# siyuanwu99/pred-occ-planner

Measured on AMD Instinct MI355X. Metric: replans/sec (SOGM update + QP: full replan = SOGM update + A* + corridors + QP + deconfliction), 128-agent batch per GPU, 200x200x200x20 voxel grid; aggregate over all agents, higher is better.
Workload: dtype f32 occupancy / f64 planning; 1 GPU; 128 agents/GPU x 1 GPU, 200x200x200x20 SOGM, sim_fkpcp-style moving cylinders, batched ADMM QP (BASELINE configs[2] per GPU); agents_total=128, cloud_points=622040, cylinders=555, map_input_staleness_ticks=0, parallelism=agents sharded x1, 1 all-gather/tick, exchange=local, sogm_grids_per_agent=3, sogm_reset=sparse (logged 32-byte sectors), sogm_cell_order=2x2x2 tiles, map_update=at the start of the tick

## Files before the change

include/sogm_abi_debug.h:

```cpp
#ifndef SOGM_ABI_DEBUG_H
#define SOGM_ABI_DEBUG_H
#include "sogm_abi.h"
#ifdef __cplusplus
extern "C" {
#endif

int sogm_sparse_reset_state(sogm_ctx *ctx, int32_t *out_host);

int         sogm_set_tuning(sogm_ctx *ctx, const char *key, double value);
int         sogm_get_tuning(const sogm_ctx *ctx, const char *key, double *out_value_host);
const char *sogm_tuning_key(int index);

int sogm_map_traffic(sogm_ctx *ctx, int64_t *out_host, int reset);

int sogm_grid_history(sogm_ctx *ctx, int32_t *out_host);

enum {
  SOGM_PROF_CLEAR = 0,
  SOGM_PROF_STAMP = 1,
  SOGM_PROF_SPLAT = 2,
  SOGM_PROF_ASTAR = 3,
  SOGM_PROF_CORRIDOR = 4,
  SOGM_PROF_QP = 5,
  SOGM_PROF_CLEAR_HEAD = 6,
  SOGM_PROF_EXCHANGE = 7,
  SOGM_PROF_N = 8
};
int sogm_set_profiling(sogm_ctx *ctx, int enable);
int sogm_set_profiling_slots(sogm_ctx *ctx, int slot_mask);
int sogm_profile_read(sogm_ctx *ctx, double *out_ms_host);
int sogm_profile_read_all(sogm_ctx *ctx, int slot, double *out_ms_host, int cap, int *out_n);

int sogm_device_clock(sogm_ctx *ctx, int64_t *out_ticks_host, void *stream);
int sogm_tick_clock(sogm_ctx *ctx, int64_t *out2_host);

int sogm_download_reference_layout(sogm_ctx *ctx, int agent, float *out_vt_host);

int sogm_dsp_download_state(sogm_dsp *d, int agent, float *store_host, float *objnum_host,
                            int32_t *counters_host);
int sogm_dsp_download_born(sogm_dsp *d, int agent, float *born_host, int cap, int32_t *n_born, int32_t *counters4);
int sogm_dsp_download_observations(sogm_dsp *d, int agent, int32_t *nobs_host, float *pc_host,
                                   float *maxlen_host);

int sogm_gridmap_download(sogm_gridmap *g, int agent, double *occupancy_host, int8_t *inflate_host,
                          int32_t *bounds_host, int32_t *counters_host);
int sogm_gridmap_force_frame(sogm_gridmap *g, int raycast_num);

int sogm_corridor_rules_batched(sogm_planner *counters_of, const SogmPlannerParams *pp_host, const double *start_pva,
                                const double *route, const int32_t *route_len, int route_cap, const double *polys,
                                const int32_t *nfaces, const int32_t *seg_state, int n, int max_faces, double *out_box,
                                double *out_shrunk, int32_t *out_seg_nfaces, int32_t *out_seg_state, double *out_polys,
                                int32_t *out_nfaces, int32_t *out_npoly, double *out_goal, void *stream);

#ifdef __cplusplus
}
#endif
#endif
```

pred-occ-planner_amd/_abi.py:

```python
import ctypes as C
import os

_HERE = os.path.dirname(os.path.abspath(__file__))
LIB_PATH = os.environ.get("SOGM_LIB_PATH") or os.path.join(_HERE, "libsogm_hip.so")

SOGM_ABI_VERSION = 6
SOGM_MAX_PIECES = 16
SOGM_MAP_FAKE = 0
SOGM_MAP_RISKBASE = 1
SOGM_MAP_RISKVOXEL = 2
SOGM_STORE_F32, SOGM_STORE_F16 = 0, 1
SOGM_LAYOUT_TILED = 16
SOGM_DSP_MAX_T = 16

SOGM_OK = 0
SOGM_ERR_INVALID_ARG = -1
SOGM_ERR_NO_DEVICE = -2
SOGM_ERR_HIP = -3
SOGM_ERR_CAPACITY = -4
SOGM_ERR_STATE = -5
SOGM_ERR_COMM = -6
SOGM_COMM_ID_BYTES = 128
PROF_CLEAR, PROF_STAMP, PROF_SPLAT, PROF_ASTAR, PROF_CORRIDOR, PROF_QP, PROF_CLEAR_HEAD, PROF_EXCHANGE, PROF_N = range(9)

COUNTER_NAMES = ("replan_ok", "fail_search", "fail_corridor", "fail_qp", "fail_unsafe", "corridor_capacity",
                 "pieces_capacity", "deconflict_capacity")

ASTAR_NO_PATH, ASTAR_INIT_ERR, ASTAR_SEARCH_ERR, ASTAR_REACH_HORIZON, ASTAR_REACH_END, ASTAR_NEAR_END = range(6)


class SogmSpec(C.Structure):
    _fields_ = [("L", C.c_int32), ("W", C.c_int32), ("H", C.c_int32), ("T", C.c_int32),
                ("resolution", C.c_float), ("time_resolution", C.c_float),
                ("risk_threshold", C.c_float), ("clearance", C.c_float),
                ("ground_height", C.c_float), ("ceiling_height", C.c_float),
                ("risk_threshold_region", C.c_float), ("risk_thres_reg_decay", C.c_float),
                ("risk_thres_vox_decay", C.c_float), ("map_kind", C.c_int32),
                ("storage", C.c_int32)]


class SogmDspParams(C.Structure):
    _fields_ = [("max_particle_num_voxel", C.c_int32), ("half_fov_h", C.c_int32),
                ("half_fov_v", C.c_int32), ("angle_resolution", C.c_int32),
                ("newborn_num", C.c_int32), ("obs_max_per_pyramid", C.c_int32),
                ("prediction_times", C.c_float * SOGM_DSP_MAX_T),
                ("sigma_observation", C.c_float), ("p_detection", C.c_float), ("kappa", C.c_float),
                ("newborn_weight", C.c_float), ("obstacle_thickness", C.c_float)]


class SogmGridMapParams(C.Structure):
    _fields_ = [("resolution", C.c_double), ("map_size", C.c_double * 3), ("local_update_range", C.c_double * 3),
                ("obstacles_inflation", C.c_double), ("fx", C.c_double), ("fy", C.c_double), ("cx", C.c_double),
                ("cy", C.c_double), ("depth_filter_maxdist", C.c_double), ("depth_filter_mindist", C.c_double),
                ("k_depth_scaling_factor", C.c_double), ("p_hit", C.c_double), ("p_miss", C.c_double),
                ("p_min", C.c_double), ("p_max", C.c_double), ("p_occ", C.c_double), ("max_ray_length", C.c_double),
                ("virtual_ceil_height", C.c_double), ("ground_height", C.c_double),
                ("use_depth_filter", C.c_int32), ("depth_filter_margin", C.c_int32), ("skip_pixel", C.c_int32),
                ("local_map_margin", C.c_int32), ("rows", C.c_int32), ("cols", C.c_int32)]


class SogmCylinder(C.Structure):
    _fields_ = [("type", C.c_int32), ("_pad", C.c_int32)] + [
        (k, C.c_double) for k in ("x", "y", "z", "w", "h", "vx", "vy", "qw", "qx", "qy", "qz")]


class SogmTrajRecord(C.Structure):
    _fields_ = [("drone_id", C.c_int32), ("n_pieces", C.c_int32), ("time_start", C.c_double),
                ("duration", C.c_double * SOGM_MAX_PIECES),
                ("cpts", C.c_double * (SOGM_MAX_PIECES * 15))]


class SogmAstarParams(C.Structure):
    _fields_ = [("max_tau", C.c_double), ("max_vel", C.c_double), ("max_acc", C.c_double),
                ("w_time", C.c_double), ("horizon", C.c_double), ("lambda_heu", C.c_double),
                ("resolution", C.c_double), ("time_resolution", C.c_double),
                ("allocate_num", C.c_int32), ("check_num", C.c_int32), ("tolerance", C.c_int32),
                ("shot_ignores_time", C.c_int32)]


class SogmPlannerParams(C.Structure):
    _fields_ = [("corridor_tau", C.c_double), ("init_range", C.c_double),
                ("shrink_size", C.c_double), ("opt_max_vel", C.c_double),
                ("opt_max_acc", C.c_double), ("fake_planner", C.c_int32),
                ("firi_iterations", C.c_int32), ("pc_capacity", C.c_int32),
                ("max_faces", C.c_int32)]


class SogmQpSettings(C.Structure):
    _fields_ = [("rho", C.c_double), ("sigma", C.c_double), ("alpha", C.c_double),
                ("eps_abs", C.c_double), ("eps_rel", C.c_double), ("max_iter", C.c_int32),
                ("check_termination", C.c_int32), ("scaling_iters", C.c_int32),
                ("adaptive_rho_interval", C.c_int32), ("residual_fp32", C.c_int32), ("reserved_", C.c_int32)]


class SogmWorld(C.Structure):
    _fields_ = [("cloud_xyz", C.c_void_p), ("block_bounds", C.c_void_p), ("cylinders", C.c_void_p),
                ("n_points", C.c_int32), ("n_blocks", C.c_int32), ("block_points", C.c_int32), ("n_cyl", C.c_int32)]


class SogmPrestamp(C.Structure):
    _fields_ = [("cloud_xyz", C.c_void_p), ("cloud_range", C.c_void_p), ("cylinders", C.c_void_p),
                ("n_cyl", C.c_int32), ("reserved_", C.c_int32), ("next_stamp", C.c_double),
                ("replan_start_offset", C.c_double), ("hover_inout", C.c_void_p), ("out_now", C.c_void_p),
                ("out_t_start", C.c_void_p), ("out_pva", C.c_void_p), ("out_poses", C.c_void_p),
                ("world", C.POINTER(SogmWorld))]


class SogmFlight(C.Structure):
    _fields_ = [("n_ticks", C.c_int32), ("first_tick", C.c_int32), ("t0", C.c_double), ("period", C.c_double),
                ("replan_start_offset", C.c_double), ("worlds", C.POINTER(SogmWorld)), ("goals", C.c_void_p),
                ("drone_ids", C.c_void_p), ("hover_inout", C.c_void_p), ("own_inout", C.c_void_p),
                ("tables", C.c_void_p), ("n_total", C.c_int32), ("agent0", C.c_int32), ("log_records", C.c_void_p),
                ("log_ok", C.c_void_p), ("nccl_comm", C.c_void_p)]


class SogmAuditParams(C.Structure):
    _fields_ = [("body", C.c_double * 3), ("sample_dt", C.c_double), ("goal_tolerance", C.c_double),
                ("t_obstacles", C.c_double), ("event_capacity", C.c_int32), ("reserved_", C.c_int32)]


class SogmAuditAgent(C.Structure):
    _fields_ = [("min_gap", C.c_double), ("min_gap_time", C.c_double), ("min_sep", C.c_double),
                ("min_sep_time", C.c_double), ("goal_time", C.c_double), ("first_collision_time", C.c_double),
                ("path_length", C.c_double), ("last_pos", C.c_double * 3), ("min_gap_obstacle", C.c_int32),
                ("min_sep_agent", C.c_int32), ("obstacle_samples", C.c_int32), ("agent_samples", C.c_int32),
                ("n_samples", C.c_int32), ("has_last", C.c_int32)]


class SogmAuditEvent(C.Structure):
    _fields_ = [("t", C.c_double), ("agent", C.c_int32), ("other", C.c_int32), ("kind", C.c_int32),
                ("reserved_", C.c_int32)]


SOGM_AUDIT_AGENT, SOGM_AUDIT_OBSTACLE = 0, 1
AUDIT_AGENT_BYTES = C.sizeof(SogmAuditAgent)
AUDIT_EVENT_BYTES = C.sizeof(SogmAuditEvent)


class SogmFsmParams(C.Structure):
    _fields_ = [("replan_duration", C.c_double), ("replan_start_time", C.c_double), ("goal_tolerance", C.c_double),
                ("new_plan_interval", C.c_double), ("replan_max_failures", C.c_int32), ("reserved_", C.c_int32)]


class SogmFsmState(C.Structure):
    _fields_ = [("traj_start", C.c_double), ("status", C.c_int32), ("fail", C.c_int32), ("success", C.c_int32),
                ("reserved_", C.c_int32)]


class SogmFlightFsm(C.Structure):
    _fields_ = [("prm", SogmFsmParams), ("check_duration", C.c_double), ("state_inout", C.c_void_p),
                ("log_state", C.c_void_p), ("log_due", C.c_void_p), ("log_safe", C.c_void_p), ("log_reached", C.c_void_p),
                ("log_pub", C.c_void_p), ("log_hover_start", C.c_void_p), ("log_own", C.c_void_p)]


FSM_STATE_BYTES = C.sizeof(SogmFsmState)
FSM_PUB_NONE, FSM_PUB_NEW, FSM_PUB_HOVER = 0, 1, 2

FLIGHT_MAX_TICKS = 64
FLIGHT_HDR_ERR, FLIGHT_HDR_FINISHED, FLIGHT_HDR_LATE_WGS = 4, 5, 15
FLIGHT_STAT_NAMES = ("gate_wait", "map", "search", "corridor", "qp", "finish", "chain", "ticks")
TRAJ_RECORD_BYTES = C.sizeof(SogmTrajRecord)
CYLINDER_BYTES = C.sizeof(SogmCylinder)

_vp = C.c_void_p
_i = C.c_int

PROTOTYPES = {
    "sogm_abi_version": (_i, []),
    "sogm_last_error": (C.c_char_p, []),
    "sogm_device_count": (_i, []),
    "sogm_create": (_i, [C.POINTER(SogmSpec), _i, _i, C.POINTER(_vp)]),
    "sogm_destroy": (None, [_vp]),
    "sogm_grid_bytes": (C.c_int64, [_vp]),
    "sogm_grid_ptr": (_vp, [_vp]),
    "sogm_set_sparse_reset": (_i, [_vp, _i, _i]),
    "sogm_sparse_reset_state": (_i, [_vp, _vp]),
    "sogm_grid_history": (_i, [_vp, _vp]),
    "sogm_map_traffic": (_i, [_vp, _vp, _i]),
    "sogm_set_resample": (_i, [_vp, C.c_float, _i, _vp, _i]),
    "sogm_set_tuning": (_i, [_vp, C.c_char_p, C.c_double]),
    "sogm_get_tuning": (_i, [_vp, C.c_char_p, C.POINTER(C.c_double)]),
    "sogm_tuning_key": (C.c_char_p, [_i]),
    "sogm_set_body_particles": (_i, [_vp, C.POINTER(C.c_double), _i]),
    "sogm_set_overlap_clear": (_i, [_vp, _i]),
    "sogm_set_profiling": (_i, [_vp, _i]),
    "sogm_set_profiling_slots": (_i, [_vp, _i]),
    "sogm_profile_read": (_i, [_vp, C.POINTER(C.c_double)]),
    "sogm_profile_read_all": (_i, [_vp, _i, C.POINTER(C.c_double), _i, C.POINTER(_i)]),
    "sogm_update_gt": (_i, [_vp, _vp, _vp, _vp, _i, _vp, _vp, _vp]),
    "sogm_project_neighbours": (_i, [_vp, _vp, _i, _vp, _vp]),
    "sogm_update_gt_swarm": (_i, [_vp, _vp, _vp, _vp, _i, _vp, _vp, _vp, _i, _vp, _vp]),
    "sogm_device_clock": (_i, [_vp, C.POINTER(C.c_int64), _vp]),
    "sogm_tick_clock": (_i, [_vp, C.POINTER(C.c_int64)]),
    "sogm_cloud_block_bounds": (_i, [_vp, _i, _i, _vp, _vp]),
    "sogm_update_world": (_i, [_vp, C.POINTER(SogmWorld), _vp, _vp, _vp, _i, _vp, _vp]),
    "sogm_set_future_risk": (_i, [_vp, _vp, _vp, _vp, _vp]),
    "sogm_download_reference_layout": (_i, [_vp, _i, _vp]),
    "sogm_tick_inputs": (_i, [_vp, _i, C.c_double, C.c_double, _vp, _vp, _vp, _vp, _vp, _vp]),
    "sogm_merge_latest": (_i, [_vp, _vp, _vp, _vp, _i, _vp]),
    "sogm_fsm_init": (_i, [_vp, _i, C.c_double, _vp]),
    "sogm_fsm_inputs": (_i, [C.POINTER(SogmFsmParams), _vp, _vp, _vp, _i, C.c_double, _vp, _vp, _vp, _vp, _vp, _vp, _vp,
                             _vp, _vp]),
    "sogm_fsm_apply": (_i, [C.POINTER(SogmFsmParams), _vp, _vp, _vp, _vp, _vp, _vp, _vp, _vp, _vp, _vp, _vp, _i,
                            C.c_double, _vp]),
    "sogm_map_state": (_i, [_vp, _i, C.POINTER(C.c_double), C.POINTER(C.c_float), _vp]),
    "sogm_traj_eval": (_i, [_vp, _i, _vp, _vp, _vp, _vp]),
    "sogm_firi_batched": (_i, [_vp, _i, _vp, _vp, _vp, _vp, _vp, _i, C.c_double, _i, _i, _i, _vp, _vp, _vp, _vp]),
    "sogm_planner_select_agents": (_i, [_vp, _i, _i]),
    "sogm_planner_set_search_mode": (_i, [_vp, _i]),
    "sogm_query_clear": (_i, [_vp, _vp, _vp, _vp, _i, _i, _vp, _vp]),
    "sogm_obstacle_points": (_i, [_vp, _vp, _vp, _vp, _vp, _vp, _i, _vp, _vp, _i, _vp]),
    "sogm_planner_create": (_i, [_vp, C.POINTER(SogmAstarParams), C.POINTER(SogmPlannerParams),
                                 C.POINTER(SogmQpSettings), C.POINTER(_vp)]),
    "sogm_planner_destroy": (None, [_vp]),
    "sogm_astar_search": (_i, [_vp, _vp, _vp, _vp, _vp, _vp, _vp, _i, _vp, _vp, _i, _vp]),
    "sogm_corridor_generate": (_i, [_vp, _vp, _vp, _vp, _vp, _i, _vp, _vp, _vp, _vp, _vp]),
    "sogm_bezier_qp_solve": (_i, [_vp, _vp, _vp, _vp, _vp, _vp, _vp, _vp, _vp, _vp]),
    "sogm_bezier_qp_solve_timed": (_i, [_vp, _vp, _vp, _vp, C.c_double, C.c_double, _vp, _vp, _vp, _vp, _vp, _vp, _vp]),
    "sogm_linprog_batched": (_i, [_i, _vp, _vp, _vp, _vp, _i, _vp, _vp, _vp]),
    "sogm_corridor_rules_batched": (_i, [_vp, _vp, _vp, _vp, _vp, _i, _vp, _vp, _vp, _i, _i, _vp, _vp, _vp, _vp, _vp, _vp,
                                         _vp, _vp, _vp]),
    "sogm_replan": (_i, [_vp, _vp, _vp, _vp, _vp, _vp, _vp, _vp]),
    "sogm_gridmap_create": (_i, [C.POINTER(SogmGridMapParams), _i, _i, C.POINTER(_vp)]),
    "sogm_gridmap_destroy": (None, [_vp]),
    "sogm_gridmap_update": (_i, [_vp, _vp, _vp, _vp, _vp, _vp]),
    "sogm_gridmap_query_inflate": (_i, [_vp, _vp, _vp, _i, _vp, _vp]),
    "sogm_gridmap_download": (_i, [_vp, _i, _vp, _vp, _vp, _vp]),
    "sogm_gridmap_force_frame": (_i, [_vp, _i]),
    "sogm_traj_safe": (_i, [_vp, _vp, _vp, C.c_double, _vp, _vp]),
    "sogm_safe_after_opt": (_i, [_vp, _vp, _vp, _vp, _i, _vp, _vp, _vp, _vp]),
    "sogm_planner_flow_error": (_i, [_vp]),
    "sogm_planner_flow_failures": (_i, [_vp, _vp]),
    "sogm_planner_set_publish": (_i, [_vp, _vp, _vp]),
    "sogm_planner_set_prestamp": (_i, [_vp, _vp]),
    "sogm_prestamp_pending": (_i, [_vp]),
    "sogm_prestamp_join": (_i, [_vp, _vp]),
    "sogm_update_prestamped": (_i, [_vp, _vp, _i, _vp, _vp]),
    "sogm_planner_counters": (_i, [_vp, C.POINTER(C.c_int64), _i]),
    "sogm_flight_run": (_i, [_vp, C.POINTER(SogmFlight), _vp]),
    "sogm_flight_prepare": (_i, [_vp, _i]),
    "sogm_flight_stats": (_i, [_vp, _vp, _vp]),
    "sogm_planner_set_swarm": (_i, [_vp, _vp, _i, _vp, _vp]),
    "sogm_planner_set_due": (_i, [_vp, _vp]),
    "sogm_planner_set_flight_fsm": (_i, [_vp, C.POINTER(SogmFlightFsm)]),
    "sogm_audit_init_agents": (_i, [_vp, _i, _vp]),
    "sogm_swarm_audit": (_i, [C.POINTER(SogmAuditParams), _vp, _i, _i, _vp, C.c_double, _i, C.c_double, _i, _i, _vp, _vp,
                              _vp, _i, _vp, _vp, _vp, _vp]),
    "sogm_traj_allgather": (_i, [_vp, _vp, _vp, _i, _vp, _vp]),
    "sogm_exchange_wait": (_i, [_vp, _vp]),
    "sogm_comm_unique_id": (_i, [C.c_char_p]),
    "sogm_comm_create": (_i, [C.c_char_p, _i, _i, _i, C.POINTER(_vp)]),
    "sogm_comm_destroy": (None, [_vp]),
    "sogm_comm_handle": (_vp, [_vp]),
    "sogm_comm_info": (_i, [_vp, _vp]),
    "sogm_filter_point_cloud": (_i, [_vp, _vp, _vp, C.c_float, _i, _vp, _vp, _vp]),
    "sogm_filter_reserve": (_i, [_vp, _i]),
    "sogm_dsp_create": (_i, [_vp, C.POINTER(SogmDspParams), _vp, _vp, _i, _vp, _i, _i, C.POINTER(_vp)]),
    "sogm_dsp_destroy": (None, [_vp]),
    "sogm_update_dsp": (_i, [_vp, _vp, _vp, _vp, _vp, _vp, _vp, _vp, _vp]),
    "sogm_dsp_publish": (_i, [_vp, _vp, _vp]),
    "sogm_dsp_download_state": (_i, [_vp, _i, _vp, _vp, _vp]),
    "sogm_dsp_download_born": (_i, [_vp, _i, _vp, _i, _vp, _vp]),
    "sogm_dsp_download_observations": (_i, [_vp, _i, _vp, _vp, _vp]),
}


class SogmError(RuntimeError):
    pass


def load_library(path=LIB_PATH):
    if not os.path.exists(path):
        raise SogmError(
            f"HIP extension not built: {path} is missing. Run `python -c 'import __graft_entry__ as g; "
            "g.build()'` (hipcc --offload-arch=gfx950). There is no CPU fallback.")
    try:
        import torch
    except ImportError:
        pass
    lib = C.CDLL(path)
    for name, (res, args) in PROTOTYPES.items():
        fn = getattr(lib, name)
        fn.restype = res
        fn.argtypes = args
    got = lib.sogm_abi_version()
    if got != SOGM_ABI_VERSION:
        raise SogmError(f"{path} implements ABI version {got}, this binding was written against {SOGM_ABI_VERSION}: "
                        "rebuild the extension (python -c 'import __graft_entry__ as g; g.build()')")
    return lib


_lib = None


def lib():
    global _lib
    if _lib is None:
        _lib = load_library()
    return _lib


def check(rc, what):
    if rc != SOGM_OK:
        msg = lib().sogm_last_error()
        raise SogmError(f"{what} failed: status {rc} ({msg.decode() if msg else ''})")
```

pred-occ-planner_amd/csrc/sogm_corridor.hip:

```cpp
#include <hip/hip_runtime.h>

#include <cfloat>

#include "../../include/sogm_detmath.h"
#include "sogm_fsm.hpp"
#include "sogm_lp.hpp"
#include "sogm_planner.hpp"

namespace sogm {
namespace {

__device__ inline double dot3(const double *a, const double *b) {
  return (a[0] * b[0] + a[1] * b[1]) + a[2] * b[2];
}

__device__ inline bool smoothedL1(double mu, double x, double &f, double &df) {
  if (x < 0.0) return false;
  if (x > mu) {
    f  = x - 0.5 * mu;
    df = 1.0;
    return true;
  }
  const double xdmu = x / mu, sqrxdmu = xdmu * xdmu, mumxd2 = mu - 0.5 * x;
  f  = mumxd2 * sqrxdmu * xdmu;
// ... 825 lines not shown
  const double   *rt    = DIRECT ? nullptr : io.route + (size_t)agent * io.route_cap * 6;
  const double   *sp    = DIRECT ? nullptr : io.start_pva + agent * 9;
  const int       cap   = pp.pc_capacity;
  const int       prob  = DIRECT ? fd.first + slot : 0;
  const double   *pc    = DIRECT ? fd.pc + (size_t)fd.pc_range[prob * 2] * 3 : ws.pc + (size_t)slot * cap * 3;
  double         *fpc   = ws.fpc + (size_t)slot * cap * 3;
  double         *tang  = ws.tang + (size_t)slot * cap * 4;
  double         *distR = ws.distr + (size_t)slot * cap;

  long long *dbg = ws.seg_dbg + (size_t)slot * 16;
  const long long tk0 = wall_clock64();
  const int M = DIRECT ? fd.n_bd : 6;
  if (lane == 0) {
    for (int k = 0; k < 12; ++k) dbg[k] = 0;
    if constexpr (DIRECT) {
      for (int i = 0; i < 4 * M; ++i) s_bd[i] = fd.bd[(size_t)prob * M * 4 + i];
      for (int k = 0; k < 3; ++k) {
        s_w[k]     = fd.a[prob * 3 + k];
        s_w[3 + k] = fd.b[prob * 3 + k];
      }
    } else {
      segment_box(pp, sp, rt, seg, s_box, s_w);
      for (int i = 0; i < 24; ++i) s_bd[i] = 0;
      for (int k = 0; k < 3; ++k) {
        s_bd[k * 4 + k]       = 1.0;
        s_bd[(k + 3) * 4 + k] = -1.0;
        s_bd[k * 4 + 3]       = -s_box[3 + k];
        s_bd[(k + 3) * 4 + 3] = s_box[k];
      }
    }
  }
  __syncthreads();

  int N = DIRECT ? fd.pc_range[prob * 2 + 1] - fd.pc_range[prob * 2] : ws.seg_npts[slot];
  int overflow = 0;
  if (N > cap) {
    N        = cap;
    overflow = 1;
  }
  __syncthreads();

  if (lane == 0) {
    dbg[0] = N;
    dbg[5] = wall_clock64() - tk0;
  }
  const double epsilon = DIRECT ? fd.epsilon : 1.0e-6;
  int          nH      = 0;
  const int    n_iter  = DIRECT ? fd.iterations : pp.firi_iterations;
  bool         seed_ok = true;
  if (lane == 0) {
    int ok = 1;
    for (int i = 0; i < M; ++i) {
      const double *h = s_bd + i * 4;
      if (dot3(h, s_w) + h[3] > 0.0 || dot3(h, s_w + 3) + h[3] > 0.0) ok = 0;
    }
    s_int[0] = ok;
  }
  __syncthreads();
  seed_ok = s_int[0] != 0;

  if (seed_ok) {
    double R[3][3] = {{1, 0, 0}, {0, 1, 0}, {0, 0, 1}};
    double p[3]    = {0.5 * (s_w[0] + s_w[3]), 0.5 * (s_w[1] + s_w[4]), 0.5 * (s_w[2] + s_w[5])};
    double r[3]    = {1, 1, 1};
    if constexpr (DIRECT)
      for (int k = 0; k < 3; ++k) r[k] = fd.r[prob * 3 + k];
    for (int loop = 0; loop < n_iter; ++loop) {
      if (lane == 0) {
        double forward[3][3], backward[3][3];
        for (int k = 0; k < 3; ++k)
          for (int j = 0; j < 3; ++j) {
            forward[k][j]    = (1.0 / r[k]) * R[j][k];
            backward[k][j]   = R[k][j] * r[j];
            s_fwd[k * 3 + j] = forward[k][j];
          }
        for (int i = 0; i < M; ++i) {
          const double *h = s_bd + i * 4;
          for (int j = 0; j < 3; ++j)
            s_fB[i * 3 + j] =
                (h[0] * backward[0][j] + h[1] * backward[1][j]) + h[2] * backward[2][j];
          s_fD[i] = h[3] + dot3(h, p);
        }
        const double da[3] = {s_w[0] - p[0], s_w[1] - p[1], s_w[2] - p[2]};
        const double db[3] = {s_w[3] - p[0], s_w[4] - p[1], s_w[5] - p[2]};
        for (int k = 0; k < 3; ++k) {
          s_fa[k] = dot3(forward[k], da);
          s_fb[k] = dot3(forward[k], db);
          s_p[k]  = p[k];
        }
        for (int i = 0; i < M; ++i) {
          const double *fb = s_fB + i * 3;
          s_dD[i]          = dabs(s_fD[i]) / sogm_det::sqrt_rn(dot3(fb, fb));
        }
      }
      __syncthreads();
      double lmin = INFINITY;
      int    lidx = 0x7fffffff;
      {
        double fwd[9], fa[3], fb[3], pp3[3];
        for (int k = 0; k < 9; ++k) fwd[k] = s_fwd[k];
        for (int k = 0; k < 3; ++k) {
          fa[k]  = s_fa[k];
          fb[k]  = s_fb[k];
          pp3[k] = s_p[k];
        }
        for (int i = lane; i < N; i += 64) {
          const double d[3] = {pc[i * 3] - pp3[0], pc[i * 3 + 1] - pp3[1], pc[i * 3 + 2] - pp3[2]};
          double       q[3];
          for (int k = 0; k < 3; ++k) q[k] = dot3(fwd + k * 3, d);
          double t[4];
          double dr = sogm_det::sqrt_rn(dot3(q, q));
          t[3]      = -dr;
          for (int k = 0; k < 3; ++k) t[k] = q[k] / dr;
          if (dot3(t, fa) + t[3] > epsilon) {
            const double delta[3] = {q[0] - fa[0], q[1] - fa[1], q[2] - fa[2]};
            const double s        = dot3(delta, fa) / dot3(delta, delta);
            for (int k = 0; k < 3; ++k) t[k] = fa[k] - s * delta[k];
            dr   = sogm_det::sqrt_rn(dot3(t, t));
            t[3] = -dr;
            for (int k = 0; k < 3; ++k) t[k] /= dr;
          }
          if (dot3(t, fb) + t[3] > epsilon) {
            const double delta[3] = {q[0] - fb[0], q[1] - fb[1], q[2] - fb[2]};
            const double s        = dot3(delta, fb) / dot3(delta, delta);
            for (int k = 0; k < 3; ++k) t[k] = fb[k] - s * delta[k];
            dr   = sogm_det::sqrt_rn(dot3(t, t));
            t[3] = -dr;
            for (int k = 0; k < 3; ++k) t[k] /= dr;
          }
          if (dot3(t, fa) + t[3] > epsilon) {
            const double u[3] = {fa[0] - q[0], fa[1] - q[1], fa[2] - q[2]};
            const double v[3] = {fb[0] - q[0], fb[1] - q[1], fb[2] - q[2]};
            double       n[3] = {u[1] * v[2] - u[2] * v[1], u[2] * v[0] - u[0] * v[2],
                                 u[0] * v[1] - u[1] * v[0]};
            const double nn   = sogm_det::sqrt_rn(dot3(n, n));
            if (nn > 0)
              for (int k = 0; k < 3; ++k) n[k] /= nn;
            for (int k = 0; k < 3; ++k) t[k] = n[k];
            t[3]            = -dot3(t, fa);
            const double sg = t[3] > 0.0 ? -1.0 : 1.0;
            for (int k = 0; k < 4; ++k) t[k] *= sg;
          }
          for (int k = 0; k < 3; ++k) fpc[i * 3 + k] = q[k];
          for (int k = 0; k < 4; ++k) tang[i * 4 + k] = t[k];
          distR[i]  = dr;
          {
            const unsigned long long act = __ballot(1);
            if (lane == 0) s_fw[i >> 6] = act;
          }
          if (dr < lmin) {
            lmin = dr;
            lidx = i;
          }
        }
      }
      wave_argmin(lmin, lidx);
      double minSqrR = lmin;
      int    pcMinId = lidx == 0x7fffffff ? 0 : lidx;
      double minSqrD = INFINITY;
      int    bdMinId = 0;
      unsigned bdFlags = M >= 32 ? 0xffffffffu : (1u << M) - 1u;
      for (int j = 0; j < M; ++j)
        if (s_dD[j] < minSqrD) {
          minSqrD = s_dD[j];
          bdMinId = j;
        }
      nH             = 0;
      bool completed = false;
      for (int i = 0; !completed && i < (M + N); ++i) {
        __syncthreads();
        if (lane == 0) {
          double *fh = s_fH + (nH < FIRI_MAX_H ? nH : FIRI_MAX_H - 1) * 4;
          if (minSqrD < minSqrR) {
            for (int k = 0; k < 3; ++k) fh[k] = s_fB[bdMinId * 3 + k];
            fh[3] = s_fD[bdMinId];
          } else {
            for (int k = 0; k < 4; ++k) fh[k] = tang[pcMinId * 4 + k];
            s_fw[pcMinId >> 6] &= ~(1ull << (pcMinId & 63));
          }
          for (int k = 0; k < 4; ++k) s_fh[k] = fh[k];
        }
        if (minSqrD < minSqrR) bdFlags &= ~(1u << bdMinId);
        __syncthreads();
        completed = true;
        minSqrD   = INFINITY;
        for (int j = 0; j < M; ++j)
          if (bdFlags & (1u << j)) {
            completed = false;
            if (minSqrD > s_dD[j]) {
              bdMinId = j;
              minSqrD = s_dD[j];
            }
          }
        const double fh0 = s_fh[0], fh1 = s_fh[1], fh2 = s_fh[2], fh3 = s_fh[3];
        double       lm = INFINITY;
        int          li = 0x7fffffff;
        int          open = 0;
        for (int j = lane; j < N; j += 64) {
          const unsigned long long word = s_fw[j >> 6];
          bool                     covered = false;
          if ((word >> lane) & 1ull) {
            const double *q = fpc + j * 3;
            if (((fh0 * q[0] + fh1 * q[1]) + fh2 * q[2]) + fh3 > -epsilon) {
              covered = true;
            } else {
              open = 1;
              if (lm > distR[j]) {
                lm = distR[j];
                li = j;
              }
            }
          }
          const unsigned long long clr = __ballot(covered);
          if (clr != 0ull && lane == 0) s_fw[j >> 6] = word & ~clr;
        }
        wave_argmin(lm, li);
        if (__any(open)) completed = false;
        minSqrR = lm;
        pcMinId = li == 0x7fffffff ? 0 : li;
        ++nH;
      }
      __syncthreads();
      if (nH > FIRI_MAX_H) {
        nH       = FIRI_MAX_H;
        overflow = 1;
      }
      for (int i = lane; i < nH; i += 64) {
        const double *fh = s_fH + i * 4;
        double        h[4];
        for (int j = 0; j < 3; ++j)
          h[j] = (fh[0] * s_fwd[0 * 3 + j] + fh[1] * s_fwd[1 * 3 + j]) + fh[2] * s_fwd[2 * 3 + j];
        h[3] = fh[3] - dot3(h, s_p);
        for (int k = 0; k < 4; ++k) s_poly[i * 4 + k] = h[k];
      }
      __syncthreads();
      if (lane == 0) {
        dbg[1 + (loop > 0)] = nH;
        dbg[6 + 2 * (loop > 0)] = wall_clock64() - tk0;
      }
      if (loop == n_iter - 1) break;
      {
        const int       mm  = nH < LP_MAX_ROWS - 9 ? nH : LP_MAX_ROWS - 9;
        const long long tm0 = wall_clock64();
        maxVolInsEllipsoid(s_poly, mm, R, p, r, sc, base + L::lm, base + L::handoff, dbg);
        if (lane == 0) dbg[7] = wall_clock64() - tm0;
      }
      __syncthreads();
    }
    if constexpr (DIRECT)
      if (lane == 0)
        for (int k = 0; k < 3; ++k) fd.r[prob * 3 + k] = r[k];
  }

  if constexpr (DIRECT) {
    int nf = seed_ok ? nH : 0;
    if (nf > fd.max_faces) {
      nf       = fd.max_faces;
      overflow = 1;
    }
    double *out = fd.hpoly + (size_t)prob * fd.max_faces * 4;
    for (int i = lane; i < nf * 4; i += 64) out[i] = s_poly[i];
    if (lane == 0) {
      fd.nfaces[prob] = nf;
      fd.status[prob] = overflow ? -3 : (seed_ok ? 1 : 0);
    }
    return;
  }
  int nf = seed_ok ? nH : 0;
  if (nf > pp.max_faces) {
    nf       = pp.max_faces;
    overflow = 1;
  }
  shrink_corridor(pp, s_w, s_poly, nf);
  wave_lds_sync();
  const bool valid = corridorValidW(s_poly, nf, nullptr, 0, sc);
  {
    double *out = ws.polys + (size_t)slot * pp.max_faces * 4;
    for (int i = lane; i < nf * 4; i += 64) out[i] = s_poly[i];
  }
  if (lane == 0) {
    ws.seg_nfaces[slot] = nf;
    ws.seg_state[slot]  = overflow ? -3 : (valid ? 1 : 0);
    ws.seg_npts[slot]   = N;
    dbg[10]             = wall_clock64() - tk0;
  }
}

__global__ __launch_bounds__(64) void k_corridor_segment(
    MapView m, SogmPlannerParams pp, CorridorWorkspace ws, const double *__restrict__ start_pva,
    const double *__restrict__ t_start, const double *__restrict__ route,
    const int32_t *__restrict__ route_len, int route_cap, int agent0) {
  extern __shared__ __attribute__((aligned(16))) char smem[];
  const CorridorIO io{.start_pva = start_pva, .t_start = t_start, .route = route, .route_len = route_len,
                      .route_cap = route_cap};
  corridor_segment_body<6, false>(m, pp, ws, io, blockIdx.y + agent0, blockIdx.x, smem, FiriDirect{});
}

__global__ __launch_bounds__(64) void k_firi_direct(MapView m, SogmPlannerParams pp, CorridorWorkspace ws,
                                                    FiriDirect fd) {
  extern __shared__ __attribute__((aligned(16))) char smem[];
  corridor_segment_body<FIRI_DIRECT_BD_MAX, true>(m, pp, ws, CorridorIO{}, blockIdx.x, 0, smem, fd);
}

__device__ __forceinline__ void corridor_finalize_body(const SogmPlannerParams &pp, const CorridorWorkspace &ws,
                                                       const CorridorIO &io, int agent, const LpScratch &sc) {
  const bool    w0    = threadIdx.x == 0;
  const int     MF    = pp.max_faces;
  const double *polys = ws.polys + (size_t)agent * SOGM_MAX_PIECES * MF * 4;
  const int    *nfs   = ws.seg_nfaces + agent * SOGM_MAX_PIECES;
  const int    *state = ws.seg_state + agent * SOGM_MAX_PIECES;
  const double *rt    = io.route + (size_t)agent * io.route_cap * 6;
  const double *sp    = io.start_pva + agent * 9;
  const int     rl    = io.points(agent);
  int           npoly = 0;
  if (w0) {
    for (int i = 0; i < SOGM_MAX_PIECES; ++i) io.out_nfaces[agent * SOGM_MAX_PIECES + i] = 0;
    for (int i = 0; i < 6; ++i) io.out_goal[agent * 6 + i] = 0;
    io.out_npoly[agent] = 0;
  }
  if (!pp.fake_planner && rl < 2) return;
  if (rl < 1) return;
  for (int i = 0; i < rl - 1 && i < SOGM_MAX_PIECES; ++i) {
    if (state[i] != 1) {
      if (state[i] == -3 && w0 && ws.counters) atomicAdd(&ws.counters[SOGM_CNT_CORRIDOR_CAPACITY], 1ull);
      break;
    }
    ++npoly;
  }
  if (npoly == SOGM_MAX_PIECES && io.route_len[agent] - 1 > SOGM_MAX_PIECES && w0 && ws.counters)
    atomicAdd(&ws.counters[SOGM_CNT_PIECES_CAPACITY], 1ull);
  if (npoly == 0) return;
  for (int i = 0; i + 1 < npoly; ++i) {
    if (!corridorValidW(polys + (size_t)i * MF * 4, nfs[i], polys + (size_t)(i + 1) * MF * 4,
                        nfs[i + 1], sc)) {
      if (i < 2) return;
      npoly = pp.fake_planner ? i + 1 : i;
      break;
    }
  }
  if (pp.fake_planner ? npoly == 0 : npoly <= 1) return;
  double gpos[3], gvel[3];
  int    gi = npoly - 1;
  for (int k = 0; k < 3; ++k) {
    gpos[k] = rt[gi * 6 + k];
    gvel[k] = rt[gi * 6 + 3 + k];
  }
  bool do_scan = true;
  if (!pp.fake_planner)
    do_scan = !goalReachableW(polys + (size_t)(npoly - 1) * MF * 4, nfs[npoly - 1], sp, gpos, sc);
  if (do_scan) {
    for (int it = npoly - 1; it != 0; --it) {
      if (goalReachableW(polys + (size_t)it * MF * 4, nfs[it], sp, gpos, sc)) {
        npoly         = it + 1;
        const int idx = npoly - 1;
        for (int k = 0; k < 3; ++k) {
          gpos[k] = rt[idx * 6 + k];
          gvel[k] = rt[idx * 6 + 3 + k];
        }
        break;
      }
    }
  }
  for (int i = 0; i < npoly; ++i) {
    if (w0) io.out_nfaces[agent * SOGM_MAX_PIECES + i] = nfs[i];
    const double *src = polys + (size_t)i * MF * 4;
    double       *dst = io.out_polys + ((size_t)agent * SOGM_MAX_PIECES + i) * MF * 4;
    for (int k = threadIdx.x; k < nfs[i] * 4; k += 64) dst[k] = src[k];
  }
  if (w0) {
    for (int k = 0; k < 3; ++k) {
      io.out_goal[agent * 6 + k]     = gpos[k];
      io.out_goal[agent * 6 + 3 + k] = gvel[k];
    }
    io.out_npoly[agent] = npoly;
  }
}

__global__ __launch_bounds__(64) void k_corridor_finalize(
    SogmPlannerParams pp, CorridorWorkspace ws, const double *__restrict__ start_pva,
    const double *__restrict__ route, const int32_t *__restrict__ route_len, int route_cap,
    double *__restrict__ out_polys, int32_t *__restrict__ out_nfaces,
    int32_t *__restrict__ out_npoly, double *__restrict__ out_goal, int agent0) {
  const CorridorIO io{.start_pva = start_pva, .route = route, .route_len = route_len, .route_cap = route_cap,
                      .out_polys = out_polys, .out_nfaces = out_nfaces, .out_npoly = out_npoly, .out_goal = out_goal};
  extern __shared__ __attribute__((aligned(16))) char smem[];
  corridor_finalize_body(pp, ws, io, blockIdx.x + agent0, LpLds::carve(smem));
}

struct CorridorRules {
  const SogmPlannerParams *pp;
  const double            *polys_in;
  const int32_t           *nfaces_in;
  const int32_t           *state_in;
  double                  *out_box;
};
__global__ __launch_bounds__(64) void k_corridor_rules(CorridorRules cr, CorridorWorkspace ws, CorridorIO io) {
  extern __shared__ __attribute__((aligned(16))) char smem[];
  double *base = (double *)smem, *s_poly = base + RulesLds::poly, *s_box = base + RulesLds::box, *s_w = base + RulesLds::w;
  const LpScratch sc{base + LpLds::work, base + LpLds::rows, (int *)(smem + RulesLds::perm)};
  const int               prob = blockIdx.x, lane = threadIdx.x;
  const SogmPlannerParams pp   = cr.pp[prob];
  const int               MF   = pp.max_faces;
  const int               rl   = io.points(prob);
  for (int seg = 0; seg < SOGM_MAX_PIECES; ++seg) {
    const int slot = prob * SOGM_MAX_PIECES + seg;
    if (seg >= rl - 1) {
      if (lane == 0) {
        ws.seg_state[slot]  = -2;
        ws.seg_nfaces[slot] = 0;
        for (int k = 0; k < 6; ++k) cr.out_box[slot * 6 + k] = 0.0;
      }
      continue;
    }
    int nf = cr.nfaces_in[slot];
    nf     = nf < 0 ? 0 : (nf > MF ? MF : nf);
    if (lane == 0) segment_box(pp, io.start_pva + prob * 9, io.route + (size_t)prob * io.route_cap * 6, seg, s_box, s_w);
    for (int i = lane; i < nf * 4; i += 64) s_poly[i] = cr.polys_in[(size_t)slot * MF * 4 + i];
    wave_lds_sync();
    shrink_corridor(pp, s_w, s_poly, nf);
    wave_lds_sync();
    const bool valid = corridorValidW(s_poly, nf, nullptr, 0, sc);
    double    *out   = ws.polys + (size_t)slot * MF * 4;
    for (int i = lane; i < nf * 4; i += 64) out[i] = s_poly[i];
    if (lane == 0) {
      for (int k = 0; k < 6; ++k) cr.out_box[slot * 6 + k] = s_box[k];
      ws.seg_nfaces[slot] = nf;
      ws.seg_state[slot]  = cr.state_in && cr.state_in[slot] == -3 ? -3 : (valid ? 1 : 0);
    }
    wave_lds_sync();
  }
  __threadfence_block();
  __syncthreads();
  corridor_finalize_body(pp, ws, io, prob, sc);
}

__device__ __forceinline__ bool corridor_slot(const MapView &m, const SogmPlannerParams &pp, const CorridorWorkspace &ws,
                                              const CorridorIO &io, int agent, int seg, char *smem, int *seg_done,
                                              bool cumulative, long long *stamps) {
  if (seg < io.points(agent) - 1) {
    corridor_points_body<1>(m, pp, ws, io, agent, seg);
    __threadfence_block();
    __syncthreads();
  }
  if (stamps && threadIdx.x == 0) stamps[13] = wall_clock64();
  corridor_segment_body<6, false>(m, pp, ws, io, agent, seg, smem, FiriDirect{});
  __syncthreads();
  if (stamps && threadIdx.x == 0) stamps[14] = wall_clock64();
  __threadfence();
  const int done = flow_ticket(&seg_done[agent]);
  if ((cumulative ? done & (SOGM_MAX_PIECES - 1) : done) != SOGM_MAX_PIECES - 1) return false;
  __threadfence();
  corridor_finalize_body(pp, ws, io, agent, LpLds::carve(smem));
  __syncthreads();
  return true;
}

__global__ __launch_bounds__(64) void k_corridor_flow(MapView m, SogmPlannerParams pp, CorridorWorkspace ws,
                                                      FlowCtl fc, CorridorIO io, int n_agents) {
  extern __shared__ __attribute__((aligned(16))) char smem[];
  const int lane  = threadIdx.x;
  const int total = n_agents * SOGM_MAX_PIECES;
  for (;;) {
    const int k = flow_ticket(&fc.hdr[FLOW_C_TICKET]);
    if (k >= total) break;
    const int agent = flow_wait_slot(fc.a_ready + k / SOGM_MAX_PIECES, &fc.hdr[FLOW_ERR]);
    if (agent < 0) break;
    __threadfence();
    const int seg = k % SOGM_MAX_PIECES;
    if (seg == 0 && lane == 0) fc.ts[agent * 8 + 2] = wall_clock64();
    if (corridor_slot(m, pp, ws, io, agent, seg, smem, fc.seg_done, false, nullptr)) {
      if (lane == 0) fc.ts[agent * 8 + 3] = wall_clock64();
      __threadfence();
      if (lane == 0) publish_next(fc.q_ready, &fc.hdr[FLOW_Q_READY_N], agent);
    }
    __syncthreads();
  }
}

__device__ __forceinline__ bool deconflict_pair_unsafe(const double *ca, int M, const SogmTrajRecord &r, int ego_id,
                                                       double now, const LpScratch &sc, unsigned long long *counters) {
  if (M <= 0) return false;
  if (r.n_pieces <= 0 || r.drone_id == ego_id) return false;
  double time_end = r.time_start;
  for (int k = 0; k < r.n_pieces; ++k) time_end += r.duration[k];
  if (!(r.time_start < now && now < time_end)) return false;
  double t     = now - r.time_start;
  int    piece = r.n_pieces - 1;
  for (int k = 0; k < r.n_pieces; ++k) {
    t -= r.duration[k];
    if (t < 0) {
      piece = k;
      break;
    }
  }
  const int nA = 5 * M, nB = (r.n_pieces - piece) * 5;
  if (nA + nB > DECONFLICT_MAX_ROWS) {
    if ((threadIdx.x & 63) == 0 && counters) atomicAdd(&counters[SOGM_CNT_DECONFLICT_CAPACITY], 1ull);
    return true;
  }
  double       *A = sc.A(), *b = sc.b();
  const double *cb = r.cpts + piece * 15;
  {
    double lo[6], hi[6];
    for (int k = 0; k < 6; ++k) {
      lo[k] = INFINITY;
      hi[k] = -INFINITY;
    }
    for (int q = threadIdx.x; q < nA; q += 64)
      for (int k = 0; k < 3; ++k) {
        lo[k] = fmin(lo[k], ca[q * 3 + k]);
        hi[k] = fmax(hi[k], ca[q * 3 + k]);
      }
    for (int q = threadIdx.x; q < nB; q += 64)
      for (int k = 0; k < 3; ++k) {
        lo[3 + k] = fmin(lo[3 + k], cb[q * 3 + k]);
        hi[3 + k] = fmax(hi[3 + k], cb[q * 3 + k]);
      }
    bool apart = false;
    for (int k = 0; k < 6; ++k)
      for (int d = 32; d >= 1; d >>= 1) {
        lo[k] = fmin(lo[k], __shfl_xor(lo[k], d, 64));
        hi[k] = fmax(hi[k], __shfl_xor(hi[k], d, 64));
      }
    for (int k = 0; k < 3; ++k) apart = apart || hi[k] < lo[3 + k] || hi[3 + k] < lo[k];
    if (apart) return false;
    double dirs[11][3] = {{1, 1, 0}, {1, -1, 0}, {1, 0, 1}, {1, 0, -1}, {0, 1, 1}, {0, 1, -1},
                          {1, 1, 1}, {1, 1, -1}, {1, -1, 1}, {1, -1, -1}, {0, 0, 0}};
    for (int k = 0; k < 3; ++k) dirs[10][k] = 0.5 * (lo[3 + k] + hi[3 + k]) - 0.5 * (lo[k] + hi[k]);
#pragma unroll
    for (int q = 0; q < 11; ++q) {
      const double n0 = dirs[q][0], n1 = dirs[q][1], n2 = dirs[q][2];
      double loA = INFINITY, hiA = -INFINITY, loB = INFINITY, hiB = -INFINITY;
      for (int i = threadIdx.x; i < nA; i += 64) {
        const double v = (n0 * ca[i * 3] + n1 * ca[i * 3 + 1]) + n2 * ca[i * 3 + 2];
        loA = fmin(loA, v);
        hiA = fmax(hiA, v);
      }
      for (int i = threadIdx.x; i < nB; i += 64) {
        const double v = (n0 * cb[i * 3] + n1 * cb[i * 3 + 1]) + n2 * cb[i * 3 + 2];
        loB = fmin(loB, v);
        hiB = fmax(hiB, v);
      }
      for (int d = 32; d >= 1; d >>= 1) {
        loA = fmin(loA, __shfl_xor(loA, d, 64));
        hiA = fmax(hiA, __shfl_xor(hiA, d, 64));
        loB = fmin(loB, __shfl_xor(loB, d, 64));
        hiB = fmax(hiB, __shfl_xor(hiB, d, 64));
      }
      if (hiA < loB || hiB < loA) return false;
    }
  }
  for (int q = threadIdx.x; q < nA + nB; q += 64) {
    if (q < nA) {
      A[q * 4 + 0] = -ca[q * 3 + 0];
      A[q * 4 + 1] = -ca[q * 3 + 1];
      A[q * 4 + 2] = -ca[q * 3 + 2];
      A[q * 4 + 3] = -1.0;
    } else {
      const int e  = q - nA;
      A[q * 4 + 0] = cb[e * 3 + 0];
      A[q * 4 + 1] = cb[e * 3 + 1];
      A[q * 4 + 2] = cb[e * 3 + 2];
      A[q * 4 + 3] = 1.0;
    }
    b[q] = -1.0;
  }
  if (threadIdx.x < 8) {
    const int q = nA + nB + threadIdx.x, k = threadIdx.x >> 1;
    for (int j = 0; j < 4; ++j) A[q * 4 + j] = j == k ? ((threadIdx.x & 1) ? -1.0 : 1.0) : 0.0;
    b[q] = 1.0e4;
  }
  wave_lds_sync();
  const double c[4] = {0, 0, 0, 0};
  double       x[4];
  const double v = linprog_wave<4>(c, nA + nB + 8, A, b, x, sc.work, sc.perm);
  wave_lds_sync();
  return v == INFINITY || v == -INFINITY;
}

__device__ inline bool deconflict_prefilter(const double *sA, int nA, const double *boxA, const double (*prA)[2],
                                            const SogmTrajRecord &r, int ego_id, double now) {
  const int np = r.n_pieces;
  if (np <= 0 || r.drone_id == ego_id) return false;
  const double ts = r.time_start;
  double       time_end = ts;
  for (int k = 0; k < np; ++k) time_end += r.duration[k];
  if (!(ts < now && now < time_end)) return false;
  double t     = now - ts;
  int    piece = np - 1;
  for (int k = 0; k < np; ++k) {
    t -= r.duration[k];
    if (t < 0) {
      piece = k;
      break;
    }
  }
  const int nB = (np - piece) * 5;
  if (nA + nB > DECONFLICT_MAX_ROWS) return true;
  const double *cb = r.cpts + piece * 15;
  const double  dirs[10][3] = {{1, 1, 0}, {1, -1, 0}, {1, 0, 1}, {1, 0, -1}, {0, 1, 1},
                               {0, 1, -1}, {1, 1, 1}, {1, 1, -1}, {1, -1, 1}, {1, -1, -1}};
  double lo[3] = {INFINITY, INFINITY, INFINITY}, hi[3] = {-INFINITY, -INFINITY, -INFINITY};
  double plo[10], phi[10];
#pragma unroll
  for (int q = 0; q < 10; ++q) {
    plo[q] = INFINITY;
    phi[q] = -INFINITY;
  }
#pragma unroll 4
  for (int i = 0; i < nB; ++i) {
    const double x = cb[i * 3], y = cb[i * 3 + 1], z = cb[i * 3 + 2];
    lo[0] = fmin(lo[0], x);
    hi[0] = fmax(hi[0], x);
    lo[1] = fmin(lo[1], y);
    hi[1] = fmax(hi[1], y);
    lo[2] = fmin(lo[2], z);
    hi[2] = fmax(hi[2], z);
#pragma unroll
    for (int q = 0; q < 10; ++q) {
      const double v = (dirs[q][0] * x + dirs[q][1] * y) + dirs[q][2] * z;
      plo[q]         = fmin(plo[q], v);
      phi[q]         = fmax(phi[q], v);
    }
  }
  for (int k = 0; k < 3; ++k)
    if (boxA[3 + k] < lo[k] || hi[k] < boxA[k]) return false;
#pragma unroll
  for (int q = 0; q < 10; ++q)
    if (prA[q][1] < plo[q] || phi[q] < prA[q][0]) return false;
  double n[3];
  for (int k = 0; k < 3; ++k) n[k] = 0.5 * (lo[k] + hi[k]) - 0.5 * (boxA[k] + boxA[3 + k]);
  double loA = INFINITY, hiA = -INFINITY, loB = INFINITY, hiB = -INFINITY;
  for (int i = 0; i < nA; ++i) {
    const double v = (n[0] * sA[i * 3] + n[1] * sA[i * 3 + 1]) + n[2] * sA[i * 3 + 2];
    loA            = fmin(loA, v);
    hiA            = fmax(hiA, v);
  }
  for (int i = 0; i < nB; ++i) {
    const double v = (n[0] * cb[i * 3] + n[1] * cb[i * 3 + 1]) + n[2] * cb[i * 3 + 2];
    loB            = fmin(loB, v);
    hiB            = fmax(hiB, v);
  }
  if (hiA < loB || hiB < loA) return false;
  return true;
}

__global__ __launch_bounds__(64) void k_safe_after_opt(const double *__restrict__ cpts,
                                                       const int32_t *__restrict__ npoly,
                                                       const SogmTrajRecord *__restrict__ rec, int n_rec,
                                                       const int32_t *__restrict__ ego_ids,
                                                       const double *__restrict__ t_now,
                                                       int32_t *__restrict__ out_safe, int agent0,
                                                       unsigned long long *counters) {
  extern __shared__ __attribute__((aligned(16))) double s_dyn[];
  const int a = blockIdx.y + agent0, i = blockIdx.x;
  if (deconflict_pair_unsafe(cpts + (size_t)a * SOGM_MAX_PIECES * 15, npoly[a], rec[i], ego_ids[a], t_now[a],
                             LpLds::carve(s_dyn), counters) &&
      threadIdx.x == 0)
    out_safe[a] = 0;
}

__device__ __forceinline__ int finish_agent(const FinishArgs &f, int a, const LpScratch &sc, int lane) {
  const int M    = f.npoly[a];
  int       safe = 1;
  const bool solved = f.ret[a] != 0 && M > 0 && (f.status[a] == 1 || f.status[a] == 2);
  if (f.swarm && solved) {
    const double *ca  = f.cpts + (size_t)a * SOGM_MAX_PIECES * 15;
    const int     ego = f.swarm_ego[a];
    const double  now = f.swarm_now[a];
    const int     nA  = 5 * M;
    double *sA = sc.work;
    double  boxA[6], prA[10][2];
    auto stage_A = [&]() {
      for (int q = lane; q < nA * 3; q += 64) sA[q] = ca[q];
      wave_lds_sync();
    };
    stage_A();
    {
      const double dirs[10][3] = {{1, 1, 0}, {1, -1, 0}, {1, 0, 1}, {1, 0, -1}, {0, 1, 1},
                                  {0, 1, -1}, {1, 1, 1}, {1, 1, -1}, {1, -1, 1}, {1, -1, -1}};
      double lo[13], hi[13];
#pragma unroll
      for (int k = 0; k < 13; ++k) {
        lo[k] = INFINITY;
        hi[k] = -INFINITY;
      }
      for (int q = lane; q < nA; q += 64) {
        const double x = sA[q * 3], y = sA[q * 3 + 1], z = sA[q * 3 + 2];
        lo[0] = fmin(lo[0], x);
        hi[0] = fmax(hi[0], x);
        lo[1] = fmin(lo[1], y);
        hi[1] = fmax(hi[1], y);
        lo[2] = fmin(lo[2], z);
        hi[2] = fmax(hi[2], z);
#pragma unroll
        for (int k = 0; k < 10; ++k) {
          const double v = (dirs[k][0] * x + dirs[k][1] * y) + dirs[k][2] * z;
          lo[3 + k]      = fmin(lo[3 + k], v);
          hi[3 + k]      = fmax(hi[3 + k], v);
        }
      }
#pragma unroll
      for (int k = 0; k < 13; ++k)
        for (int d = 32; d >= 1; d >>= 1) {
          lo[k] = fmin(lo[k], __shfl_xor(lo[k], d, 64));
          hi[k] = fmax(hi[k], __shfl_xor(hi[k], d, 64));
        }
      for (int k = 0; k < 3; ++k) {
        boxA[k]     = lo[k];
        boxA[3 + k] = hi[k];
      }
#pragma unroll
      for (int k = 0; k < 10; ++k) {
        prA[k][0] = lo[3 + k];
        prA[k][1] = hi[3 + k];
      }
    }
    for (int i0 = 0; i0 < f.n_swarm && safe; i0 += 64) {
      const int  i    = i0 + lane;
      const bool need = i < f.n_swarm && deconflict_prefilter(sA, nA, boxA, prA, f.swarm[i], ego, now);
      unsigned long long m = __ballot(need);
      bool               lp_ran = false;
      while (m != 0 && safe) {
        const int j = __builtin_ctzll(m);
        m &= m - 1;
        if (deconflict_pair_unsafe(ca, M, f.swarm[i0 + j], ego, now, sc, f.counters)) safe = 0;
        lp_ran = true;
      }
      if (lp_ran && safe && i0 + 64 < f.n_swarm) stage_A();
    }
  }
#ifdef SOGM_FLOW_DEBUG
  if (lane == 0) f.out_safe[a] = 101;
#else
  if (lane == 0 && f.out_safe) f.out_safe[a] = safe;
#endif
  const bool      good = solved && safe != 0;
  SogmTrajRecord *dst[3] = {f.out + a, (good && f.pub_own) ? f.pub_own + a : nullptr,
                            (good && f.pub_own && f.pub_table) ? f.pub_table + a : nullptr};
#pragma unroll
  for (int k = 0; k < 3; ++k) {
    SogmTrajRecord *r = dst[k];
    if (!r) continue;
    for (int i = lane; i < SOGM_MAX_PIECES; i += 64) r->duration[i] = (good && i < M) ? f.corridor_tau : 0.0;
    for (int i = lane; i < SOGM_MAX_PIECES * 15; i += 64)
      r->cpts[i] = (good && i < M * 15) ? f.cpts[(size_t)a * SOGM_MAX_PIECES * 15 + i] : 0.0;
    if (lane == 0) {
      r->drone_id   = f.drone_ids[a];
      r->time_start = f.t_start[a];
      r->n_pieces   = good ? M : 0;
    }
  }
  if (!good && f.pub_own && f.pub_table)
    copy_record(f.pub_table + a, f.pub_own + a, lane);
  if (lane == 0) f.out_ok[a] = good ? 1 : 0;
  return (safe ? 1 : 0) | (good ? 2 : 0);
}
// ... 3 lines not shown
  if (f.due && f.due[a] == 0) return;
  const int M = f.npoly[a];
  int       k = SOGM_CNT_REPLAN_OK;
  if (f.ret[a] == 0) k = SOGM_CNT_FAIL_SEARCH;
  else if (M <= 0) k = SOGM_CNT_FAIL_CORRIDOR;
  else if (!(f.status[a] == 1 || f.status[a] == 2)) k = SOGM_CNT_FAIL_QP;
  else if (!safe) k = SOGM_CNT_FAIL_UNSAFE;
  atomicAdd(&f.counters[k], 1ull);
}
__global__ __launch_bounds__(64) void k_finish_flow(FlowCtl fc, FinishArgs f, int n_agents) {
  extern __shared__ __attribute__((aligned(16))) double s_dyn[];
  const int lane = threadIdx.x;
  for (;;) {
    const int k = flow_ticket(&fc.hdr[FLOW_F_TICKET]);
    if (k >= n_agents) break;
    const int a = flow_wait_slot(fc.f_ready + k, &fc.hdr[FLOW_ERR]);
    if (a < 0) break;
    __threadfence();
    const int  code = finish_agent(f, a, LpLds::carve(s_dyn), lane);
    const bool safe = (code & 1) != 0;
    if (fc.p_ready) {
      __threadfence();
      if (lane == 0) publish_next(fc.p_ready, &fc.hdr[FLOW_P_READY_N], a);
    }
    if (lane == 0) {
      fc.ts[a * 8 + 6] = wall_clock64();
      finish_count(f, a, safe);
    }
  }
}

__device__ inline int flight_fsm_traj_safe(const MapView &m, const FlightFsmDev &u, const FinishArgs &f, int a, int lane) {
  const int mine = traj_safe_agent(m, a, f.pub_own[a], f.swarm_now[a], u.check_duration, lane, 64);
  return __ballot(mine == 0) == 0ull ? 1 : 0;
}
__device__ inline void flight_fsm_apply(const FlightFsmDev &u, const FinishArgs &f, int a, size_t row, bool ok, int safe,
                                        int lane) {
  const double stamp = f.swarm_now[a];
  int          kind  = 0;
  double       start = 0.0;
  if (lane == 0) {
    SogmFsmState  s       = u.state[a];
    const int32_t due     = u.due[a], reached = u.reached[a];
    const FsmPub  pub     = fsm_step(s, due, ok, safe != 0, reached != 0, stamp, u.prm);
    u.state[a]            = s;
    kind                  = pub.kind;
    start                 = pub.hover_start;
    if (u.log_state) u.log_state[row] = s;
    if (u.log_due) u.log_due[row] = due;
    if (u.log_safe) u.log_safe[row] = safe;
    if (u.log_reached) u.log_reached[row] = reached;
    if (u.log_pub) u.log_pub[row] = pub.kind;
    if (u.log_hover_start) u.log_hover_start[row] = pub.hover_start;
  }
  kind  = __shfl(kind, 0, 64);
  start = __shfl(start, 0, 64);
  if (kind == SOGM_FSM_PUB_HOVER) {
    const double p[3] = {u.pos_now[a * 3], u.pos_now[a * 3 + 1], u.pos_now[a * 3 + 2]};
    fsm_hover_record(f.pub_own[a], f.drone_ids[a], p, start, lane, 64);
    if (f.pub_table) fsm_hover_record(f.pub_table[a], f.drone_ids[a], p, start, lane, 64);
  }
  if (u.log_own) {
    __threadfence();
    copy_record(u.log_own + row, f.pub_own + a, lane);
  }
}

__global__ __launch_bounds__(64) void k_flight_light(MapView m, SogmPlannerParams pp, CorridorWorkspace ws, FlightCtl fl,
                                                     FlightLightDev d) {
  extern __shared__ __attribute__((aligned(16))) char smem[];
  const int      lane  = threadIdx.x;
  const unsigned total = (unsigned)fl.n_agents * (unsigned)fl.n_ticks * (SOGM_MAX_PIECES + 1);
  int           *err   = &fl.hdr[FL_ERR];
  fl_wg_started(fl, 2);
  long long      c1_prev = 0;
  int            kind_prev = 0;
  for (;;) {
    const unsigned t = (unsigned)flow_ticket(&fl.hdr[FL_LW_HEAD]);
    if (t >= total) break;
    const long long c0   = wall_clock64();
    const int       desc = wq_take(fl.lw, t, err);
    if (desc < 0) break;
    __threadfence();
    const long long c1 = wall_clock64();
    if (lane == 0) {
      if (c1_prev) {
        atomicAdd(&fl.prof[kind_prev == WK_FINISH ? 8 : 7], (unsigned long long)(c0 - c1_prev));
        atomicAdd(&fl.prof[kind_prev == WK_FINISH ? 15 : 14], 1ull);
      }
      atomicAdd(&fl.prof[6], (unsigned long long)(c1 - c0));
    }
    const int kind = wk_kind(desc), a = wk_agent(desc);
    c1_prev   = c1;
    kind_prev = kind;
    if (kind == WK_FINISH) {
      const int k  = fl.tick_of[a];
      const int kl = k - fl.first_tick;
      FinishArgs f = d.fin;
      f.swarm      = d.tables ? d.tables + (size_t)((k - fl.lag) & 3) * d.n_total : nullptr;
      f.pub_table  = d.tables ? d.tables + (size_t)(k & 3) * d.n_total + d.agent0 : nullptr;
      f.out        = d.log_records + (size_t)kl * fl.n_agents;
      f.out_ok     = d.log_ok + (size_t)kl * fl.n_agents;
      int traj_safe = 1;
      if (d.fsm.state) traj_safe = flight_fsm_traj_safe(m, d.fsm, f, a, lane);
      const int code = finish_agent(f, a, LpLds::carve(smem), lane);
      if (d.fsm.state) flight_fsm_apply(d.fsm, f, a, (size_t)kl * fl.n_agents + a, (code & 2) != 0, traj_safe, lane);
      __syncthreads();
      __threadfence();
      if (lane == 0) {
        const long long now = wall_clock64();
        long long      *ts  = fl.ts + (size_t)a * FL_TS, *acc = fl.acc + (size_t)a * 8;
        ts[6]               = now;
        acc[0] += ts[14] - ts[10];
        acc[1] += (ts[11] - ts[7]) - (ts[14] - ts[10]);
        acc[2] += ts[1] - ts[11];
        acc[3] += ts[3] - ts[1];
        acc[4] += ts[5] - ts[3];
        acc[5] += now - ts[5];
        acc[6] += now - ts[7];
        acc[7] += 1;
        if (fl.ts_log) {
          long long *lg = fl.ts_log + ((size_t)kl * fl.n_agents + a) * FL_TS;
          for (int q = 0; q < FL_TS; ++q) lg[q] = ts[q];
        }
        finish_count(f, a, (code & 1) != 0);
        const int A_      = fl.n_agents;
        const int done_kl = __hip_atomic_fetch_add(&fl.tick_done[kl], 1, __ATOMIC_ACQ_REL, __HIP_MEMORY_SCOPE_AGENT) + 1;
        if (atomicAdd(&fl.hdr[FL_FINISHED], 1) + 1 == A_ * fl.n_ticks)
          __hip_atomic_store(&fl.hdr[FL_END], fl.epoch, __ATOMIC_RELEASE, __HIP_MEMORY_SCOPE_AGENT);
        if (kl + 1 < fl.n_ticks) {
          fl.tick_of[a] = k + 1;
          ts[7]         = now;
          const bool urgent = fl.n_urgent > 0 && done_kl > A_ - fl.n_urgent;
          fl.urgent[a]      = urgent ? 1 : 0;
          fl_publish(urgent ? fl.u_ring : fl.m_ring, fl.ring_mask, &fl.hdr[urgent ? FL_U_READY : FL_M_READY], a);
        }
        if (done_kl == A_ && kl + fl.lag < fl.n_ticks && !fl.xready) fl_gate_release(fl, kl + fl.lag);
      }
      continue;
    }
    const int seg = wk_sub(desc);
    if (seg == 0 && lane == 0) fl.ts[a * FL_TS + 2] = wall_clock64();
    long long *sdbg = ws.seg_dbg + ((size_t)a * SOGM_MAX_PIECES + seg) * 16;
    if (lane == 0) {
      sdbg[12] = c1;
      sdbg[13] = 0;
      sdbg[14] = 0;
      sdbg[15] = (long long)(unsigned)__builtin_amdgcn_s_getreg(63492) | ((long long)(unsigned)__builtin_amdgcn_s_getreg(63508) << 32);
    }
    if (corridor_slot(m, pp, ws, d.cor, a, seg, smem, fl.seg_done, true, sdbg)) {
      if (lane == 0) {
        fl.ts[a * FL_TS + 3] = wall_clock64();
        fl_publish(fl.q_ring, fl.ring_mask, &fl.hdr[FL_Q_READY], a);
      }
    }
    __syncthreads();
  }
}

__global__ void k_flow_gate(FlowCtl fc, int expected) {
  if (threadIdx.x != 0) return;
  wait_at_least<WaitResidencyGate, false>(&fc.hdr[FLOW_ERR], &fc.hdr[FLOW_A_RESIDENT], expected);
}

template <int D>
__global__ __launch_bounds__(64) void k_linprog(const double *__restrict__ c, const double *__restrict__ A,
                                                const double *__restrict__ b,
                                                const int32_t *__restrict__ row_range,
                                                double *__restrict__ out_x, double *__restrict__ out_min) {
  extern __shared__ __attribute__((aligned(16))) double s_dyn[];
  const LpScratch sc = LpLds::carve(s_dyn);
  const int       p = blockIdx.x, lane = threadIdx.x;
  const int r0 = row_range[2 * p], rows = row_range[2 * p + 1] - r0;
  if (rows >= LP_MAX_ROWS || rows < 0) {
    if (lane == 0) {
      out_min[p] = __builtin_nan("");
      for (int j = 0; j < D; ++j) out_x[p * D + j] = __builtin_nan("");
    }
    return;
  }
  for (int i = lane; i < rows; i += 64) {
    for (int j = 0; j < D; ++j) sc.A()[i * D + j] = A[(size_t)(r0 + i) * D + j];
    sc.b()[i] = b[r0 + i];
  }
  wave_lds_sync();
  double cv[D], x[D];
  for (int j = 0; j < D; ++j) cv[j] = c[p * D + j];
  const double v = linprog_wave<D>(cv, rows, sc.A(), sc.b(), x, sc.work, sc.perm);
  if (lane == 0) {
    out_min[p] = v;
    for (int j = 0; j < D; ++j) out_x[p * D + j] = x[j];
  }
}

__global__ void k_fill_i32(int32_t *p, int n, int32_t v, int agent0) {
  const int i = blockIdx.x * blockDim.x + threadIdx.x;
  if (i < n) p[agent0 + i] = v;
}

hipError_t launch_deconflict(int n_agents, const double *cpts, const int32_t *npoly, const SogmTrajRecord *rec,
                             int n_rec, const int32_t *ego_ids, const double *t_now, int32_t *out_safe,
                             hipStream_t st, int agent0, unsigned long long *counters) {
  hipLaunchKernelGGL(k_fill_i32, dim3((n_agents + 63) / 64), dim3(64), 0, st, out_safe, n_agents, 1, agent0);
  if (n_rec > 0)
    hipLaunchKernelGGL(k_safe_after_opt, dim3(n_rec, n_agents), dim3(64), LpLds::bytes(), st, cpts, npoly, rec, n_rec,
                       ego_ids, t_now, out_safe, agent0, counters);
  return hipGetLastError();
}

hipError_t launch_flow_gate(const FlowCtl &fc, int expected, hipStream_t st) {
  hipLaunchKernelGGL(k_flow_gate, dim3(1), dim3(64), 0, st, fc, expected);
  return hipGetLastError();
}

hipError_t launch_corridor_flow(const MapView &m, const SogmPlannerParams &pp, const CorridorWorkspace &ws,
                                const FlowCtl &fc, int n_agents, int n_workgroups, const CorridorIO &io, hipStream_t st) {
  hipLaunchKernelGGL(k_corridor_flow, dim3(n_workgroups), dim3(64), SegmentLds<6>::bytes(pp.pc_capacity), st, m, pp,
                     ws, fc, io, n_agents);
  return hipGetLastError();
}

hipError_t launch_finish_flow(const FlowCtl &fc, int n_agents, int n_workgroups, const FinishArgs &f, hipStream_t st) {
  hipLaunchKernelGGL(k_finish_flow, dim3(n_workgroups), dim3(64), LpLds::bytes(), st, fc, f, n_agents);
  return hipGetLastError();
}

hipError_t launch_flight_light(const MapView &m, const SogmPlannerParams &pp, const CorridorWorkspace &ws, const FlightCtl &fl,
                               const FlightLightDev &d, int n_workgroups, hipStream_t st) {
  hipLaunchKernelGGL(k_flight_light, dim3(n_workgroups), dim3(64), SegmentLds<6>::bytes(pp.pc_capacity), st, m, pp, ws, fl, d);
  return hipGetLastError();
}

hipError_t launch_corridor(const MapView &m, const SogmPlannerParams &pp, const CorridorWorkspace &ws, int n_agents,
                           const CorridorIO &io, hipStream_t st, int agent0, hipEvent_t ev_map_read) {
  hipLaunchKernelGGL(k_corridor_points, dim3(SOGM_MAX_PIECES, n_agents), dim3(256), 0, st, m, pp, ws, io.start_pva,
                     io.t_start, io.route, io.route_len, io.route_cap, agent0);
  hipError_t e = hipGetLastError();
  if (e == hipSuccess && ev_map_read) e = hipEventRecord(ev_map_read, st);
  if (e != hipSuccess) return e;
  hipLaunchKernelGGL(k_corridor_segment, dim3(SOGM_MAX_PIECES, n_agents), dim3(64),
                     SegmentLds<6>::bytes(pp.pc_capacity), st, m, pp, ws, io.start_pva, io.t_start, io.route,
                     io.route_len, io.route_cap, agent0);
  if ((e = hipGetLastError()) != hipSuccess) return e;
  hipLaunchKernelGGL(k_corridor_finalize, dim3(n_agents), dim3(64), LpLds::bytes(), st, pp, ws, io.start_pva, io.route,
                     io.route_len, io.route_cap, io.out_polys, io.out_nfaces, io.out_npoly, io.out_goal, agent0);
  return hipGetLastError();
}

}

extern "C" int sogm_linprog_batched(int d, const double *c, const double *A, const double *b,
                                    const int32_t *row_range, int n, double *out_x, double *out_min,
                                    void *stream) {
  if ((d != 3 && d != 4) || n < 0 || (n > 0 && (!c || !row_range || !out_x || !out_min)))
    return SOGM_ERR_INVALID_ARG;
  if (n == 0) return SOGM_OK;
  const size_t lds = sogm::LpLds::bytes();
  hipStream_t  st  = (hipStream_t)stream;
  if (d == 3)
    hipLaunchKernelGGL(sogm::k_linprog<3>, dim3(n), dim3(64), lds, st, c, A, b, row_range, out_x, out_min);
  else
    hipLaunchKernelGGL(sogm::k_linprog<4>, dim3(n), dim3(64), lds, st, c, A, b, row_range, out_x, out_min);
  SOGM_HIP_CHECK(hipGetLastError());
  return SOGM_OK;
}

extern "C" int sogm_firi_batched(const double *bd, int n_bd, const double *pc_xyz, const int32_t *pc_range,
                                 const double *a, const double *b, double *r, int iterations, double epsilon, int n,
                                 int max_points, int max_faces, double *out_hpoly, int32_t *out_nfaces,
                                 int32_t *out_status, void *stream) {
  if (n < 0 || n_bd < 1 || n_bd > FIRI_DIRECT_BD_MAX || iterations < 1 || max_points < 1 || max_points > 16384 ||
      max_faces < 1 || max_faces > FIRI_MAX_H ||
      (n > 0 && (!bd || !pc_range || !a || !b || !r || !out_hpoly || !out_nfaces || !out_status)))
    return SOGM_ERR_INVALID_ARG;
  if (n == 0) return SOGM_OK;
  hipStream_t st = (hipStream_t)stream;
  const size_t per = sizeof(double) * 8 * (size_t)max_points + sizeof(long long) * 16;
  char        *scratch = nullptr;
  SOGM_HIP_CHECK(hipMallocAsync((void **)&scratch, per * (size_t)n, st));
  sogm::CorridorWorkspace ws{};
  ws.fpc     = (double *)scratch;
  ws.tang    = ws.fpc + (size_t)n * max_points * 3;
  ws.distr   = ws.tang + (size_t)n * max_points * 4;
  ws.seg_dbg = (long long *)(ws.distr + (size_t)n * max_points);
  SogmPlannerParams pp{};
  pp.pc_capacity = max_points;
  sogm::FiriDirect fd{bd, n_bd, pc_xyz, pc_range, a, b, r, iterations, out_hpoly, out_nfaces, out_status,
                      max_faces, 0, epsilon};
  hipLaunchKernelGGL(sogm::k_firi_direct, dim3(n), dim3(64), sogm::SegmentLds<FIRI_DIRECT_BD_MAX>::bytes(max_points), st, sogm::MapView{},
                     pp, ws, fd);
  const hipError_t e = hipGetLastError();
  (void)hipFreeAsync(scratch, st);
  SOGM_HIP_CHECK(e);
  return SOGM_OK;
}

extern "C" int sogm_corridor_rules_batched(sogm_planner *counters_of, const SogmPlannerParams *pp_host,
                                           const double *start_pva, const double *route, const int32_t *route_len,
                                           int route_cap, const double *polys, const int32_t *nfaces,
                                           const int32_t *seg_state, int n, int max_faces, double *out_box,
                                           double *out_shrunk, int32_t *out_seg_nfaces, int32_t *out_seg_state,
                                           double *out_polys, int32_t *out_nfaces, int32_t *out_npoly,
                                           double *out_goal, void *stream) {
  if (n < 0 || max_faces < 1 || max_faces > RULES_MAX_FACES || route_cap <= SOGM_MAX_PIECES ||
      (n > 0 && (!pp_host || !start_pva || !route || !route_len || !polys || !nfaces || !out_box || !out_shrunk ||
                 !out_seg_nfaces || !out_seg_state || !out_polys || !out_nfaces || !out_npoly || !out_goal)))
    return SOGM_ERR_INVALID_ARG;
  for (int i = 0; i < n; ++i)
    if (pp_host[i].max_faces != max_faces) return SOGM_ERR_INVALID_ARG;
  if (n == 0) return SOGM_OK;
  hipStream_t        st   = (hipStream_t)stream;
  SogmPlannerParams *d_pp = nullptr;
  SOGM_HIP_CHECK(hipMallocAsync((void **)&d_pp, sizeof(SogmPlannerParams) * (size_t)n, st));
  hipError_t e = hipMemcpyAsync(d_pp, pp_host, sizeof(SogmPlannerParams) * (size_t)n, hipMemcpyHostToDevice, st);
  if (e == hipSuccess) e = hipStreamSynchronize(st);
  if (e == hipSuccess) {
    sogm::CorridorWorkspace ws{};
    ws.polys      = out_shrunk;
    ws.seg_nfaces = out_seg_nfaces;
    ws.seg_state  = out_seg_state;
    ws.counters   = counters_of ? counters_of->cw.counters : nullptr;
    const sogm::CorridorIO    io{.start_pva = start_pva, .route = route, .route_len = route_len, .route_cap = route_cap,
                                 .out_polys = out_polys, .out_nfaces = out_nfaces, .out_npoly = out_npoly,
                                 .out_goal = out_goal};
    const sogm::CorridorRules cr{d_pp, polys, nfaces, seg_state, out_box};
    hipLaunchKernelGGL(sogm::k_corridor_rules, dim3(n), dim3(64), sogm::RulesLds::bytes(), st, cr, ws, io);
    e = hipGetLastError();
  }
  (void)hipFreeAsync(d_pp, st);
  SOGM_HIP_CHECK(e);
  return SOGM_OK;
}

extern "C" int sogm_debug_corridor_occupancy(int pc_capacity) {
  int n = 0;
  if (hipOccupancyMaxActiveBlocksPerMultiprocessor(&n, (const void *)sogm::k_corridor_segment, 64,
                                                   sogm::SegmentLds<6>::bytes(pc_capacity)) != hipSuccess)
    return -1;
  return n;
}

#ifdef SOGM_PROFILE_MVIE
extern "C" int sogm_debug_mvie_prof(unsigned long long *out2) {
  if (hipMemcpyFromSymbol(out2, HIP_SYMBOL(sogm::g_mvie_prof), 16) != hipSuccess) return -1;
  if (hipMemcpyFromSymbol(out2 + 2, HIP_SYMBOL(sogm::g_lbfgs_prof), 40) != hipSuccess) return -1;
  unsigned long long z[5] = {0, 0, 0, 0, 0};
  (void)hipMemcpyToSymbol(HIP_SYMBOL(sogm::g_mvie_prof), z, 16);
  (void)hipMemcpyToSymbol(HIP_SYMBOL(sogm::g_lbfgs_prof), z, 40);
  return 0;
}
#endif
```

pred-occ-planner_amd/csrc/sogm_flight.hip:

```cpp
#include <hip/hip_runtime.h>

#include <cstdio>
#include <new>

#include "sogm_flight_layout.hpp"
#include "sogm_planner.hpp"

using namespace sogm;

__global__ __launch_bounds__(256) void k_flight_reset(FlightCtl fl, int n_words, int *verdict, long long *acc, int *log_words,
                                                      long long n_log_words) {
  const long long i0 = (long long)blockIdx.x * blockDim.x + threadIdx.x, step = (long long)gridDim.x * blockDim.x;
  for (long long i = i0; i < n_words; i += step)
    if (i != FL_UW_TAIL && i != FL_UW_HEAD) fl.hdr[i] = 0;
  if (i0 == 0) fl.hdr[FL_UW_HEAD] = fl.hdr[FL_UW_TAIL];
  for (long long i = i0; i < n_log_words; i += step) log_words[i] = 0;
  for (long long i = i0; i < fl.n_agents; i += step) verdict[i] = 0;
  for (long long i = i0; i < 8ll * fl.n_agents; i += step) acc[i] = 0;
  for (long long i = i0; i < 16; i += step) fl.prof[i] = 0ull;
  for (long long i = i0; i < 8 * FL_WG_LOG; i += step) fl.wg_start[i] = 0;
}
__global__ __launch_bounds__(256) void k_flight_seed(FlightCtl fl) {
  const int a = blockIdx.x * blockDim.x + threadIdx.x;
  if (a < fl.n_agents) {
    fl.tick_of[a] = fl.first_tick;
    fl.m_ring[a]  = ring_encode(a, fl.ring_mask + 1, a);
    fl.ts[(size_t)a * FL_TS + 7] = wall_clock64();
  }
  if (a == 0) fl.hdr[FL_M_READY] = fl.n_agents;
  for (int i = a; i < FlightBlock::parked_words(fl.n_agents); i += (int)(gridDim.x * blockDim.x)) fl.parked[i] = -1;
}
__global__ void k_flight_xwait(FlightCtl fl, int i) {
  if (threadIdx.x != 0) return;
  wait_at_least<WaitUntimed, false>(&fl.hdr[FL_ERR], &fl.tick_done[i], fl.n_agents);
}
__global__ void k_flight_xsignal(FlightCtl fl, int i) {
  if (threadIdx.x != 0) return;
  __threadfence();
  __hip_atomic_store(&fl.xready[i], fl.epoch, __ATOMIC_RELEASE, __HIP_MEMORY_SCOPE_AGENT);
  if (i + fl.lag < fl.n_ticks) fl_gate_release(fl, i + fl.lag);
}
__global__ void k_flight_report(const int *__restrict__ hdr, int *__restrict__ host_words) {
  const int e = hdr[FL_ERR];
  if (e != 0) {
    host_words[0] = 100 + e;
    host_words[1] = host_words[1] + 1;
  }
}

static int flight_setup(sogm_planner *p) {
  sogm_ctx *c = p->map;
  const int A = c->n_agents;
  if (p->d_fl) return SOGM_OK;
  if (A >= (1 << 16)) return SOGM_ERR_INVALID_ARG;
  int n_cu = 256;
  (void)hipDeviceGetAttribute(&n_cu, hipDeviceAttributeMultiprocessorCount, c->device);
  const bool      masks = c->tune_i(SOGM_TUNE_FLIGHT_MASKS) != 0;
  const int       n_se = c->tune_i(SOGM_TUNE_FLIGHT_ENGINES), se0 = c->tune_i(SOGM_TUNE_FLIGHT_ENGINE_FIRST);
  const int       units[3] = {c->tune_i(SOGM_TUNE_FLIGHT_QP_UNITS), c->tune_i(SOGM_TUNE_FLIGHT_SEARCH_UNITS),
                              c->tune_i(SOGM_TUNE_FLIGHT_MAP_UNITS)};
  FlightPartition part;
  switch (flight_partition(n_cu, n_se, se0, c->tune_i(SOGM_TUNE_FLIGHT_EXCHANGE_UNITS), units[0], units[1], units[2], masks,
                           c->tune_i(SOGM_TUNE_FLIGHT_LIGHT_PER_CU), c->tune_i(SOGM_TUNE_FLIGHT_MAP_PER_CU), &part)) {
    case FLIGHT_PARTITION_OK: break;
    case FLIGHT_PARTITION_NO_REST:
      sogm::set_error_text("sogm_flight_run: flight_qp_units + flight_search_units + flight_map_units must leave a unit for the corridor kernel");
      return SOGM_ERR_INVALID_ARG;
    case FLIGHT_PARTITION_UNPLACEABLE: {
      char text[256];
      std::snprintf(text, sizeof(text), "sogm_flight_run: flight_qp_units = %d, flight_search_units = %d, flight_map_units = %d is a split "
                    "that cannot be placed on %d shader engines (every kernel needs the same share of each engine it touches)",
                    units[0], units[1], units[2], se0 + n_se > 4 ? 4 - se0 : n_se);
      sogm::set_error_text(text);
      return SOGM_ERR_INVALID_ARG;
    }
  }
  sogm::Resources::Setup setup(p->res);
  SOGM_HIP_CHECK(p->res.device(&p->d_fl, sizeof(int) * FlightBlock::words(A), true));
  FlightBlock::carve(p->d_fl, A, &p->fl, &p->fl_xready);
  p->fl.n_agents  = A;
  SOGM_HIP_CHECK(p->res.device(&p->fl.ts, sizeof(long long) * FL_TS * (size_t)A, true));
  SOGM_HIP_CHECK(p->res.device(&p->fl.acc, sizeof(long long) * 8 * (size_t)A, true));
  SOGM_HIP_CHECK(p->res.device(&p->fl.ts_log, sizeof(long long) * FL_TS * (size_t)A * FLIGHT_MAX_TICKS));
  SOGM_HIP_CHECK(p->res.device(&p->fl.wg_start, sizeof(long long) * 8 * FL_WG_LOG));
  SOGM_HIP_CHECK(p->res.device(&p->fl.prof, sizeof(unsigned long long) * 16, true));
  SOGM_HIP_CHECK(p->res.device(&p->d_fl_worlds, sizeof(FlightWorld) * FLIGHT_MAX_TICKS));
  SOGM_HIP_CHECK(p->res.pinned(&p->h_fl_worlds, sizeof(FlightWorld) * FLIGHT_MAX_TICKS, hipHostMallocDefault));
  SOGM_HIP_CHECK(p->res.device(&p->d_fl_pva, sizeof(double) * 9 * (size_t)A));
  SOGM_HIP_CHECK(p->res.device(&p->d_fl_tstart, sizeof(double) * (size_t)A));
  SOGM_HIP_CHECK(p->res.device(&p->d_fl_now, sizeof(double) * (size_t)A));
  SOGM_HIP_CHECK(p->res.device(&p->d_fl_due, sizeof(int32_t) * (size_t)A));
  SOGM_HIP_CHECK(p->res.device(&p->d_fl_reached, sizeof(int32_t) * (size_t)A));
  SOGM_HIP_CHECK(p->res.device(&p->d_fl_posnow, sizeof(double) * 3 * (size_t)A));
  for (int k = 0; k < 4; ++k) {
    if (masks)
      SOGM_HIP_CHECK(p->res.stream_masked(&p->fl_stream[k], (uint32_t)((n_cu + 31) / 32), part.mask[k]));
    else
      SOGM_HIP_CHECK(p->res.stream(&p->fl_stream[k]));
    SOGM_HIP_CHECK(p->res.event(&p->fl_ev_done[k]));
    p->fl_cus[k] = part.cus[k];
    p->fl_wgs[k] = part.wgs[k];
  }
  SOGM_HIP_CHECK(p->res.event(&p->fl_ev_in));
  SOGM_HIP_CHECK(hipStreamSynchronize(nullptr));
  return setup.done();
}

#ifdef SOGM_FLIGHT_TRACE
#include <chrono>
#define FL_TRACE(what) std::fprintf(stderr, "FLTRACE %p %s %.3f ms\n", (void *)p, what, std::chrono::duration<double, std::milli>(std::chrono::steady_clock::now().time_since_epoch()).count())
#else
#define FL_TRACE(what) (void)0
#endif
static int flight_check_call(const sogm_planner *p, const SogmFlight *f, bool *xchg_out, int *lag_out) {
  if (!p || !f || f->n_ticks < 1 || f->n_ticks > FLIGHT_MAX_TICKS || f->first_tick < 0 || !f->worlds || !f->goals ||
      !f->drone_ids || !f->hover_inout || !f->own_inout || !f->tables || !f->log_records || !f->log_ok || !(f->period > 0))
    return SOGM_ERR_INVALID_ARG;
  sogm_ctx *c = p->map;
  const int A = c->n_agents;
  if (f->n_total < A || f->agent0 < 0 || f->agent0 + A > f->n_total) return SOGM_ERR_INVALID_ARG;
  if (p->fl_fsm_on && f->n_total != A) {
    sogm::set_error_text("sogm_flight_run: under sogm_planner_set_flight_fsm a flight has n_total == n_agents (one process owns every row)");
    return SOGM_ERR_INVALID_ARG;
  }
  const bool xchg = f->n_total != A && f->nccl_comm != nullptr;
  const int lag = c->tune_i(SOGM_TUNE_FLIGHT_NEIGHBOUR_LAG) == 1 ? 1 : 2;
  if (f->n_total != A && !xchg && f->n_ticks > lag) {
    sogm::set_error_text("sogm_flight_run: with n_total > n_agents (other ranks' rows in the tables) and no nccl_comm a call flies at most two ticks");
    return SOGM_ERR_INVALID_ARG;
  }
  if (!p->flow || !c->sparse || !c->d_body || c->n_body <= 0) return SOGM_ERR_STATE;
  *xchg_out = xchg;
  *lag_out  = lag;
  return SOGM_OK;
}
static int flight_check_capacity(const sogm_ctx *c, size_t *agent_bytes_out) {
  const int A = c->n_agents;
  {
    const long long per_tick = (long long)A * (1 + c->tune_i(SOGM_TUNE_FLIGHT_RESET) + c->tune_i(SOGM_TUNE_FLIGHT_BITS) +
                                               c->tune_i(SOGM_TUNE_FLIGHT_MARKS) + c->tune_i(SOGM_TUNE_FLIGHT_SPLAT));
    if (2 * per_tick > FL_WQ_SLOTS || 2ll * A * (SOGM_MAX_PIECES + 1) > FL_WQ_SLOTS) {
      sogm::set_error_text("sogm_flight_run: agents x tickets per tick exceed the work queue (lower flight_marks / flight_bits)");
      return SOGM_ERR_CAPACITY;
    }
  }
  const size_t agent_bytes = (size_t)c->spec.T * (size_t)c->geom.V * c->cell_bytes();
  if (agent_bytes % 32 != 0 || (reinterpret_cast<uintptr_t>(c->d_grid) & 31) != 0) {
    sogm::set_error_text("sogm_flight_run: agent grids must be 32-byte aligned (V * T * cell bytes a multiple of 32)");
    return SOGM_ERR_INVALID_ARG;
  }
  *agent_bytes_out = agent_bytes;
  return SOGM_OK;
}
static int flight_stage_frames(sogm_planner *p, const SogmFlight *f, hipStream_t main, sogm::FlightMapDev &md) {
  sogm_ctx *c = p->map;
  int max_blocks = 0;
  for (int i = 0; i < f->n_ticks; ++i) {
    const SogmWorld &w = f->worlds[i];
    if (!w.cloud_xyz || !w.block_bounds || w.n_points < 0 || w.block_points < 64 || w.block_points > 4096 ||
        w.n_blocks != (w.n_points + w.block_points - 1) / w.block_points || w.n_cyl < 0 || (w.n_cyl > 0 && !w.cylinders))
      return SOGM_ERR_INVALID_ARG;
    if (w.n_blocks > max_blocks) max_blocks = w.n_blocks;
    p->h_fl_worlds[i] = FlightWorld{w.cloud_xyz, w.block_bounds, w.cylinders, w.n_points, w.n_blocks, w.block_points, w.n_cyl};
  }
  {
    SogmWorld big = f->worlds[0];
    big.n_blocks  = max_blocks;
    big.n_points  = max_blocks * big.block_points;
    if (int rc = sogm::world_blocks(c, &big, &md.cb)) return rc;
    md.cb.n_blocks = max_blocks;
  }
  const int slot = c->pool.current();
  if (!c->pool.loggable(slot)) {
    if (int rc = sogm::launch_clear(c, main, c->d_grid, false)) return rc;
    if (!c->pool.loggable(slot)) {
      sogm::set_error_text("sogm_flight_run: the current grid has no mark log (sogm_set_sparse_reset)");
      return SOGM_ERR_STATE;
    }
  }
  return sogm::map_target(c, slot, false, nullptr, &md.tgt);
}
static void flight_args(const sogm_planner *p, const SogmFlight *f, bool xchg, int lag, size_t agent_bytes, FlightCtl &fl,
                        sogm::FlightMapDev &md) {
  const sogm_ctx *c = p->map;
  const int       A = c->n_agents;
  fl             = p->fl;
  fl.xready      = xchg ? p->fl_xready : nullptr;
  fl.lag         = lag;
  fl.n_ticks     = f->n_ticks;
  fl.first_tick  = f->first_tick;
  md.worlds      = p->d_fl_worlds;
  md.ov          = {.rec = nullptr, .n_rec = 0, .ego_ids = f->drone_ids, .body = c->d_body, .n_body = c->n_body};
  md.tables      = f->tables;
  md.n_total     = f->n_total;
  md.tick        = {.own = f->own_inout, .hover = f->hover_inout, .now = p->d_fl_now, .t_start = p->d_fl_tstart,
                    .pva = p->d_fl_pva, .start_offset = f->replan_start_offset};
  md.t0          = f->t0;
  md.period      = f->period;
  md.n_reset     = c->tune_i(SOGM_TUNE_FLIGHT_RESET);
  md.n_bits      = c->tune_i(SOGM_TUNE_FLIGHT_BITS);
  md.n_marks     = c->tune_i(SOGM_TUNE_FLIGHT_MARKS);
  md.n_splat     = c->tune_i(SOGM_TUNE_FLIGHT_SPLAT);
  md.n_head_wgs  = c->tune_i(SOGM_TUNE_FLIGHT_HEADS) < p->fl_wgs[3] / 2 ? c->tune_i(SOGM_TUNE_FLIGHT_HEADS)
                                                                        : (p->fl_wgs[3] / 2 > 0 ? p->fl_wgs[3] / 2 : 1);
  fl.n_urgent    = c->tune_i(SOGM_TUNE_FLIGHT_URGENT) < A ? c->tune_i(SOGM_TUNE_FLIGHT_URGENT) : A - 1;
  if (fl.n_urgent < 0) fl.n_urgent = 0;
  md.n_uhead_wgs = 0;
  md.n_uwork_wgs = 0;
  {
    const int fine = c->tune_i(SOGM_TUNE_FLIGHT_URGENT_FINE);
    auto      cut  = [fine](int n, int hi) { return n * fine < hi ? n * fine : hi; };
    md.un_reset = cut(md.n_reset, 256);
    md.un_bits  = cut(md.n_bits, 256) > 2 * md.n_bits ? 2 * md.n_bits : cut(md.n_bits, 256);
    md.un_marks = cut(md.n_marks, 256);
    md.un_splat = cut(md.n_splat, 64);
  }
  fl.gate_pace_ticks = (int)(c->tune[SOGM_TUNE_FLIGHT_GATE_PACE_US] * 100.0);
  fl.epoch    = p->fl_epoch;
  fl.n_splat  = md.n_splat;
  fl.un_splat = md.un_splat;
  if (fl.n_urgent > 0) {
    const int workers = p->fl_wgs[3] - md.n_head_wgs;
    md.n_uhead_wgs = md.n_head_wgs >= 8 ? 4 : md.n_head_wgs / 2;
    md.n_uwork_wgs = c->tune_i(SOGM_TUNE_FLIGHT_URGENT_WAVES) < workers ? c->tune_i(SOGM_TUNE_FLIGHT_URGENT_WAVES) : workers;
    if (md.n_uhead_wgs < 1 || md.n_uwork_wgs < 1) fl.n_urgent = 0, md.n_uhead_wgs = 0, md.n_uwork_wgs = 0;
  }
  md.n_admit     = c->tune_i(SOGM_TUNE_FLIGHT_ADMIT);
  md.pace_ticks  = (int)(c->tune[SOGM_TUNE_FLIGHT_PACE_US] * 100.0);
  md.agent_bytes = agent_bytes;
  md.reset_stat  = c->d_reset_stat;
  sogm::FlightFsmDev fd{};
  if (p->fl_fsm_on) {
    const SogmFlightFsm &u = p->fl_fsm;
    fd = sogm::FlightFsmDev{.prm = u.prm, .check_duration = u.check_duration, .state = u.state_inout, .goals = f->goals,
                            .due = p->d_fl_due, .reached = p->d_fl_reached, .pos_now = p->d_fl_posnow,
                            .log_state = u.log_state, .log_due = u.log_due, .log_safe = u.log_safe,
                            .log_reached = u.log_reached, .log_pub = u.log_pub, .log_hover_start = u.log_hover_start,
                            .log_own = u.log_own};
  }
  md.fsm = fd;
}
static int flight_reset_and_seed(sogm_planner *p, const SogmFlight *f, const FlightCtl &fl, hipStream_t main) {
  const int A = p->map->n_agents;
  SOGM_HIP_CHECK(hipMemcpyAsync(p->d_fl_worlds, p->h_fl_worlds, sizeof(FlightWorld) * (size_t)f->n_ticks, hipMemcpyHostToDevice, main));
  const int       n_words = FlightBlock::reset_words(A);
  const long long n_log  = (long long)f->n_ticks * A * (long long)(sizeof(SogmTrajRecord) / sizeof(int));
  hipLaunchKernelGGL(k_flight_reset, dim3(256), dim3(256), 0, main, fl, n_words, p->aw.verdict, p->fl.acc,
                     reinterpret_cast<int *>(f->log_records), n_log);
  SOGM_HIP_CHECK(hipGetLastError());
  SOGM_HIP_CHECK(hipMemsetAsync(f->log_ok, 0, sizeof(int32_t) * (size_t)f->n_ticks * A, main));
  hipLaunchKernelGGL(k_flight_seed, dim3((A + 255) / 256), dim3(256), 0, main, fl);
  SOGM_HIP_CHECK(hipGetLastError());
  SOGM_HIP_CHECK(hipEventRecord(p->fl_ev_in, main));
  for (int k = 0; k < 4; ++k) SOGM_HIP_CHECK(hipStreamWaitEvent(p->fl_stream[k], p->fl_ev_in, 0));
  FL_TRACE("waits queued");
  return SOGM_OK;
}
static int flight_launch(sogm_planner *p, const SogmFlight *f, const FlightCtl &fl, const sogm::FlightMapDev &md) {
  sogm_ctx                 *c  = p->map;
  const MapView             mv = view_of(c);
  const sogm::FlightFsmDev &fd = md.fsm;
  const int spec = c->tune_i(SOGM_TUNE_FLIGHT_SPEC) != 0 ? 1 : 0;
  hipError_t e = sogm::launch_flight_qp(p->pp, p->qs, p->qw, p->qc, fl, p->fl_wgs[0], qp_io(p, p->d_fl_pva), p->fl_stream[0]);
  if (e == hipSuccess) {
    sogm::SearchIO sio = search_io(p, p->d_fl_pva, f->goals, p->d_fl_tstart);
    sio.due            = fd.state ? fd.due : nullptr;
    e = sogm::launch_flight_search(mv, p->ap, p->pp.corridor_tau, astar_ws(p), fl, p->fl_wgs[1], sio, spec, p->fl_stream[1]);
  }
  if (int rc = launched("sogm_flight_run: launch", e)) {
    (void)hipDeviceSynchronize();
    return rc;
  }
  FL_TRACE("qp + search launched");
  sogm::FlightLightDev ld{};
  ld.cor = corridor_io(p, p->d_fl_pva, p->d_fl_tstart);
  ld.fin = sogm::FinishArgs{.corridor_tau = p->pp.corridor_tau, .ret = p->d_ret, .npoly = p->d_npoly,
                            .status = p->d_status, .cpts = p->d_cpts, .n_swarm = f->n_total, .swarm_ego = f->drone_ids,
                            .swarm_now = p->d_fl_now, .t_start = p->d_fl_tstart, .drone_ids = f->drone_ids,
                            .out_safe = p->d_safe, .counters = p->cw.counters, .pub_own = f->own_inout,
                            .due = fd.state ? fd.due : nullptr};
  ld.fsm         = fd;
  ld.tables      = f->tables;
  ld.n_total     = f->n_total;
  ld.agent0      = f->agent0;
  ld.log_records = f->log_records;
  ld.log_ok      = f->log_ok;
  e = sogm::launch_flight_light(mv, p->pp, p->cw, fl, ld, p->fl_wgs[2], p->fl_stream[2]);
  if (e == hipSuccess) e = sogm::launch_flight_map(c->geom, fl, md, p->fl_wgs[3], p->fl_stream[3]);
  if (int rc = launched("sogm_flight_run: launch", e)) {
    (void)hipDeviceSynchronize();
    return rc;
  }
  FL_TRACE("light + map launched");
  return SOGM_OK;
}
static int flight_exchange(sogm_planner *p, const SogmFlight *f, const FlightCtl &fl, hipStream_t main) {
  sogm_ctx *c = p->map;
  const int A = c->n_agents;
  hipStream_t xs = nullptr;
  if (int rc = sogm::exchange_stream(c, &xs)) return rc;
  SOGM_HIP_CHECK(hipStreamWaitEvent(xs, p->fl_ev_in, 0));
  int rc_x = SOGM_OK;
  for (int i = 0; i < f->n_ticks; ++i) {
    const int       k   = f->first_tick + i;
    SogmTrajRecord *tab = f->tables + (size_t)(k & 3) * f->n_total;
    hipLaunchKernelGGL(k_flight_xwait, dim3(1), dim3(64), 0, xs, fl, i);
    if (rc_x == SOGM_OK)
      rc_x = sogm::exchange_allgather_raw(c, f->nccl_comm, tab + f->agent0, tab, sizeof(SogmTrajRecord) * (size_t)A);
    hipLaunchKernelGGL(k_flight_xsignal, dim3(1), dim3(64), 0, xs, fl, i);
    if (i == 0) FL_TRACE("first collective queued");
  }
  FL_TRACE("collectives queued");
  SOGM_HIP_CHECK(hipGetLastError());
  if (int rc = sogm::exchange_mark_pending(c)) return rc;
  if (int rc = sogm::join_exchange(c, main)) return rc;
  if (rc_x != SOGM_OK) {
    (void)hipDeviceSynchronize();
    return rc_x;
  }
  return SOGM_OK;
}
static int flight_fan_in(sogm_planner *p, const SogmFlight *f, hipStream_t main) {
  sogm_ctx *c = p->map;
  for (int k = 0; k < 4; ++k) {
    SOGM_HIP_CHECK(hipEventRecord(p->fl_ev_done[k], p->fl_stream[k]));
    SOGM_HIP_CHECK(hipStreamWaitEvent(main, p->fl_ev_done[k], 0));
  }
  hipLaunchKernelGGL(k_flight_report, dim3(1), dim3(1), 0, main, (const int *)p->fl.hdr, p->h_flow_fail);
  SOGM_HIP_CHECK(hipGetLastError());
  c->updated             = 1;
  c->pool.current_rebuilt();
  c->records_final_valid = 0;
  c->n_stamps += f->n_ticks;
  return SOGM_OK;
}

extern "C" {
int sogm_flight_run(sogm_planner *p, const SogmFlight *f, void *stream) {
  bool xchg = false;
  int  lag  = 2;
  if (int rc = flight_check_call(p, f, &xchg, &lag)) return rc;
  sogm_ctx *c = p->map;
  SOGM_HIP_CHECK(hipSetDevice(c->device));
  hipStream_t main = (hipStream_t)stream;
  if (int rc = sogm::join_update(c, main)) return rc;
  if (int rc = sogm::join_prestamp(c, main)) return rc;
  if (int rc = sogm::join_exchange(c, main)) return rc;
  if (int rc = flight_setup(p)) return rc;
  size_t agent_bytes = 0;
  if (int rc = flight_check_capacity(c, &agent_bytes)) return rc;
  sogm::FlightMapDev md{};
  if (int rc = flight_stage_frames(p, f, main, md)) return rc;
  p->fl_epoch = p->fl_epoch >= 0x7ffffff0 ? 1 : p->fl_epoch + 1;
  FlightCtl fl;
  flight_args(p, f, xchg, lag, agent_bytes, fl, md);
  if (int rc = flight_reset_and_seed(p, f, fl, main)) return rc;
  if (int rc = flight_launch(p, f, fl, md)) return rc;
  if (xchg)
    if (int rc = flight_exchange(p, f, fl, main)) return rc;
  return flight_fan_in(p, f, main);
}

}
__global__ void k_flight_touch(int *word) {
  if (threadIdx.x == 0 && word) atomicAdd(word, 0);
}
extern "C" {
int sogm_flight_prepare(sogm_planner *p, int max_cloud_points) {
  if (!p || max_cloud_points < 0) return SOGM_ERR_INVALID_ARG;
  SOGM_HIP_CHECK(hipSetDevice(p->map->device));
  if (int rc = flight_setup(p)) return rc;
  {
    SogmWorld big{};
    big.block_points = 256;
    big.n_points     = max_cloud_points;
    big.n_blocks     = (max_cloud_points + 255) / 256;
    sogm::CloudBlocks cb{};
    if (int rc = sogm::world_blocks(p->map, &big, &cb)) return rc;
    if (p->map->sparse) {
      sogm_ctx       *c = p->map;
      sogm::MapTarget tgt{};
      if (int rc = sogm::map_target(c, c->pool.current(), false, nullptr, &tgt)) return rc;
      if (!c->pool.loggable(c->pool.current()))
        if (int rc = sogm::launch_clear(c, nullptr, c->d_grid, false)) return rc;
    }
  }
  hipStream_t xs = nullptr;
  if (int rc = sogm::exchange_stream(p->map, &xs)) return rc;
  for (int k = 0; k < 4; ++k) hipLaunchKernelGGL(k_flight_touch, dim3(1), dim3(64), 0, p->fl_stream[k], (int *)nullptr);
  hipLaunchKernelGGL(k_flight_touch, dim3(1), dim3(64), 0, xs, (int *)nullptr);
  SOGM_HIP_CHECK(hipGetLastError());
  SOGM_HIP_CHECK(hipDeviceSynchronize());
  return SOGM_OK;
}

int sogm_debug_flight_times(sogm_planner *p, long long *out_host, int n_ticks) {
  if (!p || !p->d_fl || !out_host || n_ticks < 1 || n_ticks > FLIGHT_MAX_TICKS) return SOGM_ERR_INVALID_ARG;
  SOGM_HIP_CHECK(hipDeviceSynchronize());
  SOGM_HIP_CHECK(hipMemcpy(out_host, p->fl.ts_log, sizeof(long long) * FL_TS * (size_t)p->map->n_agents * n_ticks, hipMemcpyDeviceToHost));
  return SOGM_OK;
}

int sogm_debug_flight_dump(sogm_planner *p, int32_t *out_words, int cap_words, long long *out_ts) {
  if (!p || !p->d_fl || !out_words) return SOGM_ERR_INVALID_ARG;
  const int A = p->map->n_agents;
  const struct { const int *src; int n; } part[] = {{p->fl.tick_done, FLIGHT_MAX_TICKS}, {p->fl.parked_n, FLIGHT_MAX_TICKS},
                                                    {p->fl.tick_of, A}, {p->fl.seg_done, A}, {p->fl.stage, A}, {p->fl.urgent, A}};
  int need = FL_COUNTERS;
  for (const auto &s : part) need += s.n;
  if (cap_words < need) return SOGM_ERR_INVALID_ARG;
  SOGM_HIP_CHECK(hipSetDevice(p->map->device));
  SOGM_HIP_CHECK(hipDeviceSynchronize());
  for (int i = 0; i < FL_COUNTERS; ++i)
    SOGM_HIP_CHECK(hipMemcpy(out_words + i, p->fl.hdr + (size_t)i * FL_STRIDE, sizeof(int), hipMemcpyDeviceToHost));
  int32_t *o = out_words + FL_COUNTERS;
  for (const auto &s : part) {
    SOGM_HIP_CHECK(hipMemcpy(o, s.src, sizeof(int) * (size_t)s.n, hipMemcpyDeviceToHost));
    o += s.n;
  }
  if (out_ts) SOGM_HIP_CHECK(hipMemcpy(out_ts, p->fl.ts, sizeof(long long) * FL_TS * (size_t)A, hipMemcpyDeviceToHost));
  return SOGM_OK;
}

int sogm_debug_flight_wg_starts(sogm_planner *p, long long *out_host, int32_t *out_wgs_host) {
  if (!p || !p->d_fl || !out_host) return SOGM_ERR_INVALID_ARG;
  SOGM_HIP_CHECK(hipSetDevice(p->map->device));
  SOGM_HIP_CHECK(hipDeviceSynchronize());
  SOGM_HIP_CHECK(hipMemcpy(out_host, p->fl.wg_start, sizeof(long long) * 8 * FL_WG_LOG, hipMemcpyDeviceToHost));
  if (out_wgs_host)
    for (int k = 0; k < 4; ++k) out_wgs_host[k] = p->fl_wgs[k];
  return SOGM_OK;
}

int sogm_flight_stats(sogm_planner *p, double *out_ms, int32_t *out_hdr) {
  if (!p || !p->d_fl) return SOGM_ERR_INVALID_ARG;
  SOGM_HIP_CHECK(hipSetDevice(p->map->device));
  SOGM_HIP_CHECK(hipDeviceSynchronize());
  const int A = p->map->n_agents;
  if (out_ms) {
    long long *tmp = new (std::nothrow) long long[8 * (size_t)A];
    if (!tmp) return SOGM_ERR_INVALID_ARG;
    const hipError_t e = hipMemcpy(tmp, p->fl.acc, sizeof(long long) * 8 * (size_t)A, hipMemcpyDeviceToHost);
    for (int i = 0; i < 8 * A; ++i) out_ms[i] = (i % 8) == 7 ? (double)tmp[i] : (double)tmp[i] / 1.0e5;
    delete[] tmp;
    SOGM_HIP_CHECK(e);
  }
  if (out_hdr) {
    int *tmp = new (std::nothrow) int[FL_HDR];
    if (!tmp) return SOGM_ERR_INVALID_ARG;
    const hipError_t e = hipMemcpy(tmp, p->fl.hdr, sizeof(int) * FL_HDR, hipMemcpyDeviceToHost);
    for (int i = 0; i < 32; ++i) out_hdr[i] = i < 15 ? tmp[(size_t)i * FL_STRIDE] : 0;
    delete[] tmp;
    SOGM_HIP_CHECK(e);
    {
      long long *ws = new (std::nothrow) long long[4 * FL_WG_LOG];
      if (!ws) return SOGM_ERR_INVALID_ARG;
      const hipError_t e2 = hipMemcpy(ws, p->fl.wg_start, sizeof(long long) * 4 * FL_WG_LOG, hipMemcpyDeviceToHost);
      int late = 0;
      for (int k = 0; k < 4; ++k) {
        long long first = 0;
        for (int b = 0; b < p->fl_wgs[k] && b < FL_WG_LOG; ++b) {
          const long long v = ws[(size_t)k * FL_WG_LOG + b];
          if (v > 0 && (first == 0 || v < first)) first = v;
        }
        for (int b = 0; b < p->fl_wgs[k] && b < FL_WG_LOG; ++b) {
          const long long v = ws[(size_t)k * FL_WG_LOG + b];
          if (v == 0 || v - first > 100000) ++late;
        }
      }
      delete[] ws;
      SOGM_HIP_CHECK(e2);
      out_hdr[15] = late;
    }
    unsigned long long prof[16];
    SOGM_HIP_CHECK(hipMemcpy(prof, p->fl.prof, sizeof(prof), hipMemcpyDeviceToHost));
    for (int i = 0; i < 16; ++i) out_hdr[16 + i] = (int32_t)(i < 9 ? prof[i] / 1000ull : prof[i]);
  }
  return SOGM_OK;
}
}
```

pred-occ-planner_amd/csrc/sogm_planner.hip:

```cpp
#include <hip/hip_runtime.h>

#include <cmath>
#include <cstdio>
#include <cstdlib>
#include <cstring>
#include <new>

#include "sogm_planner.hpp"

using namespace sogm;

static void min_jerk_block(double *QM ) {
  auto diff = [](int rows, double scale, double *out, int cols) {
    for (int i = 0; i < rows * cols; ++i) out[i] = 0.0;
    for (int i = 0; i < rows / 3; ++i)
      for (int d = 0; d < 3; ++d) {
        out[(i * 3 + d) * cols + i * 3 + d]       = -scale;
        out[(i * 3 + d) * cols + (i + 1) * 3 + d] = scale;
      }
  };
  double p2v[12 * 15], v2a[9 * 12], a2j[6 * 9], p2a[9 * 15], p2j[6 * 15], W[6 * 6], T[6 * 15];
  diff(12, 4, p2v, 15);
  diff(9, 3, v2a, 12);
  diff(6, 2, a2j, 9);
  auto mul = [](const double *A, const double *B, double *C, int r, int k, int c) {
    for (int i = 0; i < r; ++i)
      for (int j = 0; j < c; ++j) {
        double s = 0;
        for (int q = 0; q < k; ++q) s += A[i * k + q] * B[q * c + j];
        C[i * c + j] = s;
      }
  };
  mul(v2a, p2v, p2a, 9, 12, 15);
  mul(a2j, p2a, p2j, 6, 9, 15);
  for (int i = 0; i < 36; ++i) W[i] = 0.0;
  for (int d = 0; d < 3; ++d) {
    W[d * 6 + d]           = 1.0 / 3;
    W[d * 6 + 3 + d]       = 1.0 / 6;
    W[(3 + d) * 6 + d]     = 1.0 / 6;
    W[(3 + d) * 6 + 3 + d] = 1.0 / 3;
  }
  mul(W, p2j, T, 6, 6, 15);
  for (int i = 0; i < 15; ++i)
    for (int j = 0; j < 15; ++j) {
      double s = 0;
      for (int q = 0; q < 6; ++q) s += p2j[q * 15 + i] * T[q * 15 + j];
      QM[i * 15 + j] = s;
    }
}

__global__ void k_pack_records(int A, FinishArgs f, int agent0) {
  const int a = blockIdx.x * blockDim.x + threadIdx.x + agent0;
  if (a >= A) return;
  const int32_t *ret = f.ret, *npoly = f.npoly, *status = f.status;
  const int32_t *safe = f.swarm ? f.out_safe : nullptr;
  if (unsigned long long *counters = (f.due && f.due[a] == 0) ? nullptr : f.counters) {
    int k = SOGM_CNT_REPLAN_OK;
    if (ret[a] == 0) k = SOGM_CNT_FAIL_SEARCH;
    else if (npoly[a] <= 0) k = SOGM_CNT_FAIL_CORRIDOR;
    else if (!(status[a] == 1 || status[a] == 2)) k = SOGM_CNT_FAIL_QP;
    else if (safe != nullptr && safe[a] == 0) k = SOGM_CNT_FAIL_UNSAFE;
    atomicAdd(&counters[k], 1ull);
  }
  SogmTrajRecord &r = f.out[a];
  const bool good = ret[a] != 0 && npoly[a] > 0 && (status[a] == 1 || status[a] == 2) &&
                    (safe == nullptr || safe[a] != 0);
  r.drone_id        = f.drone_ids[a];
  r.time_start      = f.t_start[a];
  r.n_pieces        = good ? npoly[a] : 0;
  for (int i = 0; i < SOGM_MAX_PIECES; ++i) r.duration[i] = (good && i < npoly[a]) ? f.corridor_tau : 0.0;
  for (int i = 0; i < SOGM_MAX_PIECES * 15; ++i)
    r.cpts[i] = (good && i < npoly[a] * 15) ? f.cpts[(size_t)a * SOGM_MAX_PIECES * 15 + i] : 0.0;
  f.out_ok[a] = good ? 1 : 0;
  if (f.pub_own) {
    if (good) f.pub_own[a] = r;
    if (f.pub_table) f.pub_table[a] = f.pub_own[a];
  }
}

__global__ void k_flow_report(const int *__restrict__ hdr, int *__restrict__ host_words, int *__restrict__ epoch_word,
                              long long *__restrict__ tick_clock) {
  if (tick_clock) tick_clock[1] = wall_clock64();
  if (epoch_word) *epoch_word = 0;
  const int e = hdr[FLOW_ERR];
  if (e != 0) {
    host_words[0] = e;
    host_words[1] = host_words[1] + 1;
  }
}

extern "C" {

static int planner_acquire(sogm_planner *p) {
  sogm_ctx                *map = p->map;
  const SogmPlannerParams *pp  = &p->pp;
  const int                A   = map->n_agents;
  sogm::Resources::Setup   setup(p->res);
  SOGM_HIP_CHECK(p->res.device(&p->aw.pool, p->aw.pool_stride * A * 2));
  SOGM_HIP_CHECK(p->res.device(&p->aw.hkeys, 8 * (size_t)p->aw.hash_cap * A * 2));
  SOGM_HIP_CHECK(p->res.device(&p->aw.verdict, sizeof(int) * A));
  SOGM_HIP_CHECK(p->res.device(&p->aw.dbg, sizeof(long long) * 8 * A, true));
  SOGM_HIP_CHECK(p->res.device(&p->d_ret, sizeof(int32_t) * A));
  SOGM_HIP_CHECK(p->res.device(&p->d_route_len, sizeof(int32_t) * A));
  SOGM_HIP_CHECK(p->res.device(&p->d_stats, sizeof(int32_t) * 4 * A));
  SOGM_HIP_CHECK(p->res.device(&p->d_route, sizeof(double) * 6 * p->route_cap * A));
  const size_t slots = (size_t)A * SOGM_MAX_PIECES, cap = (size_t)pp->pc_capacity;
  SOGM_HIP_CHECK(p->res.device(&p->cw.pc, sizeof(double) * slots * cap * 3));
  SOGM_HIP_CHECK(p->res.device(&p->cw.fpc, sizeof(double) * slots * cap * 3));
  SOGM_HIP_CHECK(p->res.device(&p->cw.tang, sizeof(double) * slots * cap * 4));
  SOGM_HIP_CHECK(p->res.device(&p->cw.distr, sizeof(double) * slots * cap));
  SOGM_HIP_CHECK(p->res.device(&p->cw.polys, sizeof(double) * slots * pp->max_faces * 4));
  SOGM_HIP_CHECK(p->res.device(&p->cw.seg_nfaces, sizeof(int32_t) * slots));
  SOGM_HIP_CHECK(p->res.device(&p->cw.seg_state, sizeof(int32_t) * slots));
  SOGM_HIP_CHECK(p->res.device(&p->cw.seg_npts, sizeof(int32_t) * slots));
  SOGM_HIP_CHECK(p->res.device(&p->cw.seg_dbg, sizeof(long long) * 16 * slots, true));
  SOGM_HIP_CHECK(p->res.device(&p->cw.counters, sizeof(unsigned long long) * SOGM_CNT_N, true));
  p->qw.scratch_stride = qp_scratch_bytes_per_agent(pp->max_faces);
  p->qw.dyn_lds_bytes  = qp_kernel_setup();
  SOGM_HIP_CHECK(p->res.device(&p->qw.scratch, p->qw.scratch_stride * (size_t)A));
  SOGM_HIP_CHECK(p->res.device(&p->qw.k1_scratch, qp_k1_scratch_bytes_per_agent() * (size_t)A));
  SOGM_HIP_CHECK(p->res.device(&p->qw.dbg, sizeof(long long) * 16 * (size_t)A, true));
  SOGM_HIP_CHECK(p->res.device(&p->d_polys, sizeof(double) * slots * pp->max_faces * 4));
  SOGM_HIP_CHECK(p->res.device(&p->d_goal, sizeof(double) * 6 * A));
  SOGM_HIP_CHECK(p->res.device(&p->d_cpts, sizeof(double) * slots * 15));
  SOGM_HIP_CHECK(p->res.device(&p->d_nfaces, sizeof(int32_t) * slots));
  SOGM_HIP_CHECK(p->res.device(&p->d_npoly, sizeof(int32_t) * A));
  SOGM_HIP_CHECK(p->res.device(&p->d_status, sizeof(int32_t) * A));
  SOGM_HIP_CHECK(p->res.device(&p->d_iters, sizeof(int32_t) * A));
  SOGM_HIP_CHECK(p->res.device(&p->d_safe, sizeof(int32_t) * A));
  for (int g = 0; g < p->n_groups; ++g) {
    SOGM_HIP_CHECK(p->res.event(&p->ev_corr[g]));
    SOGM_HIP_CHECK(p->res.event(&p->ev_pts[g]));
    SOGM_HIP_CHECK(p->res.event(&p->ev_done[g]));
  }
  SOGM_HIP_CHECK(p->res.event(&p->ev_in));
  SOGM_HIP_CHECK(p->res.device(&p->d_flow, sizeof(int) * FlowBlock::words(A), true));
  FlowBlock::carve(p->d_flow, A, &p->fc);
  SOGM_HIP_CHECK(p->res.event(&p->ev_pdone));
  SOGM_HIP_CHECK(p->res.device(&p->d_flow_ts, sizeof(long long) * 12 * (size_t)A, true));
  p->fc.ts = p->d_flow_ts;
  for (int k = 0; k < 4; ++k) {
    SOGM_HIP_CHECK(p->res.stream(&p->fstream[k]));
    SOGM_HIP_CHECK(p->res.event(&p->ev_fdone[k]));
  }
  SOGM_HIP_CHECK(p->res.event(&p->ev_gate));
  SOGM_HIP_CHECK(p->res.device(&p->d_epoch, sizeof(int), true));
  SOGM_HIP_CHECK(p->res.pinned(&p->h_flow_fail, sizeof(int) * 2, hipHostMallocMapped));
  p->h_flow_fail[0] = p->h_flow_fail[1] = 0;
  SOGM_HIP_CHECK(hipStreamSynchronize(nullptr));
  return setup.done();
}

int sogm_planner_create(sogm_ctx *map, const SogmAstarParams *astar, const SogmPlannerParams *pp,
                        const SogmQpSettings *qp, sogm_planner **out) {
  if (!map || !astar || !pp || !qp || !out) return SOGM_ERR_INVALID_ARG;
  if (!(pp->opt_max_vel > 0 && pp->opt_max_vel < 1e20) || !(pp->opt_max_acc > 0 && pp->opt_max_acc < 1e20))
    return SOGM_ERR_INVALID_ARG;
  if (astar->allocate_num < 2 || astar->allocate_num > astar_pool_max() || astar->check_num < 1 || !(astar->resolution > 0) ||
      !(astar->time_resolution > 0))
    return SOGM_ERR_INVALID_ARG;
  if (pp->max_faces < 6 || pp->max_faces > 64 || pp->pc_capacity < 1 || pp->pc_capacity > 16384 || pp->firi_iterations < 1)
    return SOGM_ERR_INVALID_ARG;
  SOGM_HIP_CHECK(hipSetDevice(map->device));
  sogm_planner *p = new (std::nothrow) sogm_planner();
  if (!p) return SOGM_ERR_INVALID_ARG;
  p->map = map;
  p->ap  = *astar;
  p->pp  = *pp;
  p->ap.shot_ignores_time = pp->fake_planner ? 0 : 1;
  p->qs  = *qp;
  const int A = map->n_agents;
  int       hc = 1;
  while (hc < 2 * astar->allocate_num) hc <<= 1;
  p->aw.hash_cap    = hc;
  p->aw.pool_stride = astar_node_bytes() * (size_t)astar->allocate_num;
  p->route_cap      = 64;
  min_jerk_block(p->qc.QM);
  {
    int ng = map->tune_i(SOGM_TUNE_GROUPS);
    if (ng < 1) ng = 1;
    if (ng > SOGM_MAX_GROUPS) ng = SOGM_MAX_GROUPS;
    p->n_groups = A < ng ? A : ng;
  }
  p->sel_first   = 0;
  p->sel_count   = A;
  p->search_mode = 0;
  {
    p->spec_astar = map->tune_i(SOGM_TUNE_SPEC_ASTAR) != 0;
    if (p->spec_astar && 2 * A > sogm::astar_resident_workgroups(map->device)) p->spec_astar = 0;
  }
  {
    const char *ef = getenv("SOGM_FLOW");
    p->flow        = ef ? atoi(ef) != 0 : 1;
  }
  if (int rc = planner_acquire(p)) {
    delete p;
    return rc;
  }
  if (p->flow) {
    map->clear_gate        = p->fc.hdr + FLOW_Q_READY_N;
    map->clear_gate_err    = p->fc.hdr + FLOW_ERR;
    map->clear_gate_target = A;
    {
      const double f = map->tune[SOGM_TUNE_CLEAR_GATE_FRAC];
      if (f > 0.0 && f < 1.0) map->clear_gate_target = (int)(f * A + 0.5) < 1 ? 1 : (int)(f * A + 0.5);
    }
    map->clear_epoch_word  = p->d_epoch;
  }
  *out = p;
  return SOGM_OK;
}
void sogm_planner_destroy(sogm_planner *p) {
  if (!p) return;
  if (p->map) (void)hipSetDevice(p->map->device);
  if (p->map && p->map->ps_fail_host == p->h_flow_fail) p->map->ps_fail_host = nullptr;
  if (p->map && p->map->pdone_pending && p->map->ev_pdone == p->ev_pdone) {
    (void)hipDeviceSynchronize();
    p->map->pdone_pending = 0;
    p->map->ps_stage = p->map->ps_err = nullptr;
  }
  if (p->map && p->d_epoch && p->map->clear_epoch_word == p->d_epoch) {
    (void)hipDeviceSynchronize();
    p->map->clear_gate = p->map->clear_gate_err = p->map->clear_epoch_word = nullptr;
  }
  p->res.release_all();
  delete p;
}

int sogm_astar_search(sogm_planner *p, const double *start_pva, const double *goal,
                      const double *t_start, int32_t *out_ret, double *out_route,
                      int32_t *out_route_len, int route_cap, int32_t *out_stats,
                      int32_t *out_trace, int trace_cap, void *stream) {
  if (!p || !start_pva || !goal || !t_start || !out_ret || !out_route || !out_route_len ||
      !out_stats || route_cap < 2)
    return SOGM_ERR_INVALID_ARG;
  if (!p->map->updated) return SOGM_ERR_STATE;
  SOGM_HIP_CHECK(hipSetDevice(p->map->device));
  hipStream_t st = (hipStream_t)stream;
  if (int rc0 = sogm::join_update(p->map, st)) return rc0;
  const sogm::SearchIO io{.start_pva = start_pva, .goal = goal, .t_start = t_start, .out_ret = out_ret,
                          .out_route = out_route, .out_route_len = out_route_len, .route_cap = route_cap,
                          .out_stats = out_stats};
  prof_begin(p->map, SOGM_PROF_ASTAR, st);
  const hipError_t e = launch_astar(view_of(p->map), p->ap, p->pp.corridor_tau, astar_ws(p), p->sel_count, io, out_trace,
                                    out_trace ? trace_cap : 0, st, p->sel_first, nullptr, p->search_mode);
  prof_end(p->map, SOGM_PROF_ASTAR, st);
  return launched("k_astar", e);
}
int sogm_corridor_generate(sogm_planner *p, const double *start_pva, const double *t_start,
                           const double *route, const int32_t *route_len, int route_cap,
                           double *out_polys, int32_t *out_nfaces, int32_t *out_npoly,
                           double *out_goal, void *stream) {
  if (!p || !start_pva || !t_start || !route || !route_len || !out_polys || !out_nfaces ||
      !out_npoly || !out_goal || route_cap < 2)
    return SOGM_ERR_INVALID_ARG;
  if (!p->map->updated) return SOGM_ERR_STATE;
  SOGM_HIP_CHECK(hipSetDevice(p->map->device));
  hipStream_t st = (hipStream_t)stream;
  if (int rc0 = sogm::join_update(p->map, st)) return rc0;
  const sogm::CorridorIO io{.start_pva = start_pva, .t_start = t_start, .route = route, .route_len = route_len,
                            .route_cap = route_cap, .out_polys = out_polys, .out_nfaces = out_nfaces,
                            .out_npoly = out_npoly, .out_goal = out_goal};
  prof_begin(p->map, SOGM_PROF_CORRIDOR, st);
  const hipError_t e = launch_corridor(view_of(p->map), p->pp, p->cw, p->sel_count, io, st, p->sel_first);
  prof_end(p->map, SOGM_PROF_CORRIDOR, st);
  return launched("k_corridor", e);
}
int sogm_debug_astar_stats(sogm_planner *p, long long *out_host) {
  if (!p || !out_host) return SOGM_ERR_INVALID_ARG;
  SOGM_HIP_CHECK(hipDeviceSynchronize());
  SOGM_HIP_CHECK(hipMemcpy(out_host, p->aw.dbg, sizeof(long long) * 8 * (size_t)p->map->n_agents,
                           hipMemcpyDeviceToHost));
  return SOGM_OK;
}

int sogm_debug_astar_nodes(sogm_planner *p, int agent, void *out_host, int n) {
  if (!p || !out_host || agent < 0 || agent >= p->map->n_agents || n < 0) return SOGM_ERR_INVALID_ARG;
  SOGM_HIP_CHECK(hipDeviceSynchronize());
  SOGM_HIP_CHECK(hipMemcpy(out_host, p->aw.pool + (size_t)agent * p->aw.pool_stride, (size_t)n * sogm::astar_node_bytes(),
                           hipMemcpyDeviceToHost));
  return SOGM_OK;
}

int sogm_debug_qp_stats(sogm_planner *p, long long *out_host) {
  if (!p || !out_host) return SOGM_ERR_INVALID_ARG;
  SOGM_HIP_CHECK(hipDeviceSynchronize());
  SOGM_HIP_CHECK(hipMemcpy(out_host, p->qw.dbg, sizeof(long long) * 16 * (size_t)p->map->n_agents, hipMemcpyDeviceToHost));
  return SOGM_OK;
}

int sogm_debug_corridor_stats(sogm_planner *p, long long *out_host) {
  if (!p || !out_host) return SOGM_ERR_INVALID_ARG;
  SOGM_HIP_CHECK(hipDeviceSynchronize());
  SOGM_HIP_CHECK(hipMemcpy(out_host, p->cw.seg_dbg,
                           sizeof(long long) * 16 * (size_t)p->map->n_agents * SOGM_MAX_PIECES,
                           hipMemcpyDeviceToHost));
  return SOGM_OK;
}

int sogm_bezier_qp_solve(sogm_planner *p, const double *start_pva, const double *goal_pv,
                         const double *polys, const int32_t *nfaces, const int32_t *npoly,
                         double *out_cpts, int32_t *out_status, int32_t *out_iters, void *stream) {
  if (!p || !start_pva || !goal_pv || !polys || !nfaces || !npoly || !out_cpts || !out_status ||
      !out_iters)
    return SOGM_ERR_INVALID_ARG;
  SOGM_HIP_CHECK(hipSetDevice(p->map->device));
  hipStream_t st = (hipStream_t)stream;
  const sogm::QpIO io{.start_pva = start_pva, .goal_pv = goal_pv, .polys = polys, .nfaces = nfaces, .npoly = npoly,
                      .out_cpts = out_cpts, .out_status = out_status, .out_iters = out_iters};
  prof_begin(p->map, SOGM_PROF_QP, st);
  sogm::QpWorkspace qw0 = p->qw;
  qw0.ablate            = p->map->tune_i(SOGM_TUNE_QP_ABLATE);
  const hipError_t e    = launch_qp(p->pp, p->qs, qw0, p->qc, p->sel_count, io, st, p->sel_first);
  prof_end(p->map, SOGM_PROF_QP, st);
  return launched("k_qp", e);
}
int sogm_bezier_qp_solve_timed(sogm_planner *p, const double *start_pva, const double *end_pva,
                               const double *time_alloc, double max_vel, double max_acc, const double *polys,
                               const int32_t *nfaces, const int32_t *npoly, double *out_cpts, int32_t *out_status,
                               int32_t *out_iters, void *stream) {
  if (!p || !start_pva || !end_pva || !time_alloc || !polys || !nfaces || !npoly || !out_cpts || !out_status ||
      !out_iters || !(max_vel > 0 && max_vel < 1e20) || !(max_acc > 0 && max_acc < 1e20))
    return SOGM_ERR_INVALID_ARG;
  SOGM_HIP_CHECK(hipSetDevice(p->map->device));
  hipStream_t       st = (hipStream_t)stream;
  SogmPlannerParams pp = p->pp;
  pp.opt_max_vel       = max_vel;
  pp.opt_max_acc       = max_acc;
  sogm::QpWorkspace qw = p->qw;
  qw.t_alloc           = time_alloc;
  qw.goal_stride       = 9;
  const sogm::QpIO io{.start_pva = start_pva, .goal_pv = end_pva, .polys = polys, .nfaces = nfaces, .npoly = npoly,
                      .out_cpts = out_cpts, .out_status = out_status, .out_iters = out_iters};
  prof_begin(p->map, SOGM_PROF_QP, st);
  const hipError_t e = launch_qp(pp, p->qs, qw, p->qc, p->sel_count, io, st, p->sel_first);
  prof_end(p->map, SOGM_PROF_QP, st);
  return launched("k_qp", e);
}
int sogm_safe_after_opt(sogm_planner *p, const double *cpts, const int32_t *npoly,
                        const SogmTrajRecord *records, int n_records, const int32_t *ego_ids,
                        const double *t_now, int32_t *out_safe, void *stream) {
  if (!p || !cpts || !npoly || !ego_ids || !t_now || !out_safe || n_records < 0 || (n_records > 0 && !records))
    return SOGM_ERR_INVALID_ARG;
  SOGM_HIP_CHECK(hipSetDevice(p->map->device));
  if (int rc = sogm::join_exchange(p->map, (hipStream_t)stream)) return rc;
  return launched("sogm_safe_after_opt", sogm::launch_deconflict(p->sel_count, cpts, npoly, records, n_records, ego_ids,
                                                                t_now, out_safe, (hipStream_t)stream, p->sel_first));
}

int sogm_planner_select_agents(sogm_planner *p, int first, int count) {
  if (!p || first < 0 || count < 1 || first + count > p->map->n_agents) return SOGM_ERR_INVALID_ARG;
  p->sel_first = first;
  p->sel_count = count;
  return SOGM_OK;
}
int sogm_planner_set_search_mode(sogm_planner *p, int mode) {
  if (!p || mode < 0 || (mode & ~(3 | 4 | 16)) != 0 || (mode & 3) == 3) return SOGM_ERR_INVALID_ARG;
  p->search_mode = mode;
  return SOGM_OK;
}

int sogm_debug_flow_peek(sogm_planner *p, int *out_host, int n) {
  if (!p || !out_host || n < 0) return SOGM_ERR_INVALID_ARG;
  if (!p->peek) SOGM_HIP_CHECK(p->res.stream(&p->peek));
  hipStream_t peek = p->peek;
  const int nf = FlowBlock(p->map->n_agents).gen;
  SOGM_HIP_CHECK(hipMemcpyAsync(out_host, p->d_flow, sizeof(int) * (size_t)(n < nf ? n : nf), hipMemcpyDeviceToHost, peek));
  if (n > nf)
    SOGM_HIP_CHECK(hipMemcpyAsync(out_host + nf, p->d_safe, sizeof(int) * (size_t)(n - nf), hipMemcpyDeviceToHost, peek));
  SOGM_HIP_CHECK(hipStreamSynchronize(peek));
  return SOGM_OK;
}

int sogm_debug_flow_times(sogm_planner *p, long long *out_host) {
  if (!p || !out_host) return SOGM_ERR_INVALID_ARG;
  SOGM_HIP_CHECK(hipDeviceSynchronize());
  SOGM_HIP_CHECK(hipMemcpy(out_host, p->d_flow_ts, sizeof(long long) * 8 * (size_t)p->map->n_agents, hipMemcpyDeviceToHost));
  return SOGM_OK;
}

int sogm_debug_planner_buffer(sogm_planner *p, int which, void *out_host, size_t bytes) {
  if (!p || !out_host) return SOGM_ERR_INVALID_ARG;
  const size_t A = (size_t)p->map->n_agents, slots = A * SOGM_MAX_PIECES;
  const void  *src[11] = {p->d_polys, p->d_nfaces, p->d_npoly, p->d_goal, p->d_route, p->d_route_len, p->d_cpts, p->d_iters,
                          p->d_status, p->d_ret, p->d_stats};
  const size_t len[11] = {sizeof(double) * slots * p->pp.max_faces * 4, sizeof(int32_t) * slots, sizeof(int32_t) * A,
                          sizeof(double) * 6 * A, sizeof(double) * 6 * p->route_cap * A, sizeof(int32_t) * A,
                          sizeof(double) * slots * 15, sizeof(int32_t) * A, sizeof(int32_t) * A, sizeof(int32_t) * A,
                          sizeof(int32_t) * 4 * A};
  if (which < 0 || which > 10 || bytes > len[which]) return SOGM_ERR_INVALID_ARG;
  SOGM_HIP_CHECK(hipDeviceSynchronize());
  SOGM_HIP_CHECK(hipMemcpy(out_host, src[which], bytes, hipMemcpyDeviceToHost));
  return SOGM_OK;
}

int sogm_debug_prestamp_times(sogm_planner *p, long long *out_host) {
  if (!p || !out_host) return SOGM_ERR_INVALID_ARG;
  SOGM_HIP_CHECK(hipDeviceSynchronize());
  SOGM_HIP_CHECK(hipMemcpy(out_host, p->d_flow_ts + 8 * (size_t)p->map->n_agents, sizeof(long long) * 4 * (size_t)p->map->n_agents,
                           hipMemcpyDeviceToHost));
  return SOGM_OK;
}

int sogm_planner_flow_error(sogm_planner *p) {
  if (!p) return SOGM_ERR_INVALID_ARG;
  int hdr[FLOW_HDR];
  SOGM_HIP_CHECK(hipSetDevice(p->map->device));
  SOGM_HIP_CHECK(hipDeviceSynchronize());
  SOGM_HIP_CHECK(hipMemcpy(hdr, p->d_flow, sizeof(hdr), hipMemcpyDeviceToHost));
  return hdr[FLOW_ERR];
}

int sogm_planner_flow_failures(sogm_planner *p, int32_t out[2]) {
  if (!p || !out) return SOGM_ERR_INVALID_ARG;
  volatile int *h = p->h_flow_fail;
  out[0]          = h ? h[0] : 0;
  out[1]          = h ? h[1] : 0;
  return SOGM_OK;
}

int sogm_planner_counters(sogm_planner *p, int64_t *out_host, int reset) {
  if (!p || !out_host) return SOGM_ERR_INVALID_ARG;
  SOGM_HIP_CHECK(hipSetDevice(p->map->device));
  SOGM_HIP_CHECK(hipDeviceSynchronize());
  SOGM_HIP_CHECK(hipMemcpy(out_host, p->cw.counters, sizeof(int64_t) * SOGM_CNT_N, hipMemcpyDeviceToHost));
  if (reset) SOGM_HIP_CHECK(hipMemset(p->cw.counters, 0, sizeof(int64_t) * SOGM_CNT_N));
  return SOGM_OK;
}

int sogm_planner_set_publish(sogm_planner *p, SogmTrajRecord *own_records, SogmTrajRecord *next_table) {
  if (!p || (next_table && !own_records)) return SOGM_ERR_INVALID_ARG;
  p->pub_own   = own_records;
  p->pub_table = next_table;
  return SOGM_OK;
}

int sogm_planner_set_prestamp(sogm_planner *p, const SogmPrestamp *ps) {
  if (!p) return SOGM_ERR_INVALID_ARG;
  if (!ps) {
    p->ps_on = 0;
    return SOGM_OK;
  }
  if (!ps->hover_inout || !ps->out_now || !ps->out_t_start || !ps->out_pva) return SOGM_ERR_INVALID_ARG;
  const SogmWorld *w = ps->world;
  if (w) {
    if (!w->cloud_xyz || !w->block_bounds || w->n_points < 0 || w->block_points < 64 || w->block_points > 4096 ||
        w->n_blocks != (w->n_points + w->block_points - 1) / w->block_points || w->n_cyl < 0 || (w->n_cyl > 0 && !w->cylinders))
      return SOGM_ERR_INVALID_ARG;
  } else if (!ps->cloud_xyz || !ps->cloud_range || ps->n_cyl < 0 || (ps->n_cyl > 0 && !ps->cylinders)) {
    return SOGM_ERR_INVALID_ARG;
  }
  p->ps = sogm::PrestampDev{
      .frame      = {.cloud       = w ? w->cloud_xyz : ps->cloud_xyz,
                     .cloud_range = w ? nullptr : ps->cloud_range,
                     .cb          = {},
                     .cyl         = w ? w->cylinders : ps->cylinders,
                     .n_cyl       = w ? w->n_cyl : ps->n_cyl},
      .tick       = {.own = nullptr, .hover = ps->hover_inout, .now = ps->out_now, .t_start = ps->out_t_start,
                     .pva = ps->out_pva, .start_offset = ps->replan_start_offset},
      .stamp      = ps->next_stamp,
      .poses_host = ps->out_poses};
  p->ps_world_on = w ? 1 : 0;
  if (w) {
    p->ps_world = *w;
    sogm::CloudBlocks sized{};
    if (int rc = sogm::world_blocks(p->map, w, &sized)) return rc;
  }
  p->ps_on = 1;
  return SOGM_OK;
}

int sogm_planner_set_due(sogm_planner *p, const int32_t *due_dev_or_null) {
  if (!p) return SOGM_ERR_INVALID_ARG;
  p->due = due_dev_or_null;
  return SOGM_OK;
}

int sogm_planner_set_flight_fsm(sogm_planner *p, const SogmFlightFsm *fsm) {
  if (!p) return SOGM_ERR_INVALID_ARG;
  if (!fsm) {
    p->fl_fsm_on = 0;
    p->fl_fsm    = SogmFlightFsm{};
    return SOGM_OK;
  }
  if (!fsm->state_inout) {
    sogm::set_error_text("sogm_planner_set_flight_fsm: state_inout is NULL");
    return SOGM_ERR_INVALID_ARG;
  }
  const double v[5] = {fsm->prm.replan_duration, fsm->prm.replan_start_time, fsm->prm.goal_tolerance,
                       fsm->prm.new_plan_interval, fsm->check_duration};
  for (double x : v)
    if (!std::isfinite(x) || x < 0.0) {
      sogm::set_error_text("sogm_planner_set_flight_fsm: the parameters must be finite and not negative");
      return SOGM_ERR_INVALID_ARG;
    }
  if (fsm->prm.replan_max_failures < 0) {
    sogm::set_error_text("sogm_planner_set_flight_fsm: replan_max_failures must not be negative");
    return SOGM_ERR_INVALID_ARG;
  }
  p->fl_fsm    = *fsm;
  p->fl_fsm_on = 1;
  return SOGM_OK;
}

int sogm_planner_set_swarm(sogm_planner *p, const SogmTrajRecord *records, int n_records,
                           const int32_t *ego_ids, const double *t_now) {
  if (!p || n_records < 0 || (records && (!ego_ids || !t_now))) return SOGM_ERR_INVALID_ARG;
  p->swarm     = records;
  p->n_swarm   = records ? n_records : 0;
  p->swarm_ego = ego_ids;
  p->swarm_now = t_now;
  return SOGM_OK;
}

__global__ __launch_bounds__(1024) void k_flow_reset(int *hdr, int n_hdr, int *ready, int n_ready, int *verdict,
                                                     int n_verdict, int *epoch_word, int epoch, int *gen_word, int gen) {
  const int i0 = (int)threadIdx.x, step = (int)blockDim.x;
  for (int i = i0; i < n_hdr; i += step) hdr[i] = 0;
  for (int i = i0; i < n_ready; i += step) ready[i] = -1;
  if (verdict)
    for (int i = i0; i < n_verdict; i += step) verdict[i] = 0;
  __threadfence();
  __syncthreads();
  if (threadIdx.x == 0) {
    if (epoch_word) __hip_atomic_store(epoch_word, epoch, __ATOMIC_RELEASE, __HIP_MEMORY_SCOPE_AGENT);
    __hip_atomic_store(gen_word, gen, __ATOMIC_RELEASE, __HIP_MEMORY_SCOPE_AGENT);
  }
}

__global__ void k_update_rank(const long long *__restrict__ ts, int *__restrict__ order, int n, int by) {
  for (int a = threadIdx.x; a < n; a += blockDim.x) {
    if (!by) {
      order[a] = a;
      continue;
    }
    const long long da = ts[a * 8 + 6] - ts[a * 8 + 0];
    int             r  = 0;
    for (int b = 0; b < n; ++b) {
      const long long db = ts[b * 8 + 6] - ts[b * 8 + 0];
      r += (db > da || (db == da && b < a)) ? 1 : 0;
    }
    order[r] = a;
  }
}

struct FlowCall {
  const double   *start_pva, *goal, *t_start;
  const int32_t  *drone_ids;
  SogmTrajRecord *out_records;
  int32_t        *out_ok;
  hipStream_t     main;
  bool            spec;
  int            *gen_word;
  int             n_cu, wg_q, wg_f;
  bool            prestamp;
  hipStream_t     pst;
};

static int flow_reset(sogm_planner *p, FlowCall &call) {
  sogm_ctx         *c    = p->map;
  const hipStream_t main = call.main, sC = p->fstream[1];
  const int         A    = c->n_agents;
  const bool        spec = call.spec;
  SOGM_HIP_CHECK(hipStreamWaitEvent(sC, p->ev_pdone, 0));
  if (c->pool.current_prestamped()) {
    SOGM_HIP_CHECK(hipEventRecord(p->ev_gate, main));
    SOGM_HIP_CHECK(hipStreamWaitEvent(sC, p->ev_gate, 0));
  }
  const FlowBlock fb(A);
  int *gen_word = p->d_flow + fb.gen;
  ++p->reset_epoch;
  hipLaunchKernelGGL(k_flow_reset, dim3(1), dim3(1024), 0, sC, p->d_flow, fb.zero_words(), p->d_flow + fb.fill_first(),
                     fb.fill_words(), spec ? p->aw.verdict : nullptr, A,
                     c->overlap >= 2 && c->clear_gate ? c->clear_epoch_word : nullptr,
                     c->overlap >= 2 && c->clear_gate ? sogm::next_clear_epoch(c) : 0, gen_word, p->reset_epoch);
  SOGM_HIP_CHECK(hipGetLastError());
  call.gen_word = gen_word;
  return SOGM_OK;
}
static int flow_launch_chain(sogm_planner *p, FlowCall &call) {
  sogm_ctx         *c    = p->map;
  const hipStream_t main = call.main, sA = main, sC = p->fstream[1], sQ = p->fstream[2], sF = p->fstream[3];
  const int         A    = c->n_agents;
  const MapView     mv   = view_of(c);
  const bool        spec = call.spec;
  int              *gen_word = call.gen_word;
  const double     *start_pva = call.start_pva, *goal = call.goal, *t_start = call.t_start;
  SogmTrajRecord   *out_records = call.out_records;
  int32_t          *out_ok      = call.out_ok;
  if (c->exchange_pending)
    for (int k = 1; k < 4; ++k) SOGM_HIP_CHECK(hipStreamWaitEvent(p->fstream[k], c->ev_xdone, 0));
  prof_begin(c, SOGM_PROF_ASTAR, sA);
  sogm::FlowCtl fca = p->fc;
  fca.map_ready = c->update_pending ? c->d_map_ready : nullptr;
  fca.map_epoch = c->map_epoch;
  fca.reset_gen   = gen_word;
  fca.reset_epoch = p->reset_epoch;
  fca.out_ok      = out_ok;
  fca.out_records = reinterpret_cast<int *>(out_records);
  fca.rec_words   = (int)(sizeof(SogmTrajRecord) / sizeof(int));
  if (int rc = launched("sogm_replan: k_astar",
                        launch_astar(mv, p->ap, p->pp.corridor_tau, astar_ws(p), A, search_io(p, start_pva, goal, t_start),
                                     nullptr, 0, sA, 0, &fca, spec ? 8 : 0)))
    return rc;
  prof_end(c, SOGM_PROF_ASTAR, sA);
  SOGM_HIP_CHECK(hipEventRecord(p->ev_in, main));
  if (int rc = launched("sogm_replan: k_flow_gate", sogm::launch_flow_gate(p->fc, spec ? 2 * A : A, sC))) return rc;
  SOGM_HIP_CHECK(hipEventRecord(p->ev_gate, sC));
  SOGM_HIP_CHECK(hipStreamWaitEvent(sQ, p->ev_gate, 0));
  SOGM_HIP_CHECK(hipStreamWaitEvent(sF, p->ev_gate, 0));
  int n_cu = 256;
  (void)hipDeviceGetAttribute(&n_cu, hipDeviceAttributeMultiprocessorCount, c->device);
  int wg_c = 4 * n_cu;
  if (wg_c > A * SOGM_MAX_PIECES) wg_c = A * SOGM_MAX_PIECES;
  int wg_q = n_cu / 2;
  if (c->tune_i(SOGM_TUNE_QP_WGS) > 0) wg_q = c->tune_i(SOGM_TUNE_QP_WGS);
  if (wg_q > A) wg_q = A;
  if (wg_q < 1) wg_q = 1;
  int wg_f = A < 64 ? A : 64;
  call.n_cu = n_cu, call.wg_q = wg_q, call.wg_f = wg_f;
  prof_begin(c, SOGM_PROF_CORRIDOR, sC);
  if (int rc = launched("sogm_replan: k_corridor_flow",
                        sogm::launch_corridor_flow(mv, p->pp, p->cw, p->fc, A, wg_c, corridor_io(p, start_pva, t_start), sC)))
    return rc;
  prof_end(c, SOGM_PROF_CORRIDOR, sC);
  if (c->update_pending) SOGM_HIP_CHECK(hipStreamWaitEvent(sQ, c->ev_udone, 0));
  prof_begin(c, SOGM_PROF_QP, sQ);
  if (int rc = launched("sogm_replan: k_qp_flow",
                        sogm::launch_qp_flow(p->pp, p->qs, p->qw, p->qc, p->fc, A, wg_q, qp_io(p, start_pva), sQ)))
    return rc;
  prof_end(c, SOGM_PROF_QP, sQ);
  c->gate_open_valid = 0;
  c->gate_frac_valid = 0;
  {
    const double f      = c->tune[SOGM_TUNE_PRESTAMP_GATE_FRAC];
    c->gate_frac_agents = f > 0.0 && f < 1.0 ? ((int)(f * A + 0.5) < 1 ? 1 : (int)(f * A + 0.5)) : 0;
  }
  if (c->overlap >= 2) {
    int rc = sogm::queue_spare_clears(c, p->ev_in);
    if (rc) return rc;
  }
  return SOGM_OK;
}
static int flow_finish(sogm_planner *p, FlowCall &call) {
  sogm_ctx         *c  = p->map;
  const hipStream_t sF = p->fstream[3];
  const int         A  = c->n_agents;
  sogm::FlowCtl fcf = p->fc;
  const bool prestamp = p->ps_on && c->sparse && c->overlap >= 2 && c->pool.front_ready() >= 0 && p->pub_own && c->clear_gate;
  if (!prestamp) fcf.p_ready = nullptr;
  call.prestamp = prestamp;
  return launched("sogm_replan: k_finish_flow",
                  sogm::launch_finish_flow(fcf, A, call.wg_f, finish_args(p, call.t_start, call.drone_ids, call.out_records, call.out_ok), sF));
}
static sogm::PrestampDev prestamp_args(const sogm_planner *p) {
  const sogm_ctx   *c = p->map;
  const int         A = c->n_agents;
  sogm::PrestampDev d = p->ps;
  d.tick.own = p->pub_own;
  d.n_agents = A;
  {
    const double f = c->tune[SOGM_TUNE_PRESTAMP_GATE_FRAC];
    d.gate_agents  = f >= 1.0 ? A : f <= 0.0 ? 0 : (int)(f * A + 0.5);
  }
  const int nb = c->tune_i(SOGM_TUNE_PRESTAMP_BITS) > 0 ? c->tune_i(SOGM_TUNE_PRESTAMP_BITS) : 32;
  const int nm = c->tune_i(SOGM_TUNE_PRESTAMP_MARKS) > 0 ? c->tune_i(SOGM_TUNE_PRESTAMP_MARKS) : 64;
  d.n_bits       = nb;
  d.n_marks      = nm;
  d.n_late       = c->tune_i(SOGM_TUNE_PRESTAMP_LATE_AGENTS) < 0 ? 0 : c->tune_i(SOGM_TUNE_PRESTAMP_LATE_AGENTS);
  d.n_bits_late  = c->tune_i(SOGM_TUNE_PRESTAMP_LATE_BITS) > 0 ? c->tune_i(SOGM_TUNE_PRESTAMP_LATE_BITS) : nb;
  d.n_marks_late = c->tune_i(SOGM_TUNE_PRESTAMP_LATE_MARKS) > 0 ? c->tune_i(SOGM_TUNE_PRESTAMP_LATE_MARKS) : nm;
  return d;
}
static int flow_prestamp(sogm_planner *p, FlowCall &call) {
  sogm_ctx *c = p->map;
  const int A = c->n_agents;
  c->pool.clear_prestamp_target();
  const bool        own_stream = c->tune_i(SOGM_TUNE_PRESTAMP_STREAM) != 0 && c->pstream != nullptr;
  const hipStream_t pst        = own_stream ? c->pstream : c->side;
  call.pst = pst;
  if (call.prestamp) {
    const int nxt = c->pool.front_ready();
    sogm::PrestampDev d = prestamp_args(p);
    if (int rc = sogm::map_target(c, nxt, true, nullptr, &d.tgt)) return rc;
    if (p->ps_world_on)
      if (int rc = sogm::world_blocks(c, &p->ps_world, &d.frame.cb)) return rc;
    SOGM_HIP_CHECK(hipStreamWaitEvent(pst, p->ev_in, 0));
    if (own_stream) {
      SOGM_HIP_CHECK(hipStreamWaitEvent(pst, c->pool.cleared_event(nxt), 0));
      if (c->gate_frac_valid && d.gate_agents < A)
        SOGM_HIP_CHECK(hipStreamWaitEvent(pst, c->ev_gate_frac, 0));
      else if (c->gate_open_valid && d.gate_agents >= A)
        SOGM_HIP_CHECK(hipStreamWaitEvent(pst, c->ev_gate_open, 0));
    }
    int wg_p = 8 * call.n_cu;
    if (c->tune_i(SOGM_TUNE_PRESTAMP_WGS) > 0) wg_p = c->tune_i(SOGM_TUNE_PRESTAMP_WGS);
    if (int rc = launched("sogm_replan: k_prestamp_flow",
                          sogm::launch_prestamp_flow(c->geom, p->fc, d, wg_p, call.wg_q, call.wg_f < A ? call.wg_f : A, pst)))
      return rc;
    c->pool.set_prestamp_target(nxt);
    c->n_stamps++;
    c->ps_fail_host = p->h_flow_fail;
    c->ps_fail_seen = p->h_flow_fail ? p->h_flow_fail[1] : 0;
  }
  return SOGM_OK;
}
static int flow_fan_in(sogm_planner *p, const FlowCall &call) {
  sogm_ctx         *c    = p->map;
  const hipStream_t main = call.main, sC = p->fstream[1], pst = call.pst;
  const int         A    = c->n_agents;
  const int         retire     = c->tune_i(SOGM_TUNE_CLEAR_RETIRE_AT_END);
  auto report = [&](hipStream_t st) {
    hipLaunchKernelGGL(k_flow_report, dim3(1), dim3(1), 0, st, (const int *)p->d_flow, p->h_flow_fail,
                       retire ? p->d_epoch : (int *)nullptr, c->h_tick_clock);
    return hipGetLastError();
  };
  const bool report_on_sc = !c->pool.prestamp_pending();
  for (int k = 0; k < 4; ++k)
    if (k != 1) SOGM_HIP_CHECK(hipEventRecord(p->ev_fdone[k], p->fstream[k]));
  if (report_on_sc) {
    SOGM_HIP_CHECK(hipStreamWaitEvent(sC, p->ev_fdone[2], 0));
    SOGM_HIP_CHECK(hipStreamWaitEvent(sC, p->ev_fdone[3], 0));
    SOGM_HIP_CHECK(report(sC));
  }
  SOGM_HIP_CHECK(hipEventRecord(p->ev_fdone[1], sC));
  for (int k = 0; k < 4; ++k) SOGM_HIP_CHECK(hipStreamWaitEvent(main, p->ev_fdone[k], 0));
  if (int rc = sogm::join_update(c, main)) return rc;
  if (c->d_update_order && c->tune_i(SOGM_TUNE_UPDATE_FLOW) != 0) {
    hipLaunchKernelGGL(k_update_rank, dim3(1), dim3(256), 0, main, (const long long *)p->fc.ts, c->d_update_order, A,
                       c->tune_i(SOGM_TUNE_UPDATE_ORDER));
    SOGM_HIP_CHECK(hipGetLastError());
  }
  bool reported = report_on_sc;
  if (c->pool.prestamp_pending()) {
    for (int k = 1; k < 4; ++k) SOGM_HIP_CHECK(hipStreamWaitEvent(pst, p->ev_fdone[k], 0));
    SOGM_HIP_CHECK(report(pst));
    SOGM_HIP_CHECK(hipEventRecord(p->ev_pdone, pst));
    const int defer = c->tune_i(SOGM_TUNE_SPLAT_OVERLAP) != 0;
    if (defer) {
      c->ev_pdone      = p->ev_pdone;
      c->pdone_pending = 1;
      c->ps_stage      = p->fc.stage;
      c->ps_err        = &p->fc.hdr[FLOW_ERR];
    } else {
      SOGM_HIP_CHECK(hipStreamWaitEvent(main, p->ev_pdone, 0));
    }
    reported = true;
  }
  c->records_final_valid = 0;
  if (p->pub_own) {
    c->ev_records_final    = p->ev_fdone[3];
    c->records_final_ptr   = p->pub_own;
    c->records_final_valid = 1;
  }
  if (!reported) SOGM_HIP_CHECK(report(main));
  return SOGM_OK;
}

static int replan_flow(sogm_planner *p, const double *start_pva, const double *goal, const double *t_start,
                       const int32_t *drone_ids, SogmTrajRecord *out_records, int32_t *out_ok, void *stream) {
  FlowCall call{.start_pva = start_pva, .goal = goal, .t_start = t_start, .drone_ids = drone_ids, .out_records = out_records,
                .out_ok = out_ok, .main = (hipStream_t)stream, .spec = p->spec_astar != 0};
  if (p->swarm)
    if (int rc = sogm::join_exchange(p->map, call.main)) return rc;
  if (int rc = flow_reset(p, call)) return rc;
  if (int rc = flow_launch_chain(p, call)) return rc;
  if (int rc = flow_finish(p, call)) return rc;
  if (int rc = flow_prestamp(p, call)) return rc;
  return flow_fan_in(p, call);
}

static int replan_impl(sogm_planner *p, const double *start_pva, const double *goal,
                       const double *t_start, const int32_t *drone_ids, SogmTrajRecord *out_records,
                       int32_t *out_ok, void *stream) {
  sogm_ctx   *c    = p->map;
  hipStream_t main = (hipStream_t)stream;
  const int   A = c->n_agents, G = p->n_groups;
  const MapView mv = view_of(c);
  if (int rc = sogm::join_update(c, main)) return rc;
  for (int g = 0; g < G; ++g)
    if (!p->gstream[g]) SOGM_HIP_CHECK(p->res.stream(&p->gstream[g]));
  if (p->swarm)
    if (int rc = sogm::join_exchange(c, main)) return rc;
  SOGM_HIP_CHECK(hipEventRecord(p->ev_in, main));
  if (c->overlap >= 2) {
    int rc = sogm::queue_spare_clears(c, p->ev_in);
    if (rc) return rc;
  }
  for (int g = 0; g < G; ++g) {
    const int a0 = (int)((long long)A * g / G), a1 = (int)((long long)A * (g + 1) / G), n = a1 - a0;
    if (n <= 0) continue;
    hipStream_t st = p->gstream[g];
    SOGM_HIP_CHECK(hipStreamWaitEvent(st, p->ev_in, 0));
    hipError_t e = launch_astar(mv, p->ap, p->pp.corridor_tau, astar_ws(p), n, search_io(p, start_pva, goal, t_start),
                                nullptr, 0, st, a0);
    if (e == hipSuccess) e = launch_corridor(mv, p->pp, p->cw, n, corridor_io(p, start_pva, t_start), st, a0, p->ev_pts[g]);
    if (int rc = launched("sogm_replan launch", e)) return rc;
    SOGM_HIP_CHECK(hipEventRecord(p->ev_corr[g], st));
  }
  if (c->overlap == 1) {
    const size_t total = sogm::clear_vec4_total(c);
    size_t       head  = (size_t)28e9 / 16;
    if (head > total / 2) head = total / 2;
    for (int g = 0; g < G; ++g) SOGM_HIP_CHECK(hipStreamWaitEvent(c->side, p->ev_pts[g], 0));
    const int slot = c->pool.current();
    if (c->pool.loggable(slot)) {
      int rc = sogm::reset_slot(c, c->side, slot, c->d_grid, true);
      if (rc) return rc;
    } else {
      int rc = sogm::launch_clear(c, c->side, c->d_grid, true, 1, head);
      if (rc) return rc;
      for (int g = 0; g < G; ++g) SOGM_HIP_CHECK(hipStreamWaitEvent(c->side, p->ev_corr[g], 0));
      rc = sogm::launch_clear(c, c->side, c->d_grid, false, 2, head);
      if (rc) return rc;
    }
    SOGM_HIP_CHECK(hipEventRecord(c->ev_cleared, c->side));
    c->pool.cleared_in_place();
    c->updated = 0;
  }
  for (int g = 0; g < G; ++g) {
    const int a0 = (int)((long long)A * g / G), a1 = (int)((long long)A * (g + 1) / G), n = a1 - a0;
    if (n <= 0) continue;
    hipStream_t st = p->gstream[g];
    if (int rc = launched("sogm_replan launch_qp", launch_qp(p->pp, p->qs, p->qw, p->qc, n, qp_io(p, start_pva), st, a0)))
      return rc;
    if (p->swarm)
      if (int rc = launched("sogm_replan launch_deconflict",
                            sogm::launch_deconflict(n, p->d_cpts, p->d_npoly, p->swarm, p->n_swarm, p->swarm_ego,
                                                    p->swarm_now, p->d_safe, st, a0, p->cw.counters)))
        return rc;
    hipLaunchKernelGGL(k_pack_records, dim3((n + 63) / 64), dim3(64), 0, st, a1,
                       finish_args(p, t_start, drone_ids, out_records, out_ok), a0);
    SOGM_HIP_CHECK(hipGetLastError());
    SOGM_HIP_CHECK(hipEventRecord(p->ev_done[g], st));
    SOGM_HIP_CHECK(hipStreamWaitEvent(main, p->ev_done[g], 0));
  }
  return SOGM_OK;
}


int sogm_replan(sogm_planner *p, const double *start_pva, const double *goal,
                const double *t_start, const int32_t *drone_ids, SogmTrajRecord *out_records,
                int32_t *out_ok, void *stream) {
  if (!p || !start_pva || !goal || !t_start || !drone_ids || !out_records || !out_ok)
    return SOGM_ERR_INVALID_ARG;
  if (!p->map->updated) return SOGM_ERR_STATE;
  sogm_ctx *c = p->map;
  if (p->pub_table && p->swarm) {
    const char *a0 = (const char *)p->pub_table, *a1 = a0 + sizeof(SogmTrajRecord) * (size_t)c->n_agents;
    const char *b0 = (const char *)p->swarm, *b1 = b0 + sizeof(SogmTrajRecord) * (size_t)p->n_swarm;
    if (a0 < b1 && b0 < a1) {
      sogm::set_error_text("sogm_replan: sogm_planner_set_publish's next_table overlaps the table given to sogm_planner_set_swarm");
      return SOGM_ERR_INVALID_ARG;
    }
  }
  if (p->pub_own) {
    const char *a0 = (const char *)p->pub_own, *a1 = a0 + sizeof(SogmTrajRecord) * (size_t)c->n_agents;
    const char *b0 = (const char *)out_records, *b1 = b0 + sizeof(SogmTrajRecord) * (size_t)c->n_agents;
    if (a0 < b1 && b0 < a1) {
      sogm::set_error_text("sogm_replan: out_records overlaps sogm_planner_set_publish's own_records");
      return SOGM_ERR_INVALID_ARG;
    }
  }
  SOGM_HIP_CHECK(hipSetDevice(c->device));
  const bool use_flow = p->flow && c->overlap != 1;
  if (int jr = sogm::join_prestamp(c, (hipStream_t)stream)) return jr;
  const int  rc = use_flow ? replan_flow(p, start_pva, goal, t_start, drone_ids, out_records, out_ok, stream)
                           : replan_impl(p, start_pva, goal, t_start, drone_ids, out_records, out_ok, stream);
  if (rc != SOGM_OK) {
    (void)hipDeviceSynchronize();
    if (c->pool.precleared() && c->overlap == 1) c->updated = 0;
    if (c->overlap < 2) c->pool.forget_preclear();
  }
  return rc;
}
}
// ... 1 lines not shown
```

pred-occ-planner_amd/csrc/sogm_planner.hpp:

```cpp
#pragma once

#include "sogm_device.hpp"
#include "sogm_handover.hpp"

namespace sogm {

struct AstarWorkspace {
  char  *pool;
  size_t pool_stride;
  void  *hkeys;
  int    hash_cap;
  long long *dbg;
  int *verdict;
};
int astar_pool_max();

struct CorridorWorkspace {
  double  *pc;
  double  *fpc;
  double  *tang;
  double  *distr;
  double  *polys;
  int32_t *seg_nfaces;
  int32_t *seg_state;
  int32_t *seg_npts;
  long long *seg_dbg;
  unsigned long long *counters;
};

static_assert(SOGM_MAX_PIECES <= WK_MAX_SUB, "a search pushes one corridor descriptor per segment slot, sub = the slot");
struct FlightWorld {
  const float        *cloud, *bounds;
  const SogmCylinder *cyl;
  int                 n_points, n_blocks, block_points, n_cyl;
};
#define FL_WG_LOG 4096
#ifdef __HIPCC__
__device__ inline void fl_wg_started(const FlightCtl &fl, int kernel) {
  if (threadIdx.x == 0 && fl.wg_start && blockIdx.x < FL_WG_LOG) {
    fl.wg_start[(size_t)kernel * FL_WG_LOG + blockIdx.x] = wall_clock64();
    fl.wg_start[(size_t)(4 + kernel) * FL_WG_LOG + blockIdx.x] =
        (long long)(unsigned)__builtin_amdgcn_s_getreg(63492) | ((long long)(unsigned)__builtin_amdgcn_s_getreg(63508) << 32);
  }
}
#endif
struct FlightFsmDev {
  SogmFsmParams   prm;
  double          check_duration;
  SogmFsmState   *state;
  const double   *goals;
  int32_t        *due, *reached;
  double         *pos_now;
  SogmFsmState   *log_state;
  int32_t        *log_due, *log_safe, *log_reached, *log_pub;
  double         *log_hover_start;
  SogmTrajRecord *log_own;
};
struct MapTarget {
  void     *grid;
  unsigned *bits;
  int       words;
  void     *cand;
  int      *n_cand;
  MarkLog   lg;
  float    *poses;
  double   *stamps;
};
struct MapFrame {
  const float        *cloud;
  const int32_t      *cloud_range;
  CloudBlocks         cb;
  const SogmCylinder *cyl;
  int                 n_cyl;
};
struct OverlayIO {
  const SogmTrajRecord *rec;
  int                   n_rec;
  const int32_t        *ego_ids;
  const double         *body;
  int                   n_body;
};
struct TickInputsIO {
  const SogmTrajRecord *own;
  double               *hover, *now, *t_start, *pva;
  double                start_offset;
};
struct FlightMapDev {
  MapTarget             tgt;
  const FlightWorld    *worlds;
  CloudBlocks           cb;
  OverlayIO             ov;
  const SogmTrajRecord *tables;
  int                   n_total;
  TickInputsIO          tick;
  double                t0, period;
  int                   n_reset, n_bits, n_marks, n_splat;
  int                   un_reset, un_bits, un_marks, un_splat;
  int                   n_head_wgs;
  int                   n_uhead_wgs;
  int                   n_uwork_wgs;
  int                   n_admit;
  int                   pace_ticks;
  size_t                agent_bytes;
  unsigned long long   *reset_stat;
  FlightFsmDev          fsm;
};
hipError_t launch_flight_map(const GridGeom &g, const FlightCtl &fl, const FlightMapDev &d, int n_workgroups, hipStream_t st);

struct SearchIO {
  const double *start_pva, *goal, *t_start;
  int32_t      *out_ret;
  double       *out_route;
  int32_t      *out_route_len;
  int           route_cap;
  int32_t      *out_stats;
  const int32_t *due;
};
struct CorridorIO {
  const double  *start_pva, *t_start, *route;
  const int32_t *route_len;
  int            route_cap;
  double        *out_polys;
  int32_t       *out_nfaces, *out_npoly;
  double        *out_goal;
  __device__ __forceinline__ int points(int agent) const {
    const int n = route_len[agent];
    return n < route_cap ? n : route_cap;
  }
};
struct QpIO {
  const double  *start_pva, *goal_pv, *polys;
  const int32_t *nfaces, *npoly;
  double        *out_cpts;
  int32_t       *out_status, *out_iters;
};
struct FinishArgs {
  double                corridor_tau;
  const int32_t        *ret, *npoly, *status;
  const double         *cpts;
  const SogmTrajRecord *swarm;
  int                   n_swarm;
  const int32_t        *swarm_ego;
  const double         *swarm_now, *t_start;
  const int32_t        *drone_ids;
  SogmTrajRecord       *out;
  int32_t              *out_ok, *out_safe;
  unsigned long long   *counters;
  SogmTrajRecord       *pub_own, *pub_table;
  const int32_t        *due;
};
struct FlightLightDev {
  CorridorIO      cor;
  FinishArgs      fin;
  SogmTrajRecord *tables;
  int             n_total, agent0;
  SogmTrajRecord *log_records;
  int32_t        *log_ok;
  FlightFsmDev    fsm;
};
struct CorridorWorkspace;
hipError_t launch_flight_light(const MapView &m, const SogmPlannerParams &pp, const CorridorWorkspace &ws, const FlightCtl &fl,
                               const FlightLightDev &d, int n_workgroups, hipStream_t st);
struct AstarWorkspace;
hipError_t launch_flight_search(const MapView &m, const SogmAstarParams &ap, double corridor_tau, const AstarWorkspace &wsp,
                                const FlightCtl &fl, int n_workgroups, const SearchIO &io, int spec, hipStream_t st);
struct QpWorkspace;
struct QpConst;
hipError_t launch_flight_qp(const SogmPlannerParams &pp, const SogmQpSettings &qs, const QpWorkspace &ws, const QpConst &qc,
                            const FlightCtl &fl, int n_workgroups, const QpIO &io, hipStream_t st);

struct PrestampDev {
  MapTarget    tgt;
  MapFrame     frame;
  TickInputsIO tick;
  double       stamp;
  float       *poses_host;
  int          n_agents;
  int          n_bits, n_marks;
  int          n_late, n_bits_late, n_marks_late;
  int          gate_agents;
};
hipError_t launch_prestamp_flow(const GridGeom &g, const FlowCtl &fc, const PrestampDev &ps, int n_workgroups, int n_qp,
                                int n_finish, hipStream_t st);

hipError_t launch_deconflict(int n_agents, const double *cpts, const int32_t *npoly, const SogmTrajRecord *rec,
                             int n_rec, const int32_t *ego_ids, const double *t_now, int32_t *out_safe,
                             hipStream_t st, int agent0, unsigned long long *counters = nullptr);
hipError_t launch_corridor(const MapView &m, const SogmPlannerParams &pp, const CorridorWorkspace &ws, int n_agents,
                           const CorridorIO &io, hipStream_t st, int agent0 = 0, hipEvent_t ev_map_read = nullptr);

hipError_t launch_flow_gate(const FlowCtl &fc, int expected, hipStream_t st);
hipError_t launch_corridor_flow(const MapView &m, const SogmPlannerParams &pp, const CorridorWorkspace &ws,
                                const FlowCtl &fc, int n_agents, int n_workgroups, const CorridorIO &io, hipStream_t st);
hipError_t launch_finish_flow(const FlowCtl &fc, int n_agents, int n_workgroups, const FinishArgs &f, hipStream_t st);

struct QpWorkspace {
  char  *scratch;
  size_t scratch_stride;
  int    dyn_lds_bytes;
  double *k1_scratch;
  const double *t_alloc;
  int           goal_stride;
  long long    *dbg;
  int           ablate;
};
size_t qp_scratch_bytes_per_agent(int max_faces);
size_t qp_k1_scratch_bytes_per_agent();
int    qp_kernel_setup();
struct QpConst {
  double QM[225];
};
int astar_resident_workgroups(int device);
hipError_t launch_qp(const SogmPlannerParams &pp, const SogmQpSettings &qs, const QpWorkspace &ws, const QpConst &qc,
                     int n_agents, const QpIO &io, hipStream_t st, int agent0 = 0);
hipError_t launch_qp_flow(const SogmPlannerParams &pp, const SogmQpSettings &qs, const QpWorkspace &ws, const QpConst &qc,
                          const FlowCtl &fc, int n_agents, int n_workgroups, const QpIO &io, hipStream_t st);

size_t astar_node_bytes();
hipError_t launch_astar(const MapView &m, const SogmAstarParams &ap, double corridor_tau, const AstarWorkspace &wsp,
                        int n_agents, const SearchIO &io, int32_t *out_trace, int trace_cap, hipStream_t st,
                        int agent0 = 0, const FlowCtl *fc = nullptr, int search_mode = 0);

}

#define SOGM_MAX_GROUPS 64

struct sogm_planner {
  sogm::Resources      res;
  sogm_ctx            *map;
  SogmAstarParams      ap;
  SogmPlannerParams    pp;
  SogmQpSettings       qs;
  sogm::AstarWorkspace aw;
  sogm::CorridorWorkspace cw;
  sogm::QpWorkspace qw;
  sogm::QpConst qc;
  int32_t *d_ret, *d_route_len, *d_stats;
  double  *d_route;
  int      route_cap;
  double  *d_polys, *d_goal, *d_cpts;
  int32_t *d_nfaces, *d_npoly, *d_status, *d_iters;
  int32_t              *d_safe;
  const SogmTrajRecord *swarm;
  int                   n_swarm;
  const int32_t        *swarm_ego;
  const double         *swarm_now;
  SogmTrajRecord       *pub_own, *pub_table;
  const int32_t        *due;
  int         n_groups;
  hipStream_t gstream[SOGM_MAX_GROUPS];
  hipEvent_t  ev_in, ev_corr[SOGM_MAX_GROUPS], ev_done[SOGM_MAX_GROUPS];
  hipEvent_t  ev_pts[SOGM_MAX_GROUPS];
  int            flow;
  int           *d_flow;
  long long     *d_flow_ts;
  sogm::FlowCtl  fc;
  hipStream_t    fstream[4];
  hipEvent_t     ev_pdone;
  sogm::PrestampDev ps;
  int            ps_on;
  int            ps_world_on;
  SogmWorld      ps_world;
  hipEvent_t     ev_gate, ev_fdone[4];
  int           *d_epoch;
  int            reset_epoch;
  int           *h_flow_fail;
  int sel_first, sel_count;
  int search_mode;
  int spec_astar;
  hipStream_t peek;
  sogm::FlightCtl     fl;
  int                *d_fl;
  sogm::FlightWorld  *d_fl_worlds, *h_fl_worlds;
  double             *d_fl_pva, *d_fl_tstart, *d_fl_now;
  hipStream_t         fl_stream[4];
  hipEvent_t          fl_ev_in, fl_ev_done[4];
  int                 fl_cus[4];
  int                 fl_wgs[4];
  int                 fl_epoch = 0;
  int                *fl_xready = nullptr;
  int                 fl_fsm_on = 0;
  SogmFlightFsm       fl_fsm{};
  int32_t            *d_fl_due = nullptr, *d_fl_reached = nullptr;
  double             *d_fl_posnow = nullptr;
};

inline sogm::AstarWorkspace astar_ws(const sogm_planner *p) {
  sogm::AstarWorkspace w = p->aw;
  if (!((p->map->profiling >> SOGM_PROF_ASTAR) & 1)) w.dbg = nullptr;
  return w;
}

inline int launched(const char *what, hipError_t e) {
  if (e == hipSuccess) return SOGM_OK;
  sogm::set_error(what, e);
  return SOGM_ERR_HIP;
}

inline sogm::SearchIO search_io(const sogm_planner *p, const double *start_pva, const double *goal, const double *t_start) {
  return sogm::SearchIO{.start_pva = start_pva, .goal = goal, .t_start = t_start, .out_ret = p->d_ret,
                        .out_route = p->d_route, .out_route_len = p->d_route_len, .route_cap = p->route_cap,
                        .out_stats = p->d_stats, .due = p->due};
}
inline sogm::CorridorIO corridor_io(const sogm_planner *p, const double *start_pva, const double *t_start) {
  return sogm::CorridorIO{.start_pva = start_pva, .t_start = t_start, .route = p->d_route,
                          .route_len = p->d_route_len, .route_cap = p->route_cap, .out_polys = p->d_polys,
                          .out_nfaces = p->d_nfaces, .out_npoly = p->d_npoly, .out_goal = p->d_goal};
}
inline sogm::QpIO qp_io(const sogm_planner *p, const double *start_pva) {
  return sogm::QpIO{.start_pva = start_pva, .goal_pv = p->d_goal, .polys = p->d_polys, .nfaces = p->d_nfaces,
                    .npoly = p->d_npoly, .out_cpts = p->d_cpts, .out_status = p->d_status, .out_iters = p->d_iters};
}
inline sogm::FinishArgs finish_args(const sogm_planner *p, const double *t_start, const int32_t *drone_ids,
                                    SogmTrajRecord *out, int32_t *out_ok) {
  return sogm::FinishArgs{.corridor_tau = p->pp.corridor_tau, .ret = p->d_ret, .npoly = p->d_npoly,
                          .status = p->d_status, .cpts = p->d_cpts, .swarm = p->swarm, .n_swarm = p->n_swarm,
                          .swarm_ego = p->swarm_ego, .swarm_now = p->swarm_now, .t_start = t_start,
                          .drone_ids = drone_ids, .out = out, .out_ok = out_ok, .out_safe = p->d_safe,
                          .counters = p->cw.counters, .pub_own = p->pub_own, .pub_table = p->pub_table,
                          .due = p->due};
}
```

pred-occ-planner_amd/planner.py:

```python
import ctypes as C

import numpy as np
import torch

from . import _abi
from ._abi import SOGM_MAX_PIECES, check, lib
from .sogm import _dev, _stream


def linprog_batched(c, A_rows, b_rows, row_range):
    n, d = c.shape
    x = torch.zeros((n, d), dtype=torch.float64, device=c.device)
    v = torch.zeros((n,), dtype=torch.float64, device=c.device)
    check(lib().sogm_linprog_batched(d, c.data_ptr(), A_rows.data_ptr(), b_rows.data_ptr(), row_range.data_ptr(),
                                     n, x.data_ptr(), v.data_ptr(), _stream()), "sogm_linprog_batched")
    return x, v


def firi_batched(bd, pc, pc_range, a, b, r=None, iterations=2, epsilon=1.0e-6, max_points=4096, max_faces=64):
    n, n_bd = int(bd.shape[0]), int(bd.shape[1])
    dev = bd.device
    if r is None:
        r = torch.ones((n, 3), dtype=torch.float64, device=dev)
    hp = torch.zeros((n, max_faces, 4), dtype=torch.float64, device=dev)
    nf = torch.zeros((n,), dtype=torch.int32, device=dev)
    st = torch.zeros((n,), dtype=torch.int32, device=dev)
    check(lib().sogm_firi_batched(bd.data_ptr(), n_bd, pc.data_ptr(), pc_range.data_ptr(), a.data_ptr(), b.data_ptr(),
                                  r.data_ptr(), iterations, epsilon, n, max_points, max_faces, hp.data_ptr(),
                                  nf.data_ptr(), st.data_ptr(), _stream()), "sogm_firi_batched")
    return hp, nf, st, r


def corridor_rules_batched(pps, start_pva, route, route_len, polys, nfaces, seg_state=None, planner=None):
    n, P, MF = int(polys.shape[0]), SOGM_MAX_PIECES, int(polys.shape[2])
    dev = polys.device
    pp = (_abi.SogmPlannerParams * max(n, 1))(*pps)
    f64 = lambda *shape: torch.zeros(shape, dtype=torch.float64, device=dev)
    i32 = lambda *shape: torch.zeros(shape, dtype=torch.int32, device=dev)
    out = {"box": f64(n, P, 6), "shrunk": f64(n, P, MF, 4), "seg_nfaces": i32(n, P), "seg_state": i32(n, P),
           "polys": f64(n, P, MF, 4), "nfaces": i32(n, P), "npoly": i32(n), "goal": f64(n, 6)}
    check(lib().sogm_corridor_rules_batched(
        planner._p if planner is not None else None, pp, start_pva.data_ptr(), route.data_ptr(), route_len.data_ptr(),
        int(route.shape[1]), polys.data_ptr(), nfaces.data_ptr(), seg_state.data_ptr() if seg_state is not None else None,
        n, MF, out["box"].data_ptr(), out["shrunk"].data_ptr(), out["seg_nfaces"].data_ptr(), out["seg_state"].data_ptr(),
        out["polys"].data_ptr(), out["nfaces"].data_ptr(), out["npoly"].data_ptr(), out["goal"].data_ptr(), _stream()),
        "sogm_corridor_rules_batched")
    return out


class SogmPlanner:
    def __init__(self, sogm_map, astar_params, planner_params, qp_settings):
        self.map = sogm_map
        self.ap, self.pp, self.qs = astar_params, planner_params, qp_settings
        self.A = sogm_map.n_agents
        self._p = C.c_void_p()
        check(lib().sogm_planner_create(sogm_map.ctx, C.byref(astar_params), C.byref(planner_params),
                                        C.byref(qp_settings), C.byref(self._p)), "sogm_planner_create")

    def close(self):
        if self._p:
            torch.cuda.synchronize()
            lib().sogm_planner_destroy(self._p)
            self._p = C.c_void_p()

    def __del__(self):
        try:
            self.close()
        except Exception:
            pass

    def select_agents(self, first=0, count=None):
        check(lib().sogm_planner_select_agents(self._p, first, self.A if count is None else count),
              "sogm_planner_select_agents")

    def set_search_mode(self, mode):
        check(lib().sogm_planner_set_search_mode(self._p, mode), "sogm_planner_set_search_mode")

    def flow_error(self):
        return int(lib().sogm_planner_flow_error(self._p))

    def flow_failures(self):
        out = (C.c_int32 * 2)()
        check(lib().sogm_planner_flow_failures(self._p, out), "sogm_planner_flow_failures")
        return int(out[0]), int(out[1])

    def counters(self, reset=False):
        out = (C.c_int64 * len(_abi.COUNTER_NAMES))()
        check(lib().sogm_planner_counters(self._p, out, 1 if reset else 0), "sogm_planner_counters")
        return dict(zip(_abi.COUNTER_NAMES, [int(v) for v in out]))

    def search(self, start_pva, goal, t_start, route_cap=64, trace_cap=0):
        A, dev = self.A, start_pva.device
        out = {
            "ret": torch.zeros((A,), dtype=torch.int32, device=dev),
            "route": torch.zeros((A, route_cap, 6), dtype=torch.float64, device=dev),
            "route_len": torch.zeros((A,), dtype=torch.int32, device=dev),
            "stats": torch.zeros((A, 4), dtype=torch.int32, device=dev),
            "trace": torch.full((A, max(trace_cap, 1)), -1, dtype=torch.int32, device=dev),
        }
        check(lib().sogm_astar_search(self._p, start_pva.data_ptr(), goal.data_ptr(), t_start.data_ptr(),
                                      out["ret"].data_ptr(), out["route"].data_ptr(),
                                      out["route_len"].data_ptr(), route_cap, out["stats"].data_ptr(),
                                      out["trace"].data_ptr() if trace_cap else None, trace_cap, _stream()),
              "sogm_astar_search")
        return out

    def generateCorridors(self, start_pva, t_start, route, route_len):
        A, dev = self.A, start_pva.device
        mf = self.pp.max_faces
        out = {
            "polys": torch.zeros((A, SOGM_MAX_PIECES, mf, 4), dtype=torch.float64, device=dev),
            "nfaces": torch.zeros((A, SOGM_MAX_PIECES), dtype=torch.int32, device=dev),
            "npoly": torch.zeros((A,), dtype=torch.int32, device=dev),
            "goal": torch.zeros((A, 6), dtype=torch.float64, device=dev),
        }
        check(lib().sogm_corridor_generate(self._p, start_pva.data_ptr(), t_start.data_ptr(),
                                           route.data_ptr(), route_len.data_ptr(), int(route.shape[1]),
                                           out["polys"].data_ptr(), out["nfaces"].data_ptr(),
                                           out["npoly"].data_ptr(), out["goal"].data_ptr(), _stream()),
              "sogm_corridor_generate")
        return out

    def optimize(self, start_pva, goal_pv, polys, nfaces, npoly):
        A, dev = self.A, start_pva.device
        out = {
            "cpts": torch.zeros((A, SOGM_MAX_PIECES * 15), dtype=torch.float64, device=dev),
            "status": torch.zeros((A,), dtype=torch.int32, device=dev),
            "iters": torch.zeros((A,), dtype=torch.int32, device=dev),
        }
        check(lib().sogm_bezier_qp_solve(self._p, start_pva.data_ptr(), goal_pv.data_ptr(),
                                         polys.data_ptr(), nfaces.data_ptr(), npoly.data_ptr(),
                                         out["cpts"].data_ptr(), out["status"].data_ptr(),
                                         out["iters"].data_ptr(), _stream()), "sogm_bezier_qp_solve")
        return out

    def optimize_timed(self, start_pva, end_pva, time_alloc, polys, nfaces, npoly, max_vel, max_acc):
        A, dev = self.A, start_pva.device
        out = {
            "cpts": torch.zeros((A, SOGM_MAX_PIECES * 15), dtype=torch.float64, device=dev),
            "status": torch.zeros((A,), dtype=torch.int32, device=dev),
            "iters": torch.zeros((A,), dtype=torch.int32, device=dev),
        }
        check(lib().sogm_bezier_qp_solve_timed(self._p, start_pva.data_ptr(), end_pva.data_ptr(), time_alloc.data_ptr(),
                                               float(max_vel), float(max_acc), polys.data_ptr(), nfaces.data_ptr(),
                                               npoly.data_ptr(), out["cpts"].data_ptr(), out["status"].data_ptr(),
                                               out["iters"].data_ptr(), _stream()), "sogm_bezier_qp_solve_timed")
        return out

    def isSafeAfterOpt(self, cpts, npoly, records, n_records, ego_ids, t_now):
        safe = torch.empty((self.A,), dtype=torch.int32, device=cpts.device)
        check(lib().sogm_safe_after_opt(self._p, cpts.data_ptr(), npoly.data_ptr(), records.data_ptr(), n_records,
                                        ego_ids.data_ptr(), t_now.data_ptr(), safe.data_ptr(), _stream()),
              "sogm_safe_after_opt")
        return safe

    def setSwarm(self, records, n_records, ego_ids, t_now):
        self._swarm = (records, ego_ids, t_now)
        if records is None:
            check(lib().sogm_planner_set_swarm(self._p, None, 0, None, None), "sogm_planner_set_swarm")
        else:
            check(lib().sogm_planner_set_swarm(self._p, records.data_ptr(), n_records, ego_ids.data_ptr(),
                                               t_now.data_ptr()), "sogm_planner_set_swarm")

    def set_due(self, due=None):
        self._due = due
        check(lib().sogm_planner_set_due(self._p, due.data_ptr() if due is not None else None), "sogm_planner_set_due")

    def set_flight_fsm(self, prm=None, check_duration=0.2, state=None, logs=None):
        if prm is None:
            self._flight_fsm = None
            check(lib().sogm_planner_set_flight_fsm(self._p, None), "sogm_planner_set_flight_fsm")
            return
        logs = dict(logs or {})
        ptr = lambda t: t.data_ptr() if t is not None else None
        f = _abi.SogmFlightFsm(prm, float(check_duration), ptr(state), ptr(logs.get("state")), ptr(logs.get("due")),
                               ptr(logs.get("safe")), ptr(logs.get("reached")), ptr(logs.get("pub")),
                               ptr(logs.get("hover_start")), ptr(logs.get("own")))
        self._flight_fsm = (state, logs)
        check(lib().sogm_planner_set_flight_fsm(self._p, C.byref(f)), "sogm_planner_set_flight_fsm")

    def setPublish(self, own_records, next_table=None):
        self._publish = (own_records, next_table)
        check(lib().sogm_planner_set_publish(self._p, own_records.data_ptr() if own_records is not None else None,
                                             next_table.data_ptr() if next_table is not None else None),
              "sogm_planner_set_publish")

    def setPrestamp(self, cloud, cloud_range, cylinders, n_cyl, next_stamp, start_offset, hover, now, t_start, pva,
                    poses=None, world=None):
        if cloud is None and world is None:
            self._prestamp = None
            check(lib().sogm_planner_set_prestamp(self._p, None), "sogm_planner_set_prestamp")
            return
        ptr = lambda t: t.data_ptr() if t is not None else None
        ps = _abi.SogmPrestamp(ptr(cloud), ptr(cloud_range), ptr(cylinders), int(n_cyl or 0), 0,
                               float(next_stamp), float(start_offset), hover.data_ptr(), now.data_ptr(),
                               t_start.data_ptr(), pva.data_ptr(), ptr(poses),
                               C.pointer(world.c) if world is not None else None)
        self._prestamp = (cloud, cloud_range, cylinders, hover, now, t_start, pva, poses, world)
        check(lib().sogm_planner_set_prestamp(self._p, C.byref(ps)), "sogm_planner_set_prestamp")

    def flight(self, worlds, first_tick, t0, period, start_offset, goals, drone_ids, hover, own, tables, log_records,
               log_ok, n_total=None, agent0=0, comm=None):
        n = len(worlds)
        arr = (_abi.SogmWorld * n)(*[w.c for w in worlds])
        f = _abi.SogmFlight(n, int(first_tick), float(t0), float(period), float(start_offset), arr, goals.data_ptr(),
                            drone_ids.data_ptr(), hover.data_ptr(), own.data_ptr(), tables.data_ptr(),
                            self.A if n_total is None else int(n_total), int(agent0),
                            log_records.data_ptr(), log_ok.data_ptr(), comm)
        self._flight_keep = (worlds, arr, goals, drone_ids, hover, own, tables, log_records, log_ok)
        check(lib().sogm_flight_run(self._p, C.byref(f), _stream()), "sogm_flight_run")

    def flight_prepare(self, max_cloud_points=0):
        check(lib().sogm_flight_prepare(self._p, int(max_cloud_points)), "sogm_flight_prepare")

    def flight_stats(self):
        ms = np.zeros((self.A, 8), np.float64)
        hdr = np.zeros((32,), np.int32)
        check(lib().sogm_flight_stats(self._p, ms.ctypes.data_as(C.c_void_p), hdr.ctypes.data_as(C.c_void_p)),
              "sogm_flight_stats")
        return ms, hdr

    def replan(self, start_pva, goal, t_start, drone_ids, out_records=None, out_ok=None):
        A, dev = self.A, start_pva.device
        if out_records is None:
            out_records = torch.zeros((A, _abi.TRAJ_RECORD_BYTES), dtype=torch.uint8, device=dev)
        if out_ok is None:
            out_ok = torch.zeros((A,), dtype=torch.int32, device=dev)
        check(lib().sogm_replan(self._p, start_pva.data_ptr(), goal.data_ptr(), t_start.data_ptr(),
                                drone_ids.data_ptr(), out_records.data_ptr(), out_ok.data_ptr(), _stream()),
              "sogm_replan")
        return out_records, out_ok


def records_from_bytes(buf):
    n = buf.shape[0]
    arr = (_abi.SogmTrajRecord * n).from_buffer_copy(np.ascontiguousarray(buf).tobytes())
    return arr


def traj_eval(records, t):
    n = int(t.numel())
    pva = torch.empty((n, 9), dtype=torch.float64, device=t.device)
    ok = torch.empty((n,), dtype=torch.int32, device=t.device)
    check(lib().sogm_traj_eval(records.data_ptr(), n, t.data_ptr(), pva.data_ptr(), ok.data_ptr(), _stream()),
          "sogm_traj_eval")
    return pva, ok


def smoke_check(pop, sogm, orc, spec, sc, dev, m):
    A = sc["n_agents"]
    ap, pp, qs = pop.config.make_astar_params(), pop.config.make_planner_params(True), pop.config.make_qp_settings()
    P = SogmPlanner(m, ap, pp, qs)
    pva = np.concatenate([sc["starts"], np.zeros((A, 6))], axis=1)
    t_start = sc["stamps"] + 0.02
    rec_d, ok_d = P.replan(_dev(pva, np.float64), _dev(sc["goals"], np.float64), _dev(t_start, np.float64),
                           dev["ego_ids"])
    got = records_from_bytes(rec_d.cpu().numpy())
    ok = ok_d.cpu().numpy()
    cyl = pop.scene.cylinders_to_struct(sc["cylinders"])
    recs = pop.scene.straight_records(sc)
    for a in range(A):
        g = orc.update_gt(spec, sc["cloud"], cyl, dev["n_cyl"], sc["poses"][a])
        orc.project_neighbours(spec, g, recs, A, a, m.body, sc["poses"][a], sc["stamps"][a])
        w_ok, w, _ = orc.replan(spec, ap, pp, qs, g, sc["poses"][a], sc["stamps"][a], pva[a], sc["goals"][a],
                                t_start[a], a)
        assert ok[a] == w_ok and got[a].n_pieces == w.n_pieces, "replan outcome differs from the oracle"
        k = w.n_pieces * 15
        assert np.allclose(np.array(got[a].cpts[:k]), np.array(w.cpts[:k]), atol=1e-4, rtol=0)
    P.close()
```

Baseline: 12670 replans/s.

## Check adjacent corridor pair validity eagerly as segments finish

Adds an eager path in which each corridor segment workgroup, once done, sets a per-agent ready bit and checks the LP-based intersection with any neighbouring segment that is already finished, recording the verdict in pair_ok. The last workgroup then finalizes using the precomputed verdicts and only runs the serial pairwise checks that were not done early. The aim is to spread the finalize tail's sequential corridorValidW calls across workgroups. In exchange it adds atomics, fences, extra reset work, debug counters and a parallel rules kernel option, and risks races on the ready bits.

```diff
diff --git a/include/sogm_abi_debug.h b/include/sogm_abi_debug.h
--- a/include/sogm_abi_debug.h
+++ b/include/sogm_abi_debug.h
@@ -51,6 +51,15 @@
                                 const int32_t *nfaces, const int32_t *seg_state, int n, int max_faces, double *out_box,
                                 double *out_shrunk, int32_t *out_seg_nfaces, int32_t *out_seg_state, double *out_polys,
                                 int32_t *out_nfaces, int32_t *out_npoly, double *out_goal, void *stream);
+#define SOGM_RULES_PARALLEL 1
+int sogm_corridor_rules_batched_flags(sogm_planner *counters_of, const SogmPlannerParams *pp_host, const double *start_pva,
+                                      const double *route, const int32_t *route_len, int route_cap, const double *polys,
+                                      const int32_t *nfaces, const int32_t *seg_state, int n, int max_faces,
+                                      double *out_box, double *out_shrunk, int32_t *out_seg_nfaces, int32_t *out_seg_state,
+                                      double *out_polys, int32_t *out_nfaces, int32_t *out_npoly, double *out_goal,
+                                      int flags, void *stream);
+
+int sogm_debug_corridor_pairs(sogm_planner *p, unsigned long long *out4);
 
 #ifdef __cplusplus
 }
diff --git a/pred-occ-planner_amd/_abi.py b/pred-occ-planner_amd/_abi.py
--- a/pred-occ-planner_amd/_abi.py
+++ b/pred-occ-planner_amd/_abi.py
@@ -157,6 +157,7 @@
 FSM_PUB_NONE, FSM_PUB_NEW, FSM_PUB_HOVER = 0, 1, 2
 
 FLIGHT_MAX_TICKS = 64
+RULES_PARALLEL = 1
 FLIGHT_HDR_ERR, FLIGHT_HDR_FINISHED, FLIGHT_HDR_LATE_WGS = 4, 5, 15
 FLIGHT_STAT_NAMES = ("gate_wait", "map", "search", "corridor", "qp", "finish", "chain", "ticks")
 TRAJ_RECORD_BYTES = C.sizeof(SogmTrajRecord)
@@ -220,6 +221,9 @@
     "sogm_linprog_batched": (_i, [_i, _vp, _vp, _vp, _vp, _i, _vp, _vp, _vp]),
     "sogm_corridor_rules_batched": (_i, [_vp, _vp, _vp, _vp, _vp, _i, _vp, _vp, _vp, _i, _i, _vp, _vp, _vp, _vp, _vp, _vp,
                                          _vp, _vp, _vp]),
+    "sogm_corridor_rules_batched_flags": (_i, [_vp, _vp, _vp, _vp, _vp, _i, _vp, _vp, _vp, _i, _i, _vp, _vp, _vp, _vp, _vp,
+                                               _vp, _vp, _vp, _i, _vp]),
+    "sogm_debug_corridor_pairs": (_i, [_vp, _vp]),
     "sogm_replan": (_i, [_vp, _vp, _vp, _vp, _vp, _vp, _vp, _vp]),
     "sogm_gridmap_create": (_i, [C.POINTER(SogmGridMapParams), _i, _i, C.POINTER(_vp)]),
     "sogm_gridmap_destroy": (None, [_vp]),
diff --git a/pred-occ-planner_amd/csrc/sogm_corridor.hip b/pred-occ-planner_amd/csrc/sogm_corridor.hip
--- a/pred-occ-planner_amd/csrc/sogm_corridor.hip
+++ b/pred-occ-planner_amd/csrc/sogm_corridor.hip
@@ -1151,8 +1151,10 @@
   corridor_segment_body<FIRI_DIRECT_BD_MAX, true>(m, pp, ws, CorridorIO{}, blockIdx.x, 0, smem, fd);
 }
 
+template <bool PAIRS = false>
 __device__ __forceinline__ void corridor_finalize_body(const SogmPlannerParams &pp, const CorridorWorkspace &ws,
-                                                       const CorridorIO &io, int agent, const LpScratch &sc) {
+                                                       const CorridorIO &io, int agent, const LpScratch &sc,
+                                                       const int32_t *pair_row = nullptr, long long *stamps = nullptr) {
   const bool    w0    = threadIdx.x == 0;
   const int     MF    = pp.max_faces;
   const double *polys = ws.polys + (size_t)agent * SOGM_MAX_PIECES * MF * 4;
@@ -1162,6 +1164,8 @@
   const double *sp    = io.start_pva + agent * 9;
   const int     rl    = io.points(agent);
   int           npoly = 0;
+  if constexpr (PAIRS)
+    if (stamps && w0) stamps[0] = stamps[1] = stamps[2] = stamps[3] = wall_clock64();
   if (w0) {
     for (int i = 0; i < SOGM_MAX_PIECES; ++i) io.out_nfaces[agent * SOGM_MAX_PIECES + i] = 0;
     for (int i = 0; i < 6; ++i) io.out_goal[agent * 6 + i] = 0;
@@ -1179,12 +1183,30 @@
   if (npoly == SOGM_MAX_PIECES && io.route_len[agent] - 1 > SOGM_MAX_PIECES && w0 && ws.counters)
     atomicAdd(&ws.counters[SOGM_CNT_PIECES_CAPACITY], 1ull);
   if (npoly == 0) return;
-  for (int i = 0; i + 1 < npoly; ++i) {
-    if (!corridorValidW(polys + (size_t)i * MF * 4, nfs[i], polys + (size_t)(i + 1) * MF * 4,
-                        nfs[i + 1], sc)) {
-      if (i < 2) return;
-      npoly = pp.fake_planner ? i + 1 : i;
-      break;
+  if constexpr (!PAIRS) {
+    for (int i = 0; i + 1 < npoly; ++i) {
+      if (!corridorValidW(polys + (size_t)i * MF * 4, nfs[i], polys + (size_t)(i + 1) * MF * 4,
+                          nfs[i + 1], sc)) {
+        if (i < 2) return;
+        npoly = pp.fake_planner ? i + 1 : i;
+        break;
+      }
+    }
+  } else {
+    int n_late = 0, n_used = 0;
+    for (int i = 0; i + 1 < npoly; ++i) {
+      const int v = pair_row ? pair_row[i] : 0;
+      ++(v ? n_used : n_late);
+      if (v == 2 || (v == 0 && !corridorValidW(polys + (size_t)i * MF * 4, nfs[i], polys + (size_t)(i + 1) * MF * 4,
+                                               nfs[i + 1], sc))) {
+        npoly = i < 2 ? 0 : pp.fake_planner ? i + 1 : i;
+        break;
+      }
+    }
+    if (w0) {
+      if (pair_row && ws.pair_cnt && n_late) atomicAdd(&ws.pair_cnt[1], (unsigned long long)n_late);
+      if (pair_row && ws.pair_cnt && n_used) atomicAdd(&ws.pair_cnt[2], (unsigned long long)n_used);
+      if (stamps) stamps[1] = stamps[2] = stamps[3] = wall_clock64();
     }
   }
   if (pp.fake_planner ? npoly == 0 : npoly <= 1) return;
@@ -1210,6 +1232,8 @@
       }
     }
   }
+  if constexpr (PAIRS)
+    if (stamps && w0) stamps[2] = stamps[3] = wall_clock64();
   for (int i = 0; i < npoly; ++i) {
     if (w0) io.out_nfaces[agent * SOGM_MAX_PIECES + i] = nfs[i];
     const double *src = polys + (size_t)i * MF * 4;
@@ -1222,6 +1246,8 @@
       io.out_goal[agent * 6 + 3 + k] = gvel[k];
     }
     io.out_npoly[agent] = npoly;
+    if constexpr (PAIRS)
+      if (stamps) stamps[3] = wall_clock64();
   }
 }
 
@@ -1243,50 +1269,99 @@
   const int32_t           *state_in;
   double                  *out_box;
 };
+__device__ __forceinline__ void rules_segment(const CorridorRules &cr, const SogmPlannerParams &pp, const CorridorWorkspace &ws,
+                                              const CorridorIO &io, int prob, int seg, char *smem) {
+  double *base = (double *)smem, *s_poly = base + RulesLds::poly, *s_box = base + RulesLds::box, *s_w = base + RulesLds::w;
+  const LpScratch sc{base + LpLds::work, base + LpLds::rows, (int *)(smem + RulesLds::perm)};
+  const int lane = threadIdx.x, MF = pp.max_faces;
+  const int slot = prob * SOGM_MAX_PIECES + seg;
+  if (seg >= io.points(prob) - 1) {
+    if (lane == 0) {
+      ws.seg_state[slot]  = -2;
+      ws.seg_nfaces[slot] = 0;
+      for (int k = 0; k < 6; ++k) cr.out_box[slot * 6 + k] = 0.0;
+    }
+    return;
+  }
+  int nf = cr.nfaces_in[slot];
+  nf     = nf < 0 ? 0 : (nf > MF ? MF : nf);
+  if (lane == 0) segment_box(pp, io.start_pva + prob * 9, io.route + (size_t)prob * io.route_cap * 6, seg, s_box, s_w);
+  for (int i = lane; i < nf * 4; i += 64) s_poly[i] = cr.polys_in[(size_t)slot * MF * 4 + i];
+  wave_lds_sync();
+  shrink_corridor(pp, s_w, s_poly, nf);
+  wave_lds_sync();
+  const bool valid = corridorValidW(s_poly, nf, nullptr, 0, sc);
+  double    *out   = ws.polys + (size_t)slot * MF * 4;
+  for (int i = lane; i < nf * 4; i += 64) out[i] = s_poly[i];
+  if (lane == 0) {
+    for (int k = 0; k < 6; ++k) cr.out_box[slot * 6 + k] = s_box[k];
+    ws.seg_nfaces[slot] = nf;
+    ws.seg_state[slot]  = cr.state_in && cr.state_in[slot] == -3 ? -3 : (valid ? 1 : 0);
+  }
+  wave_lds_sync();
+}
 __global__ __launch_bounds__(64) void k_corridor_rules(CorridorRules cr, CorridorWorkspace ws, CorridorIO io) {
   extern __shared__ __attribute__((aligned(16))) char smem[];
-  double *base = (double *)smem, *s_poly = base + RulesLds::poly, *s_box = base + RulesLds::box, *s_w = base + RulesLds::w;
+  double         *base = (double *)smem;
   const LpScratch sc{base + LpLds::work, base + LpLds::rows, (int *)(smem + RulesLds::perm)};
-  const int               prob = blockIdx.x, lane = threadIdx.x;
+  const int               prob = blockIdx.x;
   const SogmPlannerParams pp   = cr.pp[prob];
-  const int               MF   = pp.max_faces;
-  const int               rl   = io.points(prob);
-  for (int seg = 0; seg < SOGM_MAX_PIECES; ++seg) {
-    const int slot = prob * SOGM_MAX_PIECES + seg;
-    if (seg >= rl - 1) {
-      if (lane == 0) {
-        ws.seg_state[slot]  = -2;
-        ws.seg_nfaces[slot] = 0;
-        for (int k = 0; k < 6; ++k) cr.out_box[slot * 6 + k] = 0.0;
-      }
-      continue;
-    }
-    int nf = cr.nfaces_in[slot];
-    nf     = nf < 0 ? 0 : (nf > MF ? MF : nf);
-    if (lane == 0) segment_box(pp, io.start_pva + prob * 9, io.route + (size_t)prob * io.route_cap * 6, seg, s_box, s_w);
-    for (int i = lane; i < nf * 4; i += 64) s_poly[i] = cr.polys_in[(size_t)slot * MF * 4 + i];
-    wave_lds_sync();
-    shrink_corridor(pp, s_w, s_poly, nf);
-    wave_lds_sync();
-    const bool valid = corridorValidW(s_poly, nf, nullptr, 0, sc);
-    double    *out   = ws.polys + (size_t)slot * MF * 4;
-    for (int i = lane; i < nf * 4; i += 64) out[i] = s_poly[i];
-    if (lane == 0) {
-      for (int k = 0; k < 6; ++k) cr.out_box[slot * 6 + k] = s_box[k];
-      ws.seg_nfaces[slot] = nf;
-      ws.seg_state[slot]  = cr.state_in && cr.state_in[slot] == -3 ? -3 : (valid ? 1 : 0);
-    }
-    wave_lds_sync();
-  }
+  for (int seg = 0; seg < SOGM_MAX_PIECES; ++seg) rules_segment(cr, pp, ws, io, prob, seg, smem);
   __threadfence_block();
   __syncthreads();
   corridor_finalize_body(pp, ws, io, prob, sc);
 }
 
+#ifndef SOGM_PAIRS_EAGER
+#define SOGM_PAIRS_EAGER 1
+#endif
+__device__ __forceinline__ void corridor_pairs_eager(const SogmPlannerParams &pp, const CorridorWorkspace &ws, int agent,
+                                                     int seg, const LpScratch &sc) {
+  unsigned old = 0;
+  if (threadIdx.x == 0) old = __hip_atomic_fetch_or(&ws.seg_ready[agent], 1u << seg, __ATOMIC_RELAXED, __HIP_MEMORY_SCOPE_AGENT);
+  old = __builtin_amdgcn_readfirstlane(old);
+  if (!(old & ((1u << seg) >> 1 | 2u << seg))) return;
+  __threadfence();
+  const int     MF    = pp.max_faces;
+  const double *polys = ws.polys + (size_t)agent * SOGM_MAX_PIECES * MF * 4;
+  const int    *nfs   = ws.seg_nfaces + agent * SOGM_MAX_PIECES;
+  const int    *state = ws.seg_state + agent * SOGM_MAX_PIECES;
+  if (state[seg] == 1) {
+    for (int lo = seg - 1; lo <= seg; ++lo) {
+      const int other = lo == seg ? seg + 1 : lo;
+      if (other < 0 || other >= SOGM_MAX_PIECES || !((old >> other) & 1u) || state[other] != 1) continue;
+      const bool meet = corridorValidW(polys + (size_t)lo * MF * 4, nfs[lo], polys + (size_t)(lo + 1) * MF * 4, nfs[lo + 1], sc);
+      if (threadIdx.x == 0) {
+        ws.pair_ok[agent * SOGM_MAX_PIECES + lo] = meet ? 1 : 2;
+        if (ws.pair_cnt) atomicAdd(&ws.pair_cnt[0], 1ull);
+      }
+    }
+  }
+  __threadfence();
+}
+
+__device__ __forceinline__ bool corridor_slot_done(const SogmPlannerParams &pp, const CorridorWorkspace &ws, const CorridorIO &io,
+                                                   int agent, int seg, bool real, char *smem, int *seg_done, bool cumulative) {
+  __threadfence();
+  const bool eager = SOGM_PAIRS_EAGER && ws.seg_ready;
+  if (eager && real) corridor_pairs_eager(pp, ws, agent, seg, LpLds::carve(smem));
+  const int done = flow_ticket(&seg_done[agent]);
+  if ((cumulative ? done & (SOGM_MAX_PIECES - 1) : done) != SOGM_MAX_PIECES - 1) return false;
+  __threadfence();
+  corridor_finalize_body<true>(pp, ws, io, agent, LpLds::carve(smem), eager ? ws.pair_ok + agent * SOGM_MAX_PIECES : nullptr,
+                               ws.fin_dbg ? ws.fin_dbg + agent * 4 : nullptr);
+  if (eager) {
+    if (threadIdx.x < SOGM_MAX_PIECES) ws.pair_ok[agent * SOGM_MAX_PIECES + threadIdx.x] = 0;
+    if (threadIdx.x == 0) ws.seg_ready[agent] = 0u;
+  }
+  __syncthreads();
+  return true;
+}
 __device__ __forceinline__ bool corridor_slot(const MapView &m, const SogmPlannerParams &pp, const CorridorWorkspace &ws,
                                               const CorridorIO &io, int agent, int seg, char *smem, int *seg_done,
                                               bool cumulative, long long *stamps) {
-  if (seg < io.points(agent) - 1) {
+  const bool real = seg < io.points(agent) - 1;
+  if (real) {
     corridor_points_body<1>(m, pp, ws, io, agent, seg);
     __threadfence_block();
     __syncthreads();
@@ -1295,13 +1370,21 @@
   corridor_segment_body<6, false>(m, pp, ws, io, agent, seg, smem, FiriDirect{});
   __syncthreads();
   if (stamps && threadIdx.x == 0) stamps[14] = wall_clock64();
-  __threadfence();
-  const int done = flow_ticket(&seg_done[agent]);
-  if ((cumulative ? done & (SOGM_MAX_PIECES - 1) : done) != SOGM_MAX_PIECES - 1) return false;
-  __threadfence();
-  corridor_finalize_body(pp, ws, io, agent, LpLds::carve(smem));
+  return corridor_slot_done(pp, ws, io, agent, seg, real, smem, seg_done, cumulative);
+}
+
+__global__ __launch_bounds__(64) void k_corridor_rules_slots(CorridorRules cr, CorridorWorkspace ws, CorridorIO io, int *seg_done) {
+  extern __shared__ __attribute__((aligned(16))) char smem[];
+  const int               prob = blockIdx.x / SOGM_MAX_PIECES, seg = blockIdx.x % SOGM_MAX_PIECES;
+  const SogmPlannerParams pp   = cr.pp[prob];
+  rules_segment(cr, pp, ws, io, prob, seg, smem);
   __syncthreads();
-  return true;
+  corridor_slot_done(pp, ws, io, prob, seg, seg < io.points(prob) - 1, smem, seg_done, false);
+}
+__global__ void k_pairs_residue(const unsigned *words, int n, unsigned long long *pair_cnt) {
+  unsigned v = 0;
+  for (int i = threadIdx.x; i < n; i += blockDim.x) v |= words[i];
+  if (v) atomicOr(&pair_cnt[3], (unsigned long long)v);
 }
 
 __global__ __launch_bounds__(64) void k_corridor_flow(MapView m, SogmPlannerParams pp, CorridorWorkspace ws,
@@ -1911,7 +1994,20 @@
                                            double *out_shrunk, int32_t *out_seg_nfaces, int32_t *out_seg_state,
                                            double *out_polys, int32_t *out_nfaces, int32_t *out_npoly,
                                            double *out_goal, void *stream) {
-  if (n < 0 || max_faces < 1 || max_faces > RULES_MAX_FACES || route_cap <= SOGM_MAX_PIECES ||
+  return sogm_corridor_rules_batched_flags(counters_of, pp_host, start_pva, route, route_len, route_cap, polys, nfaces, seg_state,
+                                           n, max_faces, out_box, out_shrunk, out_seg_nfaces, out_seg_state, out_polys,
+                                           out_nfaces, out_npoly, out_goal, 0, stream);
+}
+
+extern "C" int sogm_corridor_rules_batched_flags(sogm_planner *counters_of, const SogmPlannerParams *pp_host,
+                                                 const double *start_pva, const double *route, const int32_t *route_len,
+                                                 int route_cap, const double *polys, const int32_t *nfaces,
+                                                 const int32_t *seg_state, int n, int max_faces, double *out_box,
+                                                 double *out_shrunk, int32_t *out_seg_nfaces, int32_t *out_seg_state,
+                                                 double *out_polys, int32_t *out_nfaces, int32_t *out_npoly,
+                                                 double *out_goal, int flags, void *stream) {
+  if ((flags & ~SOGM_RULES_PARALLEL) || ((flags & SOGM_RULES_PARALLEL) && n > (1 << 20)) ||
+      n < 0 || max_faces < 1 || max_faces > RULES_MAX_FACES || route_cap <= SOGM_MAX_PIECES ||
       (n > 0 && (!pp_host || !start_pva || !route || !route_len || !polys || !nfaces || !out_box || !out_shrunk ||
                  !out_seg_nfaces || !out_seg_state || !out_polys || !out_nfaces || !out_npoly || !out_goal)))
     return SOGM_ERR_INVALID_ARG;
@@ -1923,6 +2019,12 @@
   SOGM_HIP_CHECK(hipMallocAsync((void **)&d_pp, sizeof(SogmPlannerParams) * (size_t)n, st));
   hipError_t e = hipMemcpyAsync(d_pp, pp_host, sizeof(SogmPlannerParams) * (size_t)n, hipMemcpyHostToDevice, st);
   if (e == hipSuccess) e = hipStreamSynchronize(st);
+  int         *d_ctl = nullptr;
+  const size_t n_ctl = (size_t)n + sogm::corridor_pair_words(n);
+  if (e == hipSuccess && (flags & SOGM_RULES_PARALLEL)) {
+    e = hipMallocAsync((void **)&d_ctl, sizeof(int) * n_ctl, st);
+    if (e == hipSuccess) e = hipMemsetAsync(d_ctl, 0, sizeof(int) * n_ctl, st);
+  }
   if (e == hipSuccess) {
     sogm::CorridorWorkspace ws{};
     ws.polys      = out_shrunk;
@@ -1933,9 +2035,21 @@
                                  .out_polys = out_polys, .out_nfaces = out_nfaces, .out_npoly = out_npoly,
                                  .out_goal = out_goal};
     const sogm::CorridorRules cr{d_pp, polys, nfaces, seg_state, out_box};
-    hipLaunchKernelGGL(sogm::k_corridor_rules, dim3(n), dim3(64), sogm::RulesLds::bytes(), st, cr, ws, io);
+    if (flags & SOGM_RULES_PARALLEL) {
+      ws.seg_ready = reinterpret_cast<unsigned *>(d_ctl + n);
+      ws.pair_ok   = d_ctl + 2 * (size_t)n;
+      ws.pair_cnt  = counters_of ? counters_of->cw.pair_cnt : nullptr;
+      hipLaunchKernelGGL(sogm::k_corridor_rules_slots, dim3(n * SOGM_MAX_PIECES), dim3(64), sogm::RulesLds::bytes(), st, cr, ws,
+                         io, d_ctl);
+      if (ws.pair_cnt)
+        hipLaunchKernelGGL(sogm::k_pairs_residue, dim3(1), dim3(256), 0, st, ws.seg_ready, (int)sogm::corridor_pair_words(n),
+                           ws.pair_cnt);
+    } else {
+      hipLaunchKernelGGL(sogm::k_corridor_rules, dim3(n), dim3(64), sogm::RulesLds::bytes(), st, cr, ws, io);
+    }
     e = hipGetLastError();
   }
+  if (d_ctl) (void)hipFreeAsync(d_ctl, st);
   (void)hipFreeAsync(d_pp, st);
   SOGM_HIP_CHECK(e);
   return SOGM_OK;
diff --git a/pred-occ-planner_amd/csrc/sogm_flight.hip b/pred-occ-planner_amd/csrc/sogm_flight.hip
--- a/pred-occ-planner_amd/csrc/sogm_flight.hip
+++ b/pred-occ-planner_amd/csrc/sogm_flight.hip
@@ -9,13 +9,14 @@
 using namespace sogm;
 
 __global__ __launch_bounds__(256) void k_flight_reset(FlightCtl fl, int n_words, int *verdict, long long *acc, int *log_words,
-                                                      long long n_log_words) {
+                                                      long long n_log_words, unsigned *pairs, int n_pairs) {
   const long long i0 = (long long)blockIdx.x * blockDim.x + threadIdx.x, step = (long long)gridDim.x * blockDim.x;
   for (long long i = i0; i < n_words; i += step)
     if (i != FL_UW_TAIL && i != FL_UW_HEAD) fl.hdr[i] = 0;
   if (i0 == 0) fl.hdr[FL_UW_HEAD] = fl.hdr[FL_UW_TAIL];
   for (long long i = i0; i < n_log_words; i += step) log_words[i] = 0;
   for (long long i = i0; i < fl.n_agents; i += step) verdict[i] = 0;
+  for (long long i = i0; i < n_pairs; i += step) pairs[i] = 0u;
   for (long long i = i0; i < 8ll * fl.n_agents; i += step) acc[i] = 0;
   for (long long i = i0; i < 16; i += step) fl.prof[i] = 0ull;
   for (long long i = i0; i < 8 * FL_WG_LOG; i += step) fl.wg_start[i] = 0;
@@ -246,7 +247,7 @@
   const int       n_words = FlightBlock::reset_words(A);
   const long long n_log  = (long long)f->n_ticks * A * (long long)(sizeof(SogmTrajRecord) / sizeof(int));
   hipLaunchKernelGGL(k_flight_reset, dim3(256), dim3(256), 0, main, fl, n_words, p->aw.verdict, p->fl.acc,
-                     reinterpret_cast<int *>(f->log_records), n_log);
+                     reinterpret_cast<int *>(f->log_records), n_log, p->cw.seg_ready, (int)corridor_pair_words(A));
   SOGM_HIP_CHECK(hipGetLastError());
   SOGM_HIP_CHECK(hipMemsetAsync(f->log_ok, 0, sizeof(int32_t) * (size_t)f->n_ticks * A, main));
   hipLaunchKernelGGL(k_flight_seed, dim3((A + 255) / 256), dim3(256), 0, main, fl);
diff --git a/pred-occ-planner_amd/csrc/sogm_planner.hip b/pred-occ-planner_amd/csrc/sogm_planner.hip
--- a/pred-occ-planner_amd/csrc/sogm_planner.hip
+++ b/pred-occ-planner_amd/csrc/sogm_planner.hip
@@ -5,6 +5,7 @@
 #include <cstdlib>
 #include <cstring>
 #include <new>
+#include <vector>
 
 #include "sogm_planner.hpp"
 
@@ -115,6 +116,10 @@
   SOGM_HIP_CHECK(p->res.device(&p->cw.seg_npts, sizeof(int32_t) * slots));
   SOGM_HIP_CHECK(p->res.device(&p->cw.seg_dbg, sizeof(long long) * 16 * slots, true));
   SOGM_HIP_CHECK(p->res.device(&p->cw.counters, sizeof(unsigned long long) * SOGM_CNT_N, true));
+  SOGM_HIP_CHECK(p->res.device(&p->cw.seg_ready, sizeof(int32_t) * sogm::corridor_pair_words(A), true));
+  p->cw.pair_ok = reinterpret_cast<int32_t *>(p->cw.seg_ready) + A;
+  SOGM_HIP_CHECK(p->res.device(&p->cw.pair_cnt, sizeof(unsigned long long) * 4, true));
+  SOGM_HIP_CHECK(p->res.device(&p->cw.fin_dbg, sizeof(long long) * 4 * (size_t)A, true));
   p->qw.scratch_stride = qp_scratch_bytes_per_agent(pp->max_faces);
   p->qw.dyn_lds_bytes  = qp_kernel_setup();
   SOGM_HIP_CHECK(p->res.device(&p->qw.scratch, p->qw.scratch_stride * (size_t)A));
@@ -298,6 +303,23 @@
   return SOGM_OK;
 }
 
+int sogm_debug_corridor_pairs(sogm_planner *p, unsigned long long *out4) {
+  if (!p || !out4) return SOGM_ERR_INVALID_ARG;
+  SOGM_HIP_CHECK(hipDeviceSynchronize());
+  SOGM_HIP_CHECK(hipMemcpy(out4, p->cw.pair_cnt, sizeof(unsigned long long) * 4, hipMemcpyDeviceToHost));
+  SOGM_HIP_CHECK(hipMemset(p->cw.pair_cnt, 0, sizeof(unsigned long long) * 4));
+  std::vector<uint32_t> words(sogm::corridor_pair_words(p->map->n_agents));
+  SOGM_HIP_CHECK(hipMemcpy(words.data(), p->cw.seg_ready, sizeof(uint32_t) * words.size(), hipMemcpyDeviceToHost));
+  for (const uint32_t w : words) out4[3] |= w;
+  return SOGM_OK;
+}
+int sogm_debug_corridor_finalize_times(sogm_planner *p, long long *out_host) {
+  if (!p || !out_host) return SOGM_ERR_INVALID_ARG;
+  SOGM_HIP_CHECK(hipDeviceSynchronize());
+  SOGM_HIP_CHECK(hipMemcpy(out_host, p->cw.fin_dbg, sizeof(long long) * 4 * (size_t)p->map->n_agents, hipMemcpyDeviceToHost));
+  return SOGM_OK;
+}
+
 int sogm_bezier_qp_solve(sogm_planner *p, const double *start_pva, const double *goal_pv,
                          const double *polys, const int32_t *nfaces, const int32_t *npoly,
                          double *out_cpts, int32_t *out_status, int32_t *out_iters, void *stream) {
@@ -514,10 +536,12 @@
 }
 
 __global__ __launch_bounds__(1024) void k_flow_reset(int *hdr, int n_hdr, int *ready, int n_ready, int *verdict,
-                                                     int n_verdict, int *epoch_word, int epoch, int *gen_word, int gen) {
+                                                     int n_verdict, unsigned *pairs, int n_pairs, int *epoch_word, int epoch,
+                                                     int *gen_word, int gen) {
   const int i0 = (int)threadIdx.x, step = (int)blockDim.x;
   for (int i = i0; i < n_hdr; i += step) hdr[i] = 0;
   for (int i = i0; i < n_ready; i += step) ready[i] = -1;
+  for (int i = i0; i < n_pairs; i += step) pairs[i] = 0u;
   if (verdict)
     for (int i = i0; i < n_verdict; i += step) verdict[i] = 0;
   __threadfence();
@@ -571,7 +595,7 @@
   int *gen_word = p->d_flow + fb.gen;
   ++p->reset_epoch;
   hipLaunchKernelGGL(k_flow_reset, dim3(1), dim3(1024), 0, sC, p->d_flow, fb.zero_words(), p->d_flow + fb.fill_first(),
-                     fb.fill_words(), spec ? p->aw.verdict : nullptr, A,
+                     fb.fill_words(), spec ? p->aw.verdict : nullptr, A, p->cw.seg_ready, (int)sogm::corridor_pair_words(A),
                      c->overlap >= 2 && c->clear_gate ? c->clear_epoch_word : nullptr,
                      c->overlap >= 2 && c->clear_gate ? sogm::next_clear_epoch(c) : 0, gen_word, p->reset_epoch);
   SOGM_HIP_CHECK(hipGetLastError());
diff --git a/pred-occ-planner_amd/csrc/sogm_planner.hpp b/pred-occ-planner_amd/csrc/sogm_planner.hpp
--- a/pred-occ-planner_amd/csrc/sogm_planner.hpp
+++ b/pred-occ-planner_amd/csrc/sogm_planner.hpp
@@ -26,7 +26,12 @@
   int32_t *seg_npts;
   long long *seg_dbg;
   unsigned long long *counters;
-};
+  unsigned *seg_ready;
+  int32_t  *pair_ok;
+  unsigned long long *pair_cnt;
+  long long *fin_dbg;
+};
+constexpr size_t corridor_pair_words(int A) { return (size_t)A * (1 + SOGM_MAX_PIECES); }
 
 static_assert(SOGM_MAX_PIECES <= WK_MAX_SUB, "a search pushes one corridor descriptor per segment slot, sub = the slot");
 struct FlightWorld {
diff --git a/pred-occ-planner_amd/planner.py b/pred-occ-planner_amd/planner.py
--- a/pred-occ-planner_amd/planner.py
+++ b/pred-occ-planner_amd/planner.py
@@ -31,7 +31,7 @@
     return hp, nf, st, r
 
 
-def corridor_rules_batched(pps, start_pva, route, route_len, polys, nfaces, seg_state=None, planner=None):
+def corridor_rules_batched(pps, start_pva, route, route_len, polys, nfaces, seg_state=None, planner=None, parallel=False):
     n, P, MF = int(polys.shape[0]), SOGM_MAX_PIECES, int(polys.shape[2])
     dev = polys.device
     pp = (_abi.SogmPlannerParams * max(n, 1))(*pps)
@@ -39,12 +39,12 @@
     i32 = lambda *shape: torch.zeros(shape, dtype=torch.int32, device=dev)
     out = {"box": f64(n, P, 6), "shrunk": f64(n, P, MF, 4), "seg_nfaces": i32(n, P), "seg_state": i32(n, P),
            "polys": f64(n, P, MF, 4), "nfaces": i32(n, P), "npoly": i32(n), "goal": f64(n, 6)}
-    check(lib().sogm_corridor_rules_batched(
+    check(lib().sogm_corridor_rules_batched_flags(
         planner._p if planner is not None else None, pp, start_pva.data_ptr(), route.data_ptr(), route_len.data_ptr(),
         int(route.shape[1]), polys.data_ptr(), nfaces.data_ptr(), seg_state.data_ptr() if seg_state is not None else None,
         n, MF, out["box"].data_ptr(), out["shrunk"].data_ptr(), out["seg_nfaces"].data_ptr(), out["seg_state"].data_ptr(),
-        out["polys"].data_ptr(), out["nfaces"].data_ptr(), out["npoly"].data_ptr(), out["goal"].data_ptr(), _stream()),
-        "sogm_corridor_rules_batched")
+        out["polys"].data_ptr(), out["nfaces"].data_ptr(), out["npoly"].data_ptr(), out["goal"].data_ptr(),
+        _abi.RULES_PARALLEL if parallel else 0, _stream()), "sogm_corridor_rules_batched_flags")
     return out
 
 
@@ -88,6 +88,11 @@
         out = (C.c_int64 * len(_abi.COUNTER_NAMES))()
         check(lib().sogm_planner_counters(self._p, out, 1 if reset else 0), "sogm_planner_counters")
         return dict(zip(_abi.COUNTER_NAMES, [int(v) for v in out]))
+
+    def corridor_pairs(self):
+        out = (C.c_uint64 * 4)()
+        check(lib().sogm_debug_corridor_pairs(self._p, out), "sogm_debug_corridor_pairs")
+        return dict(zip(("eager", "late", "consumed", "residue"), [int(v) for v in out]))
 
     def search(self, start_pva, goal, t_start, route_cap=64, trace_cap=0):
         A, dev = self.A, start_pva.device
```

Measured after the change: 12870 replans/s (median of 6 runs). 1.6% higher.
